# kazuto1011/dusty-gan

Measured on AMD Instinct MI355X. Metric: G+D train images/sec on 64x1024 LiDAR (steps/sec beside it), higher is better.
Workload: dtype bf16

## Files before the change

dusty_gan_amd/_lib.py:

```python
import ctypes as C
import os
import subprocess

_HERE = os.path.dirname(os.path.abspath(__file__))
CSRC = os.path.join(_HERE, "csrc")
LIB_PATH = os.path.join(CSRC, "libdustygan_hip.so")
if os.environ.get("DUSTY_GAN_LIB_DIAG"):
    _d = os.environ["DUSTY_GAN_LIB_DIAG"]
    LIB_PATH = os.path.join(CSRC, "libdustygan_hip_diag%s.so" % ("" if _d == "1" else _d))

DG_OK, DG_EINVAL, DG_EUNSUPPORTED, DG_EHIP = 0, 1, 2, 3
DG_F32, DG_BF16 = 0, 1
DG_BF16X2 = 2
MODE_S2, MODE_UP, MODE_GEMM = 0, 1, 2
EPI_LINEAR, EPI_LRELU, EPI_MASK = 0, 1, 2
DG_FORCE_AUTO, DG_FORCE_DIRECT, DG_FORCE_MFMA, DG_FORCE_THIN, DG_FORCE_LOCKSTEP, DG_FORCE_PINGPONG = 0, 1, 2, 3, 4, 5
DG_FORCE_WG_REGSTAGED, DG_FORCE_WG_DMA_PAIRS, DG_FORCE_WG_DMA_NOPAIRS, DG_FORCE_PINGPONG_SINGLE, DG_FORCE_PROJ_STREAM = 6, 7, 8, 9, 10
DG_FORCE_FP32X3 = 0x100
DG_CONV_FAMILY_DIRECT, DG_CONV_FAMILY_MFMA, DG_CONV_FAMILY_THIN, DG_CONV_FAMILY_LOCKSTEP, DG_CONV_FAMILY_PINGPONG = 1, 2, 3, 4, 5
DG_CONV_FAMILY_PROJ_STREAM = 6
DG_WGRAD_VARIANT_DIRECT, DG_WGRAD_VARIANT_MFMA, DG_WGRAD_VARIANT_THIN, DG_WGRAD_VARIANT_DMA, DG_WGRAD_VARIANT_THIN_MFMA = 1, 2, 3, 5, 7
POLICY_BITS = {"brightness": 1, "saturation": 2, "contrast": 4, "translation": 8, "cutout": 16}

_ERR = {1: "DG_EINVAL (bad argument)", 2: "DG_EUNSUPPORTED (shape not supported by the requested kernel)",
        3: "DG_EHIP (HIP runtime error)"}


class DgError(RuntimeError):
    pass


class DgConv(C.Structure):
    _fields_ = [
        ("mode", C.c_int), ("adj", C.c_int), ("ring", C.c_int),
        ("B", C.c_int), ("Hc", C.c_int), ("Wc", C.c_int),
        ("K", C.c_int), ("N", C.c_int),
        ("in_", C.c_void_p), ("in_sb", C.c_long), ("in_sp", C.c_long), ("in_sk", C.c_long),
        ("out", C.c_void_p), ("out_sb", C.c_long), ("out_sp", C.c_long), ("out_sn", C.c_long),
        ("w", C.c_void_p), ("w_st", C.c_long), ("w_sk", C.c_long), ("w_sn", C.c_long),
        ("scale", C.c_float), ("epi", C.c_int),
        ("bias", C.c_void_p), ("bias_mod", C.c_int),
        ("aux", C.c_void_p), ("dbias", C.c_void_p), ("rowscale", C.c_void_p),
        ("in_dtype", C.c_int), ("out_dtype", C.c_int), ("w_dtype", C.c_int),
        ("nscale", C.c_void_p),
        ("up_frag", C.c_void_p),
        ("dbias_ws", C.c_void_p),
        ("dbias_part", C.c_void_p),
        ("mask_out", C.c_void_p),
        ("mask_in", C.c_void_p),
        ("tanh_sum_parts", C.c_void_p),
    ]


UP_FRAG_BYTES = 3 * 18 * 1024
DBIAS_WS_FLOATS = 32 * 1024


class DgUpFrag(C.Structure):
    _fields_ = [("off", C.c_longlong), ("frag", C.c_void_p), ("m_st", C.c_longlong), ("m_sn", C.c_longlong),
                ("m_sk", C.c_longlong), ("N", C.c_int), ("Hc", C.c_int), ("adj", C.c_int)]


class DgDraw(C.Structure):
    _fields_ = [("kind", C.c_int), ("fill_kind", C.c_int), ("seed", C.c_uint64), ("stream_id", C.c_uint64),
                ("offset_dev", C.c_void_p), ("base", C.c_ulonglong), ("lo", C.c_float), ("hi", C.c_float),
                ("eps", C.c_float), ("ilo", C.c_int), ("ihi", C.c_int), ("n", C.c_long), ("out", C.c_void_p),
                ("out_bf16", C.c_void_p), ("B", C.c_int), ("H", C.c_int), ("W", C.c_int), ("uf", C.c_void_p),
                ("qi", C.c_void_p)]


class DgWgrad(C.Structure):
    _fields_ = [
        ("wmode", C.c_int), ("ring", C.c_int),
        ("B", C.c_int), ("Hc", C.c_int), ("Wc", C.c_int),
        ("Ci", C.c_int), ("Co", C.c_int),
        ("a", C.c_void_p), ("a_sb", C.c_long), ("a_sp", C.c_long), ("a_sc", C.c_long),
        ("g", C.c_void_p), ("g_sb", C.c_long), ("g_sp", C.c_long), ("g_sc", C.c_long),
        ("dw", C.c_void_p), ("scale", C.c_float), ("rowscale", C.c_void_p),
        ("a_dtype", C.c_int), ("g_dtype", C.c_int),
        ("ws", C.c_void_p), ("g_mod", C.c_int),
    ]


XSUM_PARTS = 8


class DgFetch(C.Structure):
    _fields_ = [("pol", C.c_void_p), ("mask", C.c_void_p), ("pool_ctr", C.c_void_p), ("npool", C.c_int),
                ("min_depth", C.c_float), ("max_depth", C.c_float), ("drop_const", C.c_float), ("B", C.c_int), ("HW", C.c_long),
                ("out", C.c_void_p), ("parts", C.c_void_p), ("nslab", C.c_long), ("flip_tab", C.c_void_p)]


class DgAugSet(C.Structure):
    _fields_ = [("x", C.c_void_p), ("xsum", C.c_void_p), ("xsum_parts", C.c_int), ("u_b", C.c_void_p), ("u_c", C.c_void_p), ("t_h", C.c_void_p),
                ("t_w", C.c_void_p), ("o_x", C.c_void_p), ("o_y", C.c_void_p)]


class DgOptSeg(C.Structure):
    _fields_ = [("off", C.c_longlong), ("numel", C.c_longlong), ("part", C.c_void_p), ("splits", C.c_int), ("accumulate", C.c_int),
                ("kind", C.c_int), ("ci", C.c_int), ("co", C.c_int), ("shadow_t", C.c_void_p), ("ws_src", C.c_void_p),
                ("ws_coef", C.c_void_p), ("ws_stride", C.c_longlong), ("ws_n", C.c_int), ("ws_bf16", C.c_int),
                ("ws_scale", C.c_float), ("first_block", C.c_int)]


OPT_MAX_SEG = 20


class DgWgradPlan(C.Structure):
    _fields_ = [("variant", C.c_int), ("splits", C.c_int), ("ws_floats", C.c_long), ("tap_pairs", C.c_int)]


class DgWgradReduce(C.Structure):
    _fields_ = [("ws", C.c_void_p), ("dw", C.c_void_p), ("numel", C.c_long), ("splits", C.c_int), ("accumulate", C.c_int)]


class DgConvPlan(C.Structure):
    _fields_ = [("family", C.c_int), ("bm", C.c_int), ("bn", C.c_int), ("tiles", C.c_int), ("workgroups", C.c_int),
                ("tiles_per_wg", C.c_int), ("thin_mfma", C.c_int), ("mask_bits", C.c_int), ("dbias_rows", C.c_int),
                ("sum_parts", C.c_int)]


_P, _I, _L, _F, _D, _U64 = C.c_void_p, C.c_int, C.c_long, C.c_float, C.c_double, C.c_uint64

PROTOTYPES = {
    "dg_conv": [C.POINTER(DgConv), _I, _P],
    "dg_conv_ex": [C.POINTER(DgConv), _I, _I, _P],
    "dg_conv_plan": [C.POINTER(DgConv), _I, _I, C.POINTER(DgConvPlan)],
    "dg_conv_mfma_supported": [C.POINTER(DgConv)],
    "dg_wgrad": [C.POINTER(DgWgrad), _I, _I, _P],
    "dg_wgrad_plan": [C.POINTER(DgWgrad), _I, _I, C.POINTER(DgWgradPlan)],
    "dg_wgrad_group": [C.POINTER(DgWgrad), _I, _I, _I, _P],
    "dg_wgrad_group_plan": [C.POINTER(DgWgrad), _I, _I, _I, C.POINTER(DgWgradPlan)],
    "dg_wgrad_reduce": [C.POINTER(DgWgradReduce), _I, _P],
    "dg_wgrad_mfma_supported": [C.POINTER(DgWgrad)],
    "dg_wgrad_kernel_variant": [C.POINTER(DgWgrad), _I],
    "dg_wgrad_has_sample_map": [C.POINTER(DgWgrad), _I],
    "dg_blur_fwd": [_P, _P, _I, _I, _I, _I, _I, _P],
    "dg_blur_fwd_mean": [_P, _P, _I, _I, _I, _I, _I, _P, _I, _P, _P],
    "dg_blur_bwd": [_P, _I, _P, _I, _I, _I, _I, _P],
    "dg_blur_bwd_r1": [_P, _I, _P, _F, _P, _I, _I, _I, _I, _P],
    "dg_blur_r1_tangent": [_P, _I, _P, _F, _P, _P, _I, _I, _I, _I, _I, _P],
    "dg_final_fwd": [_P, _I, _P, _P, _F, _I, _L, _P, _P],
    "dg_final_fwd_acc": [_P, _I, _P, _P, _F, _I, _L, _P, _P],
    "dg_final_bwd_data": [_P, _I, _P, _P, _P, _F, _I, _L, _I, _P, _P, _P],
    "dg_batch_wsum": [_P, _I, _P, _F, _I, _L, _P, _P],
    "dg_head_post_fwd": [_P, _P, _P, _I, _I, _F, _F, _I, _L, _P, _P, _P],
    "dg_head_post_fwd_sum": [_P, _P, _P, _I, _I, _F, _F, _I, _L, _P, _P, _P, _P],
    "dg_head_post_bwd": [_P, _P, _P, _P, _P, _I, _F, _F, _I, _L, _F, _F, _P, _P, _P, _I, _P, _P],
    "dg_logistic_noise": [_P, _P, _F, _L, _P, _P],
    "dg_diffaug_fwd": [_P, _P, _P, _P, _P, _P, _P, _I, _I, _I, _I, _P, _P, _P],
    "dg_diffaug_bwd": [_P, _P, _P, _P, _P, _P, _P, _I, _I, _I, _I, _P, _P, _P],
    "dg_diffaug_fwd_acc": [_P, _P, _P, _P, _P, _P, _P, _I, _I, _I, _I, _P, _P, _P],
    "dg_diffaug_fwd_pre": [_P, _P, _P, _P, _P, _P, _P, _I, _I, _I, _I, _P, _P, _P],
    "dg_diffaug_bwd_acc": [_P, _P, _P, _P, _P, _P, _P, _I, _I, _I, _I, _P, _P, _P],
    "dg_diffaug_blur_fwd": [C.POINTER(DgAugSet), _I, _I, _I, _I, _I, _I, _P, _I, _P],
    "dg_blur_bwd_augsum": [_P, _I, _P, _P, _P, _P, _I, _P, _I, _I, _I, _I, _P],
    "dg_diffaug_bwd_pre": [_P, _P, _P, _P, _P, _P, _P, _I, _I, _I, _I, _P, _P, _P],
    "dg_head_post_bwd_aug": [_P, _P, _P, _P, _P, _P, _P, _P, _P, _P, _P, _I, _P, _I, _F, _F, _I, _I, _I, _F, _F, _P, _P, _P,
                             _I, _P, _P],
    "dg_fetch_reals_pool_sum": [_P, _P, _P, _I, _F, _F, _F, _I, _L, _P, _P, _P],
    "dg_fetch_reals_resident_sum": [_P, _P, _L, _P, _F, _F, _F, _I, _L, _P, _P, _P],
    "dg_resident_gather": [_P, _L, _I, _L, _L, _P, _P, _P, _P],
    "dg_gan_d_step": [_I, _F, _P, _P, _I, _F, _P, _P, _P, _P, _P, _P],
    "dg_gan_g_step": [_I, _P, _P, _I, _F, _P, _P, _P],
    "dg_final_gan_bwd": [_I, _I, _F, _P, _P, _I, _F, _I, _P, _P, _P, _P, _P, _P, _I, _P, _F, _L, _I, _P, _P, _P, _P, _P],
    "dg_det_arena": [_P, _L, _P],
    "dg_mean_acc": [_P, _I, _P, _P],
    "dg_fetch_reals": [_P, _P, _F, _F, _F, _L, _P, _P],
    "dg_fetch_reals_sum": [_P, _P, _F, _F, _F, _I, _L, _P, _P, _P],
    "dg_pl_penalty": [_P, _I, _I, _F, _P, _P, _P, _P],
    "dg_head_post_bwd2": [_P, _P, _P, _P, _P, _P, _I, _F, _F, _I, _L, _F, _F, _P, _P, _P, _I, _P],
    "dg_scan_to_polar": [_P, _I, _I, _I, _I, _I, _I, _P, _D, _D, _F, _P, _P, _P, _P, _P],
    "dg_inv_to_xyz": [_P, _P, _I, _I, _I, _I, _F, _F, _F, _F, _P, _P, _P],
    "dg_unit_map": [_P, _L, _I, _P, _P],
    "dg_normals": [_P, _I, _I, _I, _I, _P, _P],
    "dg_scan_project": [_P, _P, _I, _I, _I, _P, _P, _P, _P, _P],
    "dg_angle_accum": [_P, _I, _I, _I, _I, _D, _D, _P, _P, _P],
    "dg_angle_finish": [_P, _P, _I, _I, _P, _P],
    "dg_splat_accum": [_P, _P, _I, _L, _I, _I, _I, _P, _P],
    "dg_render_points": [_P, _P, _I, _L, _I, _P, _I, _P, _I, _D, _P, _P],
    "dg_splat_finish": [_P, _I, _I, _I, _I, _I, _P, _P],
    "dg_image_grid": [_P, _L, _I, _I, _I, _I, _F, _I, _P, _P],
    "dg_turbo_lut": [_P],
    "dg_fps": [_P, _I, _I, _I, _P, _P, _P, _P],
    "dg_chamfer_dir": [_P, _I, _I, _P, _I, _I, _P, _P],
    "dg_chamfer_paired": [_P, _I, _P, _I, _I, _P, _P],
    "dg_chamfer_nn": [_P, _L, _L, _L, _I, _P, _L, _L, _L, _I, _I, _P, _P, _P],
    "dg_emd": [_P, _I, _I, _P, _I, _I, _I, _P, _P],
    "dg_grid_vote": [_P, _L, _P, _I, _P, _P],
    "dg_jsd": [_P, _P, _I, _P, _P],
    "dg_pyr_down": [_P, _L, _I, _I, _P, _P],
    "dg_pyr_up_sub": [_P, _P, _L, _I, _I, _P],
    "dg_extract_patches": [_P, _I, _I, _I, _I, _I, _I, _P, _I, _P, _P],
    "dg_sample_sum": [_P, _I, _L, _I, _P, _P],
# ... 320 lines not shown
```

dusty_gan_amd/csrc/api.hip:

```cpp
#include "common.h"

int dg_conv_direct_launch(const ConvP* p, hipStream_t stream);
int dg_lrelu_bits_launch(const ConvP* p, hipStream_t stream);
int dg_conv_mfma_launch(const ConvP* p, hipStream_t stream, int force, int fp32x3, int wg_cap, DgConvPlan* plan);
int dg_wgrad_mfma_dma_supported(const WgradP* p);
int dg_wgrad_mfma_dma_launch(const WgradP* p, int accumulate, int pairs, hipStream_t stream, DgWgradPlan* plan);
int dg_wgrad_mfma_dma_group_launch(const WgradP* items, int n, int pairs, int rounds, hipStream_t stream, DgWgradPlan* plans);
int dg_conv_thin_launch(const ConvP* p, hipStream_t stream);
int dg_conv_thin_supported(const ConvP* p);
int dg_proj_stream_supported(const ConvP* p);
int dg_proj_stream_launch(const ConvP* p, hipStream_t stream, DgConvPlan* plan);
int dg_conv_thin_mfma_variant(const ConvP* p);
int dg_conv_up_mfma_sum_parts(const ConvP* p);
int dg_conv_s2_mfma_blocks(const ConvP* p);
int dg_wgrad_thin_mfma_variant(const WgradP* p);
int dg_wgrad_thin_ws_splits(const WgradP* p);
int dg_wgrad_mfma_ws_splits(const WgradP* p, int accumulate);
int dg_wgrad_direct_ws_splits(const WgradP* p);
int dg_wgrad_direct_launch(const WgradP* p, hipStream_t stream);
int dg_wgrad_mfma_launch(const WgradP* p, int accumulate, hipStream_t stream, int x3);
int dg_wgrad_thin_launch(const WgradP* p, hipStream_t stream);
int dg_wgrad_thin_supported(const WgradP* p);

namespace {

enum ConvKernel { CONV_DIRECT, CONV_THIN, CONV_MFMA, CONV_PROJ_STREAM };

int select_conv(const DgConv* p, int force_flags, ConvKernel* k, DgConvPlan* plan) {
  if (p && (p->mask_out || p->mask_in)) {
    if (p->mask_out && p->epi != EPI_LRELU) return DG_EINVAL;
    if (p->mask_in && p->epi != EPI_MASK) return DG_EINVAL;
    if (p->out_sn != 1 || p->N % 8 != 0 || p->out_sp % 8 != 0 || p->out_sb % 8 != 0) return DG_EUNSUPPORTED;
  }
  if (!p || !p->in || !p->out || !p->w) return DG_EINVAL;
  if (p->B <= 0 || p->K <= 0 || p->N <= 0) return DG_EINVAL;
  if (p->mode != MODE_GEMM && (p->Hc < 2 || p->Wc < 2)) return DG_EINVAL;
  if (p->epi == EPI_MASK && !p->aux) return DG_EINVAL;
  if (p->bias && p->bias_mod <= 0) return DG_EINVAL;
  if (p->dbias && p->bias_mod <= 0) return DG_EINVAL;
  if (plan) *plan = DgConvPlan{};
  const int force = force_flags & ~DG_FORCE_FP32X3;
  const bool mfma_ok = !p->nscale && dg_conv_mfma_supported(p), thin_ok = dg_conv_thin_supported(p);
  const bool proj_ok = dg_proj_stream_supported(p);
  bool ok = true;
  if (force == DG_FORCE_AUTO) *k = proj_ok ? CONV_PROJ_STREAM : (mfma_ok ? CONV_MFMA : (thin_ok ? CONV_THIN : CONV_DIRECT));
  else if (force == DG_FORCE_PROJ_STREAM) *k = CONV_PROJ_STREAM, ok = proj_ok;
  else if (force == DG_FORCE_MFMA || force == DG_FORCE_LOCKSTEP || force == DG_FORCE_PINGPONG ||
           force == DG_FORCE_PINGPONG_SINGLE) *k = CONV_MFMA, ok = mfma_ok;
  else if (force == DG_FORCE_THIN) *k = CONV_THIN, ok = thin_ok;
  else *k = CONV_DIRECT;
  return ok ? DG_OK : DG_EUNSUPPORTED;
}

int conv_run(const DgConv* p, ConvKernel k, int force_flags, int wg_cap, hipStream_t s, DgConvPlan* plan) {
  if (k == CONV_PROJ_STREAM) return dg_proj_stream_launch(p, s, plan);
  if (k == CONV_MFMA)
    return dg_conv_mfma_launch(p, s, force_flags & ~DG_FORCE_FP32X3, (force_flags & DG_FORCE_FP32X3) ? 1 : 0, wg_cap, plan);
  if (!plan) return k == CONV_THIN ? dg_conv_thin_launch(p, s) : dg_conv_direct_launch(p, s);
  plan->family = k == CONV_THIN ? DG_CONV_FAMILY_THIN : DG_CONV_FAMILY_DIRECT;
  if (k == CONV_THIN) {
    plan->thin_mfma = dg_conv_thin_mfma_variant(p);
    plan->mask_bits = plan->thin_mfma == 1 ? 3 : 0;
    plan->dbias_rows = plan->thin_mfma == 1 ? dg_conv_s2_mfma_blocks(p) : 0;
    plan->sum_parts = plan->thin_mfma == 2 ? dg_conv_up_mfma_sum_parts(p) : 0;
  }
  return DG_OK;
}

int conv_dispatch(const DgConv* p, int force_flags, int wg_cap, hipStream_t s, DgConvPlan* plan) {
  ConvKernel k;
  int rc = select_conv(p, force_flags, &k, plan);
  if (rc || plan || !p->mask_out) return rc ? rc : conv_run(p, k, force_flags, wg_cap, s, plan);
  DgConvPlan pl{};
  rc = conv_run(p, k, force_flags, wg_cap, nullptr, &pl);
  if (rc == DG_OK) rc = conv_run(p, k, force_flags, wg_cap, s, nullptr);
  if (rc == DG_OK && !(pl.mask_bits & 1)) rc = dg_lrelu_bits_launch(p, s);
  return rc;
}

struct WgradKernel {
  int variant;
  int pairs;
  int splits;
  long ws_floats;
  bool takes_gmod;
  bool zero_dw;
};

int select_wgrad(const DgWgrad* p, int accumulate, int force_flags, WgradKernel* k) {
  if (!p || !p->a || !p->g || !p->dw) return DG_EINVAL;
  if (p->B <= 0 || p->Ci <= 0 || p->Co <= 0 || p->Hc <= 0 || p->Wc <= 0) return DG_EINVAL;
  const int force = force_flags & ~DG_FORCE_FP32X3;
  const bool mfma_ok = dg_wgrad_mfma_supported(p), thin_ok = dg_wgrad_thin_supported(p);
  const bool pairs = force == DG_FORCE_WG_DMA_PAIRS || force == DG_FORCE_WG_DMA_NOPAIRS;
  *k = WgradKernel{};
  if ((force == DG_FORCE_AUTO || force == DG_FORCE_MFMA || pairs) && mfma_ok && dg_wgrad_mfma_dma_supported(p)) {
    k->variant = DG_WGRAD_VARIANT_DMA, k->takes_gmod = true;
    k->pairs = force == DG_FORCE_WG_DMA_PAIRS ? 1 : (force == DG_FORCE_WG_DMA_NOPAIRS ? 2 : 0);
    return DG_OK;
  }
  if (force == DG_FORCE_AUTO)
    k->variant = mfma_ok ? DG_WGRAD_VARIANT_MFMA : (thin_ok ? DG_WGRAD_VARIANT_THIN : DG_WGRAD_VARIANT_DIRECT);
  else if (force == DG_FORCE_MFMA || force == DG_FORCE_WG_REGSTAGED) k->variant = mfma_ok ? DG_WGRAD_VARIANT_MFMA : 0;
  else if (force == DG_FORCE_THIN) k->variant = thin_ok ? DG_WGRAD_VARIANT_THIN : 0;
  else if (!pairs) k->variant = DG_WGRAD_VARIANT_DIRECT;
  if (!k->variant) return DG_EUNSUPPORTED;
  const int thin_mfma = k->variant == DG_WGRAD_VARIANT_THIN ? dg_wgrad_thin_mfma_variant(p) : 0;
  if (thin_mfma) k->variant = DG_WGRAD_VARIANT_THIN_MFMA;
  k->takes_gmod = thin_mfma == 1;
  if (k->variant == DG_WGRAD_VARIANT_THIN || k->variant == DG_WGRAD_VARIANT_THIN_MFMA) k->splits = dg_wgrad_thin_ws_splits(p);
  else if (k->variant == DG_WGRAD_VARIANT_MFMA) k->splits = dg_wgrad_mfma_ws_splits(p, accumulate);
  else if ((force == DG_FORCE_AUTO || force == DG_FORCE_DIRECT) && !p->g_mod) k->splits = dg_wgrad_direct_ws_splits(p);
  k->ws_floats = k->splits * (long)(p->wmode == 2 ? 1 : 16) * p->Ci * p->Co;
  k->zero_dw = !accumulate && !p->ws && k->variant != DG_WGRAD_VARIANT_MFMA;
  return DG_OK;
}

int wgrad_dispatch(const DgWgrad* p, int accumulate, int force_flags, hipStream_t s, DgWgradPlan* plan) {
  WgradKernel k;
  const int rc = select_wgrad(p, accumulate, force_flags, &k);
  if (rc == DG_EINVAL) return rc;
  if (plan) *plan = DgWgradPlan{k.variant, k.splits ? k.splits : 1, k.ws_floats, 0};
  if (rc) return rc;
  if (k.variant == DG_WGRAD_VARIANT_DMA) return dg_wgrad_mfma_dma_launch(p, accumulate, k.pairs, s, plan);
// ... 57 lines not shown
```

dusty_gan_amd/csrc/blur_aug.hip:

```cpp
#include "pointwise.h"
#include "diffaug.h"

template <typename T>
__global__ void blur_fwd_kernel(const float* __restrict__ x, T* __restrict__ out, int B, int H, int W, int ring) {
  const long idx = (long)blockIdx.x * blockDim.x + threadIdx.x;
  const long total = (long)B * H * W;
  if (idx >= total) return;
  const int xx = (int)(idx % W), y = (int)((idx / W) % H);
  const long base = idx - (long)y * W - xx;
  const int yu = y == 0 ? 1 : y - 1, yd = y == H - 1 ? H - 2 : y + 1;
  int xl = xx - 1, xr = xx + 1;
  if (ring) { if (xl < 0) xl += W; if (xr >= W) xr -= W; }
  else      { if (xl < 0) xl = 1;  if (xr >= W) xr = W - 2; }
  const float c = x[idx];
  const float v = 0.25f * x[base + (long)yu * W + xx] + 0.5f * c + 0.25f * x[base + (long)yd * W + xx];
  const float h = 0.25f * x[base + (long)y * W + xl] + 0.5f * c + 0.25f * x[base + (long)y * W + xr];
  out[idx * 2 + 0] = (T)v;
  out[idx * 2 + 1] = (T)h;
}

template <typename T>
__global__ void blur_bwd_kernel(const T* __restrict__ d, float* __restrict__ dx, int B, int H, int W, int ring) {
  const long idx = (long)blockIdx.x * blockDim.x + threadIdx.x;
  const long total = (long)B * H * W;
// ... 131 lines not shown
                                                        float oscale, float* __restrict__ ssq, AugP win, int use_win,
                                                        const DgDet det) {
  __shared__ float red[16];
  const int W4 = W >> 2, b = blockIdx.y;
  const long base = (long)b * H * W;
  const int y0 = blockIdx.x * NR;
  const AugSample ws = aug_window(win, b);
  float ssacc = 0.f;
  for (int q4 = threadIdx.x; q4 < W4; q4 += 256) {
    const int x0 = q4 * 4;
    float g[NR][4];
    blur_adj_rows<T, NR>(d, base, y0, x0, H, W, ring, g);
#pragma unroll
    for (int j = 0; j < NR; ++j) {
      const int y = y0 + j;
      const float g0 = g[j][0], g1 = g[j][1], g2 = g[j][2], g3 = g[j][3];
      *(float4*)(dx + base + (long)y * W + x0) = make_float4(oscale * g0, oscale * g1, oscale * g2, oscale * g3);
      if (!use_win) {
        ssacc += g0 * g0 + g1 * g1 + g2 * g2 + g3 * g3;
      } else {
        const AugRow wr = aug_row<false>(win, ws, y);
        const float gq[4] = {g0, g1, g2, g3};
#pragma unroll
        for (int k = 0; k < 4; ++k)
          if (aug_in_window(wr, x0 + k)) ssacc += gq[k];
      }
    }
  }
  if (ssq) {
    const float sblk = dg_block_sum(ssacc, red);
    if (threadIdx.x == 0) dg_acc_add(&ssq[b], sblk, gridDim.x, det);
  }
}
template <typename T>
static void blur_bwd4_launch(const void* d, float* dx, int B, int H, int W, int ring, float oscale, float* ssq, int rows_pb,
                             const AugP& win, int use_win, hipStream_t s) {
  const dim3 grid(H / rows_pb, B);
  const DgDet det = dg_det_current();
  if (rows_pb == 4) blur_bwd4_kernel<T, 4><<<grid, 256, 0, s>>>((const T*)d, dx, H, W, ring, oscale, ssq, win, use_win, det);
  else if (rows_pb == 2) blur_bwd4_kernel<T, 2><<<grid, 256, 0, s>>>((const T*)d, dx, H, W, ring, oscale, ssq, win, use_win, det);
  else blur_bwd4_kernel<T, 1><<<grid, 256, 0, s>>>((const T*)d, dx, H, W, ring, oscale, ssq, win, use_win, det);
}
static void blur_bwd4_launch(const void* d, int dtype, float* dx, int B, int H, int W, int ring, float oscale, float* ssq,
                             int rows_pb, const AugP& win, int use_win, hipStream_t s) {
  if (dtype == DG_BF16) blur_bwd4_launch<bf16>(d, dx, B, H, W, ring, oscale, ssq, rows_pb, win, use_win, s);
  else blur_bwd4_launch<float>(d, dx, B, H, W, ring, oscale, ssq, rows_pb, win, use_win, s);
}
static int blur_rows_pb(int H) { return H % 4 == 0 ? 4 : (H % 2 == 0 ? 2 : 1); }

#define R1T_ROWS 4
template <typename T>
__global__ __launch_bounds__(256) void blur_r1_tangent_kernel(const T* __restrict__ d, T* __restrict__ out, int H, int W,
                                                              int ring, float oscale, float* __restrict__ ssq,
                                                              float* __restrict__ mean_acc, int mean_n, const DgDet det) {
  extern __shared__ float s_g[];
  __shared__ float red[16];
  const int W4 = W >> 2, b = blockIdx.y;
  const long base = (long)b * H * W;
  const int y0 = blockIdx.x * R1T_ROWS;
  float ssacc = 0.f;
  for (int q4 = threadIdx.x; q4 < W4; q4 += 256) {
    const int x0 = q4 * 4;
    float g[R1T_ROWS + 2][4];
    blur_adj_rows<T, R1T_ROWS + 2>(d, base, y0 - 1, x0, H, W, ring, g);
#pragma unroll
    for (int r = 0; r < R1T_ROWS + 2; ++r) {
      const int y = y0 - 1 + r;
      if (y < 0 || y >= H) continue;
      const float g0 = g[r][0], g1 = g[r][1], g2 = g[r][2], g3 = g[r][3];
      *(float4*)(s_g + r * W + x0) = make_float4(oscale * g0, oscale * g1, oscale * g2, oscale * g3);
      if (r >= 1 && r <= R1T_ROWS) ssacc += g0 * g0 + g1 * g1 + g2 * g2 + g3 * g3;
    }
  }
  __syncthreads();
  for (int yy = 0; yy < R1T_ROWS; ++yy) {
    const int y = y0 + yy;
    const int yu = y == 0 ? 1 : y - 1, yd = y == H - 1 ? H - 2 : y + 1;
    const float* rc = s_g + (y - y0 + 1) * W;
    const float* ru = s_g + (yu - y0 + 1) * W;
    const float* rd = s_g + (yd - y0 + 1) * W;
    for (int q4 = threadIdx.x; q4 < W4; q4 += 256) {
      const int x0 = q4 * 4;
      const float4 c4 = *(const float4*)(rc + x0);
      const float4 u4 = *(const float4*)(ru + x0);
      const float4 d4 = *(const float4*)(rd + x0);
      int xl = x0 - 1, xr = x0 + 4;
      if (ring) { if (xl < 0) xl += W; if (xr >= W) xr -= W; }
      else      { if (xl < 0) xl = 1;  if (xr >= W) xr = W - 2; }
      const float c[6] = {rc[xl], c4.x, c4.y, c4.z, c4.w, rc[xr]};
      const float u[4] = {u4.x, u4.y, u4.z, u4.w}, dn[4] = {d4.x, d4.y, d4.z, d4.w};
      float o[8];
#pragma unroll
      for (int k = 0; k < 4; ++k) {
        o[2 * k] = 0.25f * u[k] + 0.5f * c[k + 1] + 0.25f * dn[k];
        o[2 * k + 1] = 0.25f * c[k] + 0.5f * c[k + 1] + 0.25f * c[k + 2];
      }
      T* op = out + (base + (long)y * W + x0) * 2;
      if constexpr (sizeof(T) == 2) {
        Vec16<bf16>::store((bf16*)op, o);
      } else {
        *(float4*)op = make_float4(o[0], o[1], o[2], o[3]);
        *(float4*)(op + 4) = make_float4(o[4], o[5], o[6], o[7]);
      }
    }
  }
  const float sblk = dg_block_sum(ssacc, red);
  if (threadIdx.x == 0) {
    float tot = 0.f;
    const int last = dg_acc_add_last(&ssq[b], sblk, gridDim.x, det, tot);
    if (mean_acc) {
      if (last == 1) dg_acc_add(mean_acc, tot / (float)mean_n, gridDim.y, det);
      else if (last < 0) atomicAdd(mean_acc, sblk / (float)mean_n);
    }
  }
}

__global__ __launch_bounds__(256) void sample_sum_kernel(const float* __restrict__ x, long n, int sq,
                                                         float* __restrict__ out, const DgDet det) {
  __shared__ float red[16];
  const int b = blockIdx.y;
  const float* row = x + (long)b * n;
  float acc = 0.f;
  if ((n & 3) == 0 && (((size_t)row) & 15) == 0) {
    for (long i = ((long)blockIdx.x * blockDim.x + threadIdx.x) * 4; i < n; i += (long)gridDim.x * blockDim.x * 4) {
      const float4 v = *(const float4*)(row + i);
      acc += sq ? v.x * v.x + v.y * v.y + v.z * v.z + v.w * v.w : v.x + v.y + v.z + v.w;
    }
  } else {
    for (long i = (long)blockIdx.x * blockDim.x + threadIdx.x; i < n; i += (long)gridDim.x * blockDim.x) {
      const float v = row[i];
      acc += sq ? v * v : v;
    }
  }
  const float s = dg_block_sum(acc, red);
  if (threadIdx.x == 0) dg_acc_add(&out[b], s, gridDim.x, det);
}


__global__ __launch_bounds__(256) void diffaug_fwd_kernel(AugP a, const float* __restrict__ x, const float* __restrict__ xsum,
                                                          float* __restrict__ y) {
  const int yy = blockIdx.x, b = blockIdx.y, W = a.W;
  const long HW = (long)a.H * W;
  float* yrow = y + (long)b * HW + (long)yy * W;
  const AugSample s = aug_sample(a, b);
  const AugRow r = aug_row<false>(a, s, yy);
  const float mean = aug_mean(a, s, (a.policy & 4) ? xsum[b] : 0.f);
  const float* xrow = x + (long)b * HW + (long)(r.ok ? r.y : 0) * W;
#pragma unroll 4
  for (int xx = threadIdx.x; xx < W; xx += 256) {
    const float v = aug_fwd_px(s, mean, xrow[aug_src_col(s, xx)]);
// ... 116 lines not shown
  const float* grow = gy + (long)b * HW + (long)(r.ok ? r.y : 0) * W;
  const float gb = grow[W - 1];
#pragma unroll 4
  for (int c = threadIdx.x; c < W; c += 256) out[c] = aug_adj_px(a, s, r, grow, gb, gm, c);
}

static inline bool blur4_ok(const void* a, const void* b, int H, int W) {
  return W % 4 == 0 && W >= 8 && H >= 2 && ((size_t)a & 15) == 0 && ((size_t)b & 15) == 0;
}

extern "C" {

int dg_blur_fwd_mean(const float* x, void* out, int dtype, int B, int H, int W, int ring, const float* mean_src, int mean_n,
                     float* mean_acc, void* s_) {
  hipStream_t s = (hipStream_t)s_;
  if (!mean_src || !mean_acc || mean_n < 1) return DG_EINVAL;
  if (!blur4_ok(x, out, H, W)) return DG_EUNSUPPORTED;
  if (dtype == DG_BF16) blur_fwd4_kernel<bf16><<<dim3(H, B), 256, 0, s>>>(x, (bf16*)out, B, H, W, ring, mean_src, mean_n, mean_acc);
  else blur_fwd4_kernel<float><<<dim3(H, B), 256, 0, s>>>(x, (float*)out, B, H, W, ring, mean_src, mean_n, mean_acc);
  HIP_CHECK_RET(hipGetLastError());
  return DG_OK;
}

int dg_blur_fwd(const float* x, void* out, int dtype, int B, int H, int W, int ring, void* s_) {
  hipStream_t s = (hipStream_t)s_;
  const long n = (long)B * H * W;
  if (blur4_ok(x, out, H, W)) {
    if (dtype == DG_BF16) blur_fwd4_kernel<bf16><<<dim3(H, B), 256, 0, s>>>(x, (bf16*)out, B, H, W, ring, nullptr, 0, nullptr);
    else blur_fwd4_kernel<float><<<dim3(H, B), 256, 0, s>>>(x, (float*)out, B, H, W, ring, nullptr, 0, nullptr);
  } else if (dtype == DG_BF16) blur_fwd_kernel<bf16><<<nblk(n), 256, 0, s>>>(x, (bf16*)out, B, H, W, ring);
  else blur_fwd_kernel<float><<<nblk(n), 256, 0, s>>>(x, (float*)out, B, H, W, ring);
  HIP_CHECK_RET(hipGetLastError());
  return DG_OK;
}

int dg_blur_bwd(const void* d, int dtype, float* dx, int B, int H, int W, int ring, void* s_) {
  hipStream_t s = (hipStream_t)s_;
  const long n = (long)B * H * W;
  if (blur4_ok(d, dx, H, W)) blur_bwd4_launch(d, dtype, dx, B, H, W, ring, 1.f, nullptr, 1, AugP{}, 0, s);
  else if (dtype == DG_BF16) blur_bwd_kernel<bf16><<<nblk(n), 256, 0, s>>>((const bf16*)d, dx, B, H, W, ring);
  else blur_bwd_kernel<float><<<nblk(n), 256, 0, s>>>((const float*)d, dx, B, H, W, ring);
  HIP_CHECK_RET(hipGetLastError());
  return DG_OK;
}

int dg_blur_bwd_r1(const void* d, int dtype, float* dx, float oscale, float* ssq, int B, int H, int W, int ring, void* s_) {
  if (!ssq) return DG_EINVAL;
  if (!blur4_ok(d, dx, H, W) || ((long)H * W) % 1024 != 0) return DG_EUNSUPPORTED;
  blur_bwd4_launch(d, dtype, dx, B, H, W, ring, oscale, ssq, blur_rows_pb(H), AugP{}, 0, (hipStream_t)s_);
  HIP_CHECK_RET(hipGetLastError());
  return DG_OK;
}

int dg_blur_r1_tangent(const void* d, int dtype, void* out, float oscale, float* ssq, float* mean_acc, int mean_n, int B, int H,
                       int W, int ring, void* s_) {
  hipStream_t s = (hipStream_t)s_;
  if (!d || !out || !ssq || B <= 0 || (mean_acc && mean_n < 1)) return DG_EINVAL;
  if (dtype != DG_BF16 && dtype != DG_F32) return DG_EINVAL;
  const size_t lds = (size_t)(R1T_ROWS + 2) * W * sizeof(float);
  if (W % 4 != 0 || W < 8 || H < 4 || H % R1T_ROWS != 0 || lds > 60 * 1024 || ((size_t)d & 15) != 0 || ((size_t)out & 15) != 0)
    return DG_EUNSUPPORTED;
  const dim3 grid(H / R1T_ROWS, B);
  const DgDet det = dg_det_current();
  if (dtype == DG_BF16) blur_r1_tangent_kernel<bf16><<<grid, 256, lds, s>>>((const bf16*)d, (bf16*)out, H, W, ring, oscale, ssq, mean_acc, mean_n, det);
  else blur_r1_tangent_kernel<float><<<grid, 256, lds, s>>>((const float*)d, (float*)out, H, W, ring, oscale, ssq, mean_acc, mean_n, det);
  HIP_CHECK_RET(hipGetLastError());
  return DG_OK;
}

static int sample_sum_impl(const float* x, int B, long n, int sq, float* out, bool zero, void* s_) {
  hipStream_t s = (hipStream_t)s_;
  if (zero) { const int zrc = dg_zero_f32(out, B, s); if (zrc) return zrc; }
  unsigned gx = nblk(n, 256 * 8);
  if (gx > 64) gx = 64;
  if (gx < 1) gx = 1;
  sample_sum_kernel<<<dim3(gx, B), 256, 0, s>>>(x, n, sq, out, dg_det_current());
  HIP_CHECK_RET(hipGetLastError());
  return DG_OK;
}

int dg_sample_sum(const float* x, int B, long n, int sq, float* out, void* s_) {
  return sample_sum_impl(x, B, n, sq, out, true, s_);
}
int dg_sample_sum_acc(const float* x, int B, long n, int sq, float* out, void* s_) {
  return sample_sum_impl(x, B, n, sq, out, false, s_);
}

static int diffaug_fwd_impl(const float* x, const float* u_b, const float* u_c, const int* t_h, const int* t_w,
                            const int* o_x, const int* o_y, int policy, int B, int H, int W, float* xsum, float* y,
                            bool zero, void* s_) {
  hipStream_t s = (hipStream_t)s_;
  const AugP a = make_aug(u_b, u_c, t_h, t_w, o_x, o_y, policy, B, H, W);
  if (policy & 4) {
    const int rc = sample_sum_impl(x, B, (long)H * W, 0, xsum, zero, s);
    if (rc) return rc;
  }
  diffaug_fwd_kernel<<<dim3(H, B), 256, 0, s>>>(a, x, xsum, y);
  HIP_CHECK_RET(hipGetLastError());
  return DG_OK;
}

int dg_diffaug_fwd(const float* x, const float* u_b, const float* u_c, const int* t_h, const int* t_w,
                   const int* o_x, const int* o_y, int policy, int B, int H, int W, float* xsum, float* y,
                   void* s_) {
  return diffaug_fwd_impl(x, u_b, u_c, t_h, t_w, o_x, o_y, policy, B, H, W, xsum, y, true, s_);
}
int dg_diffaug_fwd_acc(const float* x, const float* u_b, const float* u_c, const int* t_h, const int* t_w,
                       const int* o_x, const int* o_y, int policy, int B, int H, int W, float* xsum, float* y,
                       void* s_) {
  return diffaug_fwd_impl(x, u_b, u_c, t_h, t_w, o_x, o_y, policy, B, H, W, xsum, y, false, s_);
}

int dg_diffaug_fwd_pre(const float* x, const float* u_b, const float* u_c, const int* t_h, const int* t_w,
                       const int* o_x, const int* o_y, int policy, int B, int H, int W, const float* xsum, float* y,
                       void* s_) {
  hipStream_t s = (hipStream_t)s_;
  const AugP a = make_aug(u_b, u_c, t_h, t_w, o_x, o_y, policy, B, H, W);
  diffaug_fwd_kernel<<<dim3(H, B), 256, 0, s>>>(a, x, xsum, y);
  HIP_CHECK_RET(hipGetLastError());
  return DG_OK;
// ... 77 lines not shown
```

dusty_gan_amd/csrc/conv_mfma_pp.hip:

```cpp
#include "conv_mfma_persist_impl.h"

#include <type_traits>

namespace pp {

using persist::Geo;
using persist::Tile;

typedef __attribute__((ext_vector_type(4))) float f32x4_t;

#define PP_WAIT(vm) asm volatile("s_waitcnt vmcnt(%0) lgkmcnt(0)" ::"n"(vm) : "memory")

constexpr int NHT = 256;
struct HTab { unsigned long long e[NHT]; };

__device__ __forceinline__ unsigned long long pp_stamp() {
  unsigned long long t;
  __builtin_amdgcn_sched_barrier(0);
  asm volatile("s_memtime %0\n\ts_waitcnt lgkmcnt(0)" : "=s"(t)::"memory");
  __builtin_amdgcn_sched_barrier(0);
  return t;
}

template <int CTRL>
// ... 93 lines not shown
    t.xt += dstep.xt + c; c = t.xt >= tiles_x; if (c) t.xt -= tiles_x;
    if (MODE == MODE_UP && !DUAL) { t.px += dstep.px + c; c = t.px >> 1; t.px &= 1; }
    t.Y += dstep.Y + c; c = t.Y >= rows; if (c) t.Y -= rows;
    t.bt += dstep.bt + c;
  };

  const bf16* in = (const bf16*)p.in;
  const bf16* w = (const bf16*)p.w;
  const int lrow = lane >> 3, pos = lane & 7;
  auto swzA = [](int row) { return ((row >> 1) & 3) << 1; };
  auto swzB = [](int row) { return ((row >> 1) & 1) | (((row / CPL) & 3) << 1); };

  unsigned voffA[NPAIR][IA + 1], voffB[IB];
  int colA[IA + 1];
  unsigned sampA[IA + 1];
  {
    const int pitch = g.SW + (DUAL ? 2 : 1);
#pragma unroll
    for (int u = 0; u <= IA; ++u) {
      const int m = (u < IA ? (wave + NWV * u) : 32) * 8 + lrow;
      int seg = m / pitch, c = m - seg * pitch;
      if (seg >= g.NSB) { seg = 0; c = 0; }
      colA[u] = cmul * c;
      sampA[u] = (unsigned)(seg * (int)p.in_sb * 2 + (pos ^ swzA(m)) * 16);
    }
  }
#pragma unroll
  for (int u = 0; u < IB; ++u) {
    const int row = (wave + NWV * u) * 8 + lrow;
    voffB[u] = (unsigned)((DUAL ? row & 63 : row) * (int)p.w_sn * 2 + (pos ^ swzB(row)) * 16);
  }
  const unsigned dst_wave = (unsigned)wave * 1024u;

  const int wm = wave >> 1, wn = wave & 1;
  const int a16 = lane & 15, g4 = lane >> 4;
  const unsigned lds0 = (unsigned)(size_t)(__attribute__((address_space(3))) unsigned char*)lds;
  unsigned pbase[2];
  {
    const int rowbase = ((wm * 64) >> g.lsw) * (g.SW + (DUAL ? 2 : 1)) + ((wm * 64) & (g.SW - 1));
#pragma unroll
    for (int t = 0; t < 2; ++t) {
      const int r = rowbase + a16 + t + (DUAL ? wn : 0);
      pbase[t] = (unsigned)(r * SB + ((g4 ^ swzA(r)) << 4));
    }
  }
  const unsigned wrow = (unsigned)(wn * WC + (a16 >> 2) * CPL + (a16 & 3));
  const unsigned wbase = (unsigned)(AIMG + wrow * SB + ((g4 ^ (((a16 >> 1) & 1) | ((a16 >> 2) << 1))) << 4));

  float* s_rs = (float*)(lds + NPS * PSTAGE);
  float* s_bias = s_rs + NDB;
  float* s_db = s_bias + NDB;
  const unsigned srs0 = lds0 + NPS * PSTAGE, sbias0 = srs0 + NDB * 4, sdb0 = sbias0 + NDB * 4;
  const bool want_db = MASK && p.dbias != nullptr;
  const bool db_rows = MASK && DBW * p.N <= NDBR * NDB;
  const unsigned sdbw0 = db_rows ? sbias0 + (unsigned)((DUAL ? wave : wave / WN) * p.N) * 4u : sdb0;
  for (int i = tid; i < NDB; i += 64 * NWV) {
    s_bias[i] = (!MASK && p.bias && i < p.N) ? p.bias[i % p.bias_mod] * (p.epi == EPI_LRELU ? SQRT2 : 1.f) : 0.f;
    s_db[i] = 0.f;
    s_rs[i] = (p.rowscale && i < p.B) ? p.rowscale[i] : 1.f;
  }
  if (MASK)
    for (int i = tid; i < NDBX; i += 64 * NWV) s_db[NDB + i] = 0.f;
  __syncthreads();
  const unsigned long long tk1 = (dbg & 8) ? pp_stamp() : 0ull;

  f32x4_t acc[TM][TN];
  auto zero_acc = [&]() __attribute__((always_inline)) {
#pragma unroll
    for (int i = 0; i < TM; ++i)
#pragma unroll
      for (int j = 0; j < TN; ++j) acc[i][j] = f32x4_t{0.f, 0.f, 0.f, 0.f};
  };
  zero_acc();
  i32x4 fp[2][TM], fw[2][TN];

  bf16* out = (bf16*)p.out;
  const unsigned lane_c0 = (unsigned)((DUAL ? 0 : wn * WC) + g4 * CPL);
  const unsigned lane_coff = X2 ? lane_c0 * 2 + ((lane_c0 >> 6) << 7) : lane_c0 * 2;
  const unsigned par_off = DUAL ? (unsigned)(wn * (int)p.out_sp * 2) : 0u;
  const long px_b = (long)(MODE == MODE_S2 ? 1 : 2) * p.out_sp * 2;
  unsigned pix_off;
  {
    const int trow = wm * 64 + a16;
    const int sb = trow >> g.lsw, x = trow & (g.SW - 1);
    pix_off = (unsigned)((sb * (int)p.out_sb + (MODE == MODE_S2 ? x : 2 * x) * (int)p.out_sp) * 2) + lane_coff + par_off;
  }
  constexpr int CH = WC / 8;
  constexpr int RPB = 64 / CH;
  constexpr int NRD = 16 / RPB;
  static_assert(NRD == NST / TM, "strip geometry");
  auto swzS = [](int px) { return CH == 8 ? (px & 7) : ((px >> 1) & 3); };
  const unsigned scr0 = lds0 + NPS * PSTAGE + 3 * NDB * 4 + NDBX * 4 + (unsigned)wave * SCR;
  const unsigned scr_w = scr0 + (unsigned)(a16 * (CH * 16) + (((g4 * NRD) ^ swzS(a16)) << 4));
  unsigned scr_r, st_off;
  {
    const int pr = lane / CH, c = lane % CH;
    scr_r = scr0 + (unsigned)(pr * (CH * 16) + ((c ^ swzS(pr)) << 4));
    const int trow = wm * 64 + pr;
    const int sb = trow >> g.lsw, x = trow & (g.SW - 1);
    st_off = (unsigned)((sb * (int)p.out_sb + (MODE == MODE_S2 ? x : 2 * x) * (int)p.out_sp) * 2 + c * 16) +
             (DUAL ? par_off : (unsigned)((wn * WC) * 2));
  }
  static_assert(NRD == 1 || RPB * CH * 16 == 1024, "strip read offset");
  auto tile_off = [&](const Tile& t) __attribute__((always_inline)) -> long {
    const int n0 = t.xt * BM;
    return (long)(t.bt * g.NSB) * p.out_sb + ((long)t.Y * Wo + (MODE == MODE_S2 ? n0 : 2 * n0 + t.px)) * p.out_sp +
           t.nt * NCH * (X2 ? 2 : 1);
  };
  i32x4 axr[(MASK && !BITS) ? NST : 1];
  unsigned mbits[BITS ? TM : 1];
  const unsigned pix_off_m = pix_off >> 4;
  auto load_aux = [&](const Tile& t) __attribute__((always_inline)) {
    if constexpr (BITS) {
      const char* mb = (const char*)p.mask_in + (tile_off(t) >> 3);
#pragma unroll
      for (int i = 0; i < TM; ++i) {
        const char* src = mb + (long)i * px_b;
        if (CPL == 16) asm volatile("global_load_ushort %0, %1, %2" : "=v"(mbits[i]) : "v"(pix_off_m), "s"(src) : "memory");
        else asm volatile("global_load_ubyte %0, %1, %2" : "=v"(mbits[i]) : "v"(pix_off_m), "s"(src) : "memory");
      }
    } else {
      const char* ab = (const char*)((const bf16*)p.aux + tile_off(t));
#pragma unroll
      for (int i = 0; i < TM; ++i) {
        const char* src = ab + (long)(i * 16) * px_b;
        asm volatile("global_load_dwordx4 %0, %1, %2" : "=v"(axr[(NST / TM) * i]) : "v"(pix_off), "s"(src) : "memory");
        if (NST / TM == 2) asm volatile("global_load_dwordx4 %0, %1, %2 offset:16" : "=v"(axr[2 * i + 1]) : "v"(pix_off), "s"(src) : "memory");
      }
    }
  };
  auto flush_db = [&](float (&dbacc)[CPL], int nt) __attribute__((always_inline)) {
// ... 93 lines not shown
          unsigned pw;
          asm("v_cvt_pk_bf16_f32 %0, %1, %2" : "=v"(pw) : "v"(v2[0]), "v"(v2[1]));
          pk[e2] = (int)pw;
          if constexpr (X2) {
            const float l0 = v2[0] - __builtin_bit_cast(float, pw << 16);
            const float l1 = v2[1] - __builtin_bit_cast(float, pw & 0xffff0000u);
            unsigned pl;
            asm("v_cvt_pk_bf16_f32 %0, %1, %2" : "=v"(pl) : "v"(l0), "v"(l1));
            pkl[e2] = (int)pl;
          }
        }
        if (!MASK && mob) {
          unsigned tb[4];
#pragma unroll
          for (int e2 = 0; e2 < 4; ++e2)
            asm("v_pk_max_i16 %0, %1, 0\n\tv_pk_min_u16 %0, %0, 1 op_sel_hi:[1,0]" : "=&v"(tb[e2]) : "v"(pk[e2]));
          const unsigned mm = tb[0] | (tb[1] << 2) | (tb[2] << 4) | (tb[3] << 6);
          const unsigned gb = (mm & 0x55u) | ((mm >> 15) & 0xAAu);
          if (h == 0) mrow = gb; else mrow |= gb << 8;
          if (h == NST / TM - 1) {
            char* dstm = mob + (long)i * px_b;
            if (CPL == 16) asm volatile("global_store_short %0, %1, %2" ::"v"(pix_off_m), "v"(mrow), "s"(dstm) : "memory");
            else asm volatile("global_store_byte %0, %1, %2" ::"v"(pix_off_m), "v"(mrow), "s"(dstm) : "memory");
          }
        }
        if (!STRIP) {
          char* dstp = ob + (long)(i * 16) * px_b + pix_off + h * 16;
          if (!(dbg & 128)) *(i32x4*)dstp = pk; else asm volatile("" ::"v"(pk));
          if constexpr (X2) {
            if (!(dbg & 128)) *(i32x4*)(dstp + 128) = pkl; else asm volatile("" ::"v"(pkl));
          }
          continue;
        }
        if (h == 0 && i > 0) store_row(i - 1);
        asm volatile("ds_write_b128 %0, %1" ::"v"(scr_w ^ (unsigned)(h << 4)), "v"(pk) : "memory");
      }
      if (STRIP) {
        asm volatile("s_waitcnt lgkmcnt(0)" ::: "memory");
#pragma unroll
        for (int h = 0; h < NRD; ++h)
          asm volatile("ds_read_b128 %0, %1 offset:%2" : "=v"(rd[h]) : "v"(scr_r), "n"(h * 1024) : "memory");
      }
      __builtin_amdgcn_sched_barrier(0);
    }
    if (STRIP) store_row(TM - 1);
    if (want_db) flush_db(dbacc, t.nt);
    zero_acc();
  };

  const bool stamps = (dbg & 8) != 0;
  unsigned long long tsum[6] = {0, 0, 0, 0, 0, 0};
  unsigned long long tend = 0, tkf = 0;

  if (wave >= 4) __builtin_amdgcn_s_barrier();
  unsigned so_c = PSTAGE, so_i = 0;
  bool pending = false;
  bool warm = true;
  Tile tprev = first;
  const long tap_b = (long)p.w_st * 2;
  const unsigned spb = (unsigned)p.in_sp * 2u;

  auto dma_s = [&](unsigned voff, const char* sbase, unsigned ldsbase, auto off_tag) __attribute__((always_inline)) {
    constexpr int OFF = decltype(off_tag)::value;
    asm volatile("s_add_u32 m0, %0, %3\n\ts_nop 0\n\tglobal_load_lds_dwordx4 %1, %2"
                 ::"s"(ldsbase), "v"(voff), "s"(sbase), "n"(OFF) : "memory", "scc");
  };

  auto pair_iter = [&](auto iss_tag, const bool first, const int pi, const char* sA, const char* sB0, const char* sB1,
                       const char* sB0b, const char* sB1b) __attribute__((always_inline)) {
    constexpr bool ISS = decltype(iss_tag)::value;
    const bool comp = !warm;
    auto step = [&](auto t_tag) __attribute__((always_inline)) {
      constexpr int t = decltype(t_tag)::value;
      unsigned long long t0 = 0, t1 = 0, t2 = 0, t3 = 0, t4 = 0, t5 = 0;
      if (stamps) { t0 = pp_stamp(); if (tend) tsum[5] += t0 - tend; }
      const bool last = t == 1 && first && !warm;
      {
        const unsigned so = lds0 + so_c;
        const unsigned pa0 = so + pbase[t], pa1 = so + (pbase[t] ^ 64u);
        const unsigned wa0 = so + wbase + t * BT, wa1 = so + ((wbase ^ 64u) + t * BT);
        const unsigned dst = lds0 + so_i + dst_wave;
        constexpr int NP = t == 0 ? IA + IB : IB;
        auto piece = [&](auto q_tag) __attribute__((always_inline)) {
          constexpr int q = decltype(q_tag)::value;
          if (!ISS || (dbg & 1)) return;
          if constexpr (t == 0 && q < IA) dma_s(voffA[pi][q], sA, dst, std::integral_constant<int, NWV * q * 1024>{});
          else if constexpr (t == 0) dma_s(voffB[q - IA], (DUAL && q - IA == 1) ? sB0b : sB0, dst, std::integral_constant<int, AIMG + NWV * (q - IA) * 1024>{});
          else dma_s(voffB[q], (DUAL && q == 1) ? sB1b : sB1, dst, std::integral_constant<int, AIMG + BT + NWV * q * 1024>{});
        };
        if (ISS && t == 0 && wave == 0 && !(dbg & 1))
          dma_s(voffA[pi][IA], sA, lds0 + so_i, std::integral_constant<int, 32 * 1024>{});
        constexpr int NR = 2 * TM + 2 * TN;
        int q = 0;
        auto pieces_upto = [&](int r) __attribute__((always_inline)) {
#define PP_PIECE(Q) if constexpr (Q < NP) { if (q == Q && r * NP >= Q * NR) { piece(std::integral_constant<int, Q>{}); ++q; } }
          PP_PIECE(0) PP_PIECE(1) PP_PIECE(2) PP_PIECE(3) PP_PIECE(4) PP_PIECE(5) PP_PIECE(6) PP_PIECE(7)
#undef PP_PIECE
        };
#pragma unroll
        for (int r = 0; r < NR; ++r) {
          pieces_upto(r);
          if (dbg & 16) continue;
          if (r < 2 * TM) {
            const int i = r >> 1;
            if (r & 1) LDS_READ128(fp[1][i], pa1, i * 16 * SB); else LDS_READ128(fp[0][i], pa0, i * 16 * SB);
          } else {
            const int jj = (r - 2 * TM) >> 1;
            if (r & 1) LDS_READ128(fw[1][jj], wa1, jj * 4 * SB); else LDS_READ128(fw[0][jj], wa0, jj * 4 * SB);
          }
        }
        pieces_upto(1 << 20);
        pieces_upto(1 << 20);
      }
      if (stamps) t1 = pp_stamp();
      if (!ISS) PP_WAIT(0);
      else if (t == 0) { if (wave == 0) PP_WAIT(IA + IB + 1); else PP_WAIT(IA + IB); }
      else PP_WAIT(IB);
      auto finish_tile = [&]() __attribute__((always_inline)) {
        if (!(dbg & 4)) epilogue(tprev);
        else {
#pragma unroll
          for (int i = 0; i < TM; ++i)
#pragma unroll
            for (int jj = 0; jj < TN; ++jj) asm volatile("" ::"v"(acc[i][jj]));
          zero_acc();
        }
        pending = false;
      };
      if (t == 0 && pending && wave >= 4) finish_tile();
      if (stamps) t2 = pp_stamp();
      __builtin_amdgcn_s_barrier();
      if (stamps) t3 = pp_stamp();
      __builtin_amdgcn_sched_barrier(0);
      if (t == 0 && pending) finish_tile();
      __builtin_amdgcn_sched_barrier(0);
      if (comp) {
        if (stamps && tkf == 0) tkf = t3;
#pragma unroll
        for (int ks = 0; ks < 2; ++ks) {
          if (!(dbg & 2)) {
#pragma unroll
            for (int i = 0; i < TM; ++i)
#pragma unroll
              for (int jj = 0; jj < TN; ++jj)
                acc[i][jj] = __builtin_amdgcn_mfma_f32_16x16x32_bf16(__builtin_bit_cast(bf16x8, fw[ks][jj]),
                                                                      __builtin_bit_cast(bf16x8, fp[ks][i]), acc[i][jj], 0, 0, 0);
          }
          if (ks == 0) {
            __builtin_amdgcn_sched_barrier(0);
            if (MASK && last && !(dbg & (4 | 64))) load_aux(tprev);
          }
        }
        if (last) pending = true;
      }
      __builtin_amdgcn_sched_barrier(0);
      if (stamps) t4 = pp_stamp();
      if (ISS || t == 0 || wave < 4) __builtin_amdgcn_s_barrier();
      if (stamps) {
        t5 = pp_stamp();
        tsum[0] += t1 - t0; tsum[1] += t2 - t1; tsum[2] += t3 - t2; tsum[3] += t4 - t3; tsum[4] += t5 - t4;
        tend = t5;
      }
    };
    step(std::integral_constant<int, 0>{});
    step(std::integral_constant<int, 1>{});
    const unsigned sw_ = so_c; so_c = so_i; so_i = sw_;
  };

  Tile ti = first;
  for (int c = 0; c < tcount; ++c) {
    unsigned long long hl;
    int nh;
    {
      const unsigned long long e = ht.e[ti.Y];
      nh = (int)(e >> 60) & 7;
      hl = e & 0x0fffffffffffffffull;
    }
    const char* in_t = (const char*)(in + (long)(ti.bt * g.NSB) * p.in_sb);
    const char* w_t = (const char*)(w + (long)(ti.nt * NCH) * p.w_sn);
    const int x0 = cmul * ti.xt * BM;
#pragma unroll
    for (int pi = 0; pi < NPAIR; ++pi) {
      const int cb = MODE == MODE_S2 ? pi - 1 : ((DUAL || ti.px == 0) ? -1 : 0);
#pragma unroll
      for (int u = 0; u <= IA; ++u)
        voffA[pi][u] = __umul24((unsigned)((x0 + colA[u] + cb) & (Ws - 1)), spb) + sampA[u];
    }
    const int kxa = MODE == MODE_S2 ? 0 : (ti.px == 0 ? 3 : 2), kxb = MODE == MODE_S2 ? 2 : (ti.px == 0 ? 1 : 0);
    bool firstg = true;
    for (int h = 0; h < nh; ++h) {
      const int it_r = (int)(hl & 1023) >> 2, it_ky = (int)hl & 3;
      hl >>= 10;
      const char* sA_row = in_t + (long)it_r * Ws * spb;
      const char* sB_row = w_t + (long)(it_ky * 4) * tap_b;
      for (int kc = 0; kc < (X2 ? 3 : 1) * KC; ++kc) {
        const int kq = X2 ? kc / 3 : kc, sub = X2 ? kc - 3 * kq : 0;
        const char* sA_k = sA_row + kq * (X2 ? 2 * SB : SB) + (sub == 1 ? SB : 0);
        const char* sB_k = sB_row + kq * (X2 ? 2 * SB : SB) + (sub == 2 ? SB : 0);
#pragma unroll
        for (int pi = 0; pi < NPAIR; ++pi) {
          pair_iter(std::true_type{}, firstg, pi, sA_k, sB_k + (long)(kxa + pi) * tap_b, sB_k + (long)(kxb + pi) * tap_b,
                    sB_k + 2 * tap_b, sB_k);
          if (firstg) { firstg = false; warm = false; }
        }
      }
    }
    tprev = ti;
    tile_next(ti);
  }
  pair_iter(std::false_type{}, true, 0, nullptr, nullptr, nullptr, nullptr, nullptr);
  const unsigned long long tk2 = (dbg & 8) ? pp_stamp() : 0ull;
  const unsigned long long tr2 = (dbg & 8) ? __builtin_amdgcn_s_memrealtime() : 0ull;
  if (pending && !(dbg & 4)) {
    asm volatile("s_waitcnt vmcnt(0)" ::: "memory");
    epilogue(tprev);
  }
  if (stamps && blockIdx.x == 0 && lane == 0) {
    float* sink = (float*)p.out + wave * 8;
    asm volatile("s_waitcnt vmcnt(0)" ::: "memory");
    const unsigned long long tk3 = pp_stamp();
    for (int k = 0; k < 6; ++k) sink[k] = (float)tsum[k];
    float* ph = (float*)p.out + 64 + wave * 8;
    ph[0] = (float)(tk1 - tk0); ph[1] = (float)(tkf - tk0); ph[2] = (float)(tk2 - tk0); ph[3] = (float)(tk3 - tk0);
    ph[4] = (float)tcount;
    ph[5] = (float)(tr2 - tr0);
  }
  if (want_db) {
    asm volatile("s_waitcnt vmcnt(0) lgkmcnt(0)" ::: "memory");
    __syncthreads();
    for (int n = tid; n < p.N; n += 64 * NWV) {
// ... 27 lines not shown
  const int cap = (wg_cap > 0 && wg_cap < resident) ? wg_cap : resident;
  const int G = g.ntiles < cap ? g.ntiles : cap;
  if (plan) {
    plan->family = DG_CONV_FAMILY_PINGPONG; plan->bm = DUAL ? 512 : 256; plan->bn = DUAL ? BN / 2 : BN; plan->tiles = g.ntiles; plan->workgroups = G;
    plan->tiles_per_wg = (g.ntiles + G - 1) / G;
    plan->mask_bits = MASK ? (bits ? 2 : 0) : 1;
    plan->dbias_rows = (MASK && (DUAL ? 8 : 4) * p->N <= 2048) ? G : 0;
    return DG_OK;
  }
  HTab ht;
  {
    const int rows = MODE == MODE_S2 ? p->Hc : 2 * p->Hc;
    for (int y = 0; y < NHT; ++y) {
      unsigned long long hl = 0;
      const int nh = y < rows ? persist::pack_htaps<MODE>(p->adj, y, p->Hc, hl) : 0;
      ht.e[y] = hl | ((unsigned long long)nh << 60);
    }
  }
  if constexpr (X2) {
    conv_pp_kernel<BN, MODE, MASK, DUAL, false, true><<<(unsigned)G, 512, 0, stream>>>(*p, g, ht);
  } else if constexpr (MASK) {
    if (bits) conv_pp_kernel<BN, MODE, true, DUAL, true><<<(unsigned)G, 512, 0, stream>>>(*p, g, ht);
    else conv_pp_kernel<BN, MODE, true, DUAL, false><<<(unsigned)G, 512, 0, stream>>>(*p, g, ht);
  } else conv_pp_kernel<BN, MODE, false, DUAL><<<(unsigned)G, 512, 0, stream>>>(*p, g, ht);
  HIP_CHECK_RET(hipGetLastError());
  return DG_OK;
}

}

int dg_conv_mfma_pp_launch(const ConvP* p0, hipStream_t stream, int min_tiles, int wg_cap, DgConvPlan* plan, int dual) {
  if (p0->mode != MODE_S2 && p0->mode != MODE_UP) return DG_EUNSUPPORTED;
  const bool x2 = p0->in_dtype == DG_BF16X2;
  if (p0->in_dtype != p0->out_dtype || p0->in_dtype != p0->w_dtype || (p0->in_dtype != DG_BF16 && !x2)) return DG_EUNSUPPORTED;
  ConvP q = *p0;
  if (x2) {
    if (p0->K % 64 || p0->N % 64 || p0->in_sp % 64 || p0->in_sb % 64 || p0->out_sp % 64 || p0->out_sb % 64 || p0->w_sn % 64 ||
        p0->w_st % 64 || (((size_t)p0->in | (size_t)p0->out | (size_t)p0->w | (size_t)p0->aux) & 255))
      return DG_EUNSUPPORTED;
    if (p0->mask_out || p0->mask_in) return DG_EUNSUPPORTED;
    q.in_sb *= 2; q.in_sp *= 2; q.out_sb *= 2; q.out_sp *= 2; q.w_st *= 2; q.w_sn *= 2;
  }
  const ConvP* p = &q;
  if (p->K % 64 != 0 || !p->ring || p->nscale) return DG_EUNSUPPORTED;
  if (p->mode == MODE_UP && p->adj && p->K < 128) return DG_EUNSUPPORTED;
  if (p->in_sk != 1 || p->w_sk != 1 || p->out_sn != 1) return DG_EUNSUPPORTED;
  if (p->out_sp % 8 != 0 || p->in_sp % 8 != 0 || p->w_sn % 8 != 0) return DG_EUNSUPPORTED;
  if (p->N > 512 || (p->bias && p->bias_mod < p->N && p->N % p->bias_mod != 0)) return DG_EUNSUPPORTED;
  if (p->dbias && p->bias_mod < p->N) return DG_EUNSUPPORTED;
  const int Ws = p->mode == MODE_S2 ? 2 * p->Wc : p->Wc;
  if ((Ws & (Ws - 1)) != 0 || p->in_sp * 2 >= (1 << 24)) return DG_EUNSUPPORTED;
  if ((p->mode == MODE_S2 ? p->Hc : 2 * p->Hc) > 256) return DG_EUNSUPPORTED;
  const bool mask = p->epi == EPI_MASK;
  if (mask ? p->bias != nullptr : p->dbias != nullptr) return DG_EUNSUPPORTED;
  if (p->rowscale && p->B > 512) return DG_EUNSUPPORTED;
  persist::Geo g;
  int bn = 0;
  if (dual && p->mode == MODE_UP && p->N % 128 != 0 && p->N % 64 == 0 && persist::make_geo<256, 64>(p, g) && g.SW >= 64 &&
      g.NSB * (g.SW + 2) <= 264 && g.ntiles / 2 >= min_tiles) {
    g.ntiles /= 2;
    if (x2) return mask ? pp::launch<128, MODE_UP, true, true, true>(p, g, stream, wg_cap, plan)
                        : pp::launch<128, MODE_UP, false, true, true>(p, g, stream, wg_cap, plan);
    return mask ? pp::launch<128, MODE_UP, true, true>(p, g, stream, wg_cap, plan)
                : pp::launch<128, MODE_UP, false, true>(p, g, stream, wg_cap, plan);
  }
  if (p->N % 128 == 0 && persist::make_geo<256, 128>(p, g) && g.SW >= 64 && g.ntiles >= min_tiles) bn = 128;
  else if (p->N % 64 == 0 && persist::make_geo<256, 64>(p, g) && g.SW >= 64 && g.ntiles >= min_tiles) bn = 64;
  if (!bn) return DG_EUNSUPPORTED;
  const int sel = (bn == 128 ? 0 : 4) + (p->mode == MODE_UP ? 2 : 0) + (mask ? 1 : 0);
  if (x2) switch (sel) {
    case 0: return pp::launch<128, MODE_S2, false, false, true>(p, g, stream, wg_cap, plan);
    case 1: return pp::launch<128, MODE_S2, true, false, true>(p, g, stream, wg_cap, plan);
    case 2: return pp::launch<128, MODE_UP, false, false, true>(p, g, stream, wg_cap, plan);
    case 3: return pp::launch<128, MODE_UP, true, false, true>(p, g, stream, wg_cap, plan);
    case 4: return pp::launch<64, MODE_S2, false, false, true>(p, g, stream, wg_cap, plan);
    case 5: return pp::launch<64, MODE_S2, true, false, true>(p, g, stream, wg_cap, plan);
    case 6: return pp::launch<64, MODE_UP, false, false, true>(p, g, stream, wg_cap, plan);
    default: return pp::launch<64, MODE_UP, true, false, true>(p, g, stream, wg_cap, plan);
  }
  switch (sel) {
    case 0: return pp::launch<128, MODE_S2, false>(p, g, stream, wg_cap, plan);
    case 1: return pp::launch<128, MODE_S2, true>(p, g, stream, wg_cap, plan);
    case 2: return pp::launch<128, MODE_UP, false>(p, g, stream, wg_cap, plan);
    case 3: return pp::launch<128, MODE_UP, true>(p, g, stream, wg_cap, plan);
    case 4: return pp::launch<64, MODE_S2, false>(p, g, stream, wg_cap, plan);
    case 5: return pp::launch<64, MODE_S2, true>(p, g, stream, wg_cap, plan);
    case 6: return pp::launch<64, MODE_UP, false>(p, g, stream, wg_cap, plan);
    default: return pp::launch<64, MODE_UP, true>(p, g, stream, wg_cap, plan);
  }
}
```

dusty_gan_amd/csrc/conv_thin.hip:

```cpp
#include "common.h"
#include "mfma_common.h"
#include "thin_up_frag.h"

#include <stdlib.h>
#include <type_traits>

#define SK_PX 64
template <int KMAX>
__global__ __launch_bounds__(256) void thin_smallk_kernel(ConvP p, int tiles_x, int n_base) {
  __shared__ float s_in[6][2 * SK_PX + 2][KMAX];
  __shared__ float s_w[16][KMAX][64];
  __shared__ int s_tap[1 + 2 * 6];
  __shared__ float s_db[64];
  const int tid = threadIdx.x;
  const int Y = blockIdx.x % p.Hc, b = blockIdx.x / p.Hc;
  const int Wf = 2 * p.Wc;
  if (tid == 0) {
    int nt = 0;
    for (int i = 0; i < 6; ++i) {
      int r, ky;
      if (dg_tap1d(MODE_S2, p.adj, 0, Y, p.Hc, i, r, ky)) { s_tap[1 + 2 * nt] = r; s_tap[2 + 2 * nt] = ky; ++nt; }
    }
    s_tap[0] = nt;
  }
// ... 411 lines not shown
  const int tid = threadIdx.x, lane = tid & 63;
  const int wave = __builtin_amdgcn_readfirstlane(tid >> 6);
  const long units = (long)p.B * p.Hc;
  const long u0 = (long)blockIdx.x * rows_pb;
  const bf16* A = (const bf16*)p.a;
  const bf16* G = (const bf16*)p.g;
  const int lr = lane & 31, lh = lane >> 5;
  const int m_ky = lr >> 3, m_kx = (lr >> 1) & 3, m_ci = lr & 1;
  const int g16 = lane >> 4, i16 = lane & 15;
  const int kh = g16 >> 1, cb = g16 & 1, q = i16 >> 2, pp = i16 & 3;
  unsigned char* my_g = s_g + wave * 16 * 144;
  tw_f32x16 acc[2];
#pragma unroll
  for (int j = 0; j < 2; ++j)
#pragma unroll
    for (int e = 0; e < 16; ++e) acc[j][e] = 0.f;
  const int seg = p.Wc / 4;
  const int npc = Wf / 4;
  tw_u32x4 sa[NPT];
  unsigned sh = 0;
  auto fetch_a = [&](long u) __attribute__((always_inline)) {
    const int b = (int)(u / p.Hc), Y = (int)(u % p.Hc);
    const bf16* img = A + (long)b * p.a_sb;
#pragma unroll
    for (int k = 0; k < NPT; ++k) {
      const int i = tid + 256 * k;
      if (i < Wf) {
        const int kk = i / npc, pc = i % npc;
        int ra, rg;
        dg_wgrad1d(0, 0, Y, p.Hc, kk, ra, rg);
        sa[k] = *(const tw_u32x4*)(img + ((long)ra * Wf + 4 * pc) * 2);
      }
    }
    if (tid < 8) {
      int ra, rg;
      dg_wgrad1d(0, 0, Y, p.Hc, tid >> 1, ra, rg);
      sh = *(const unsigned*)(img + ((long)ra * Wf + ((tid & 1) ? 0 : Wf - 1)) * 2);
    }
  };
  auto put_a = [&]() __attribute__((always_inline)) {
#pragma unroll
    for (int k = 0; k < NPT; ++k) {
      const int i = tid + 256 * k;
      if (i < Wf) *(tw_u32x4*)(s_a + (i / npc) * ncol + 4 + 4 * (i % npc)) = sa[k];
    }
    if (tid < 8) s_a[(tid >> 1) * ncol + ((tid & 1) ? Wf + 4 : 3)] = sh;
  };
  const long uend = u0 + rows_pb < units ? u0 + rows_pb : units;
  const int spr = seg / 16, gpr = (spr + WG_GS - 1) / WG_GS, ngr = (int)(uend - u0) * gpr;
  auto load_group = [&](int gq, tw_u32x4 (&gt)[WG_GS][2]) __attribute__((always_inline)) {
    const long u = u0 + gq / gpr;
    const int s0 = (gq % gpr) * WG_GS;
    const int b = (int)(u / p.Hc), Y = (int)(u % p.Hc);
    const int bg = p.g_mod > 0 ? b % p.g_mod : b;
    const bf16* grow = G + (long)bg * p.g_sb + ((long)Y * p.Wc + wave * seg + 16 * s0) * p.g_sp;
#pragma unroll
    for (int st = 0; st < WG_GS; ++st)
      if (s0 + st < spr) {
#pragma unroll
        for (int v = 0; v < 2; ++v) {
          const int c = lane + 64 * v, row = c >> 3, part = c & 7;
          gt[st][v] = *(const tw_u32x4*)(grow + (long)(16 * st + row) * p.g_sp + part * 8);
        }
      }
  };
  const bf16* s_a16 = (const bf16*)s_a;
  auto run_group = [&](int gq, const tw_u32x4 (&gt)[WG_GS][2]) __attribute__((always_inline)) {
    if (gq % gpr == 0) {
      __syncthreads();
      put_a();
      __syncthreads();
      if (u0 + gq / gpr + 1 < uend) fetch_a(u0 + gq / gpr + 1);
    }
    const int s0 = (gq % gpr) * WG_GS;
#pragma unroll
    for (int st = 0; st < WG_GS; ++st) {
      if (s0 + st >= spr) break;
      const int xb = wave * seg + 16 * (s0 + st);
#pragma unroll
      for (int v = 0; v < 2; ++v) {
        const int c = lane + 64 * v, row = c >> 3, part = c & 7;
        *(tw_u32x4*)(my_g + row * 144 + part * 16) = gt[st][v];
      }
      tw_bf16x8 fa;
#pragma unroll
      for (int j = 0; j < 8; ++j)
        fa[j] = s_a16[((long)m_ky * ncol + 2 * (xb + 8 * lh + j) + m_kx + 3) * 2 + m_ci];
#pragma unroll
      for (int jt = 0; jt < 2; ++jt) {
        const unsigned char* ptr = my_g + (8 * kh + q) * 144 + (jt * 32 + 16 * cb + 4 * pp) * 2;
        const tw_bf16x4 lo = __builtin_amdgcn_ds_read_tr16_b64_v4bf16((tw_bf16x4 __attribute__((address_space(3)))*)(ptr));
        const tw_bf16x4 hi = __builtin_amdgcn_ds_read_tr16_b64_v4bf16((tw_bf16x4 __attribute__((address_space(3)))*)(ptr + 4 * 144));
        const tw_bf16x8 fg = __builtin_shufflevector(lo, hi, 0, 1, 2, 3, 4, 5, 6, 7);
        acc[jt] = __builtin_amdgcn_mfma_f32_32x32x16_bf16(fa, fg, acc[jt], 0, 0, 0);
      }
    }
  };
  tw_u32x4 gta[WG_GS][2], gtb[WG_GS][2];
  fetch_a(u0);
  load_group(0, gta);
  for (int gq = 0; gq < ngr; gq += 2) {
    if (gq + 1 < ngr) load_group(gq + 1, gtb);
    run_group(gq, gta);
    if (gq + 2 < ngr) load_group(gq + 2, gta);
    if (gq + 1 < ngr) run_group(gq + 1, gtb);
  }
  const int b0 = (int)(u0 / p.Hc);
// ... 435 lines not shown
}
static bool wgrad_down_mfma_ok(const WgradP* p) {
  if (!(p->wmode == 0 && p->a_dtype == DG_BF16 && p->g_dtype == DG_BF16 && p->Ci == 2 && p->Co == 64 && p->a_sc == 1 &&
        p->g_sc == 1 && p->a_sp == 2 && p->g_sp == 64 && p->Wc % 64 == 0 && p->Hc % WG_ROWS_PB == 0))
    return false;
  return wgrad_down_mfma_lds(p) <= 160 * 1024 && 2 * p->Wc <= 4096 && p->a_sb % 8 == 0 && ((size_t)p->a & 15) == 0 &&
         p->g_sb % 8 == 0 && ((size_t)p->g & 15) == 0;
}
static int wgrad_up_pairs(const WgradP* p) { return (p->Co > 2 && p->g_sp == 4) ? 2 : 1; }
static size_t wgrad_up_mfma_lds_np(const WgradP* p, int np) {
  size_t lds = (size_t)np * 32 * (p->Wc * 2 + 16) + 4 * 16 * 144;
  if (lds < (size_t)4 * np * 32 * 64 * 4) lds = (size_t)4 * np * 32 * 64 * 4;
  return lds;
}
static size_t wgrad_up_mfma_lds(const WgradP* p) {
  const size_t two = wgrad_up_mfma_lds_np(p, wgrad_up_pairs(p));
  return two <= 160 * 1024 ? two : wgrad_up_mfma_lds_np(p, 1);
}
static bool wgrad_up_mfma_ok(const WgradP* p) {
  if (!(p->wmode == 1 && p->a_dtype == DG_BF16 && p->g_dtype == DG_BF16 && p->Ci == 64 && p->a_sc == 1 &&
        p->a_sp == 64 && p->g_sc == 1 && (p->g_sp == 2 || p->g_sp == 4) && p->Co <= p->g_sp && p->g_sb % 2 == 0 &&
        p->Wc % 64 == 0 && p->Hc >= 2 && p->Hc % WGU_ROWS_PB == 0 && p->a_sb % 8 == 0 && ((size_t)p->a & 15) == 0))
    return false;
  return wgrad_up_mfma_lds(p) <= 160 * 1024;
}
int dg_wgrad_thin_mfma_variant(const WgradP* p) {
  if (!dg_wgrad_thin_supported(p)) return 0;
  return wgrad_down_mfma_ok(p) ? 1 : (wgrad_up_mfma_ok(p) ? 2 : 0);
}

static int wgrad_down_rows_pb(const WgradP* p) {
  return ((long)p->B * p->Hc >= 2048 && p->Hc % 4 == 0) ? 4 : WG_ROWS_PB;
}
static unsigned wgrad_valu_grid(const WgradP* p) {
  const long units = (long)p->B * p->Hc;
  return units < 1024 ? (unsigned)units : 1024u;
}
int dg_wgrad_thin_ws_splits(const WgradP* p) {
  if (!dg_wgrad_thin_supported(p)) return 0;
  const long units = (long)p->B * p->Hc;
  long nb = 0;
  if (wgrad_down_mfma_ok(p)) nb = units / wgrad_down_rows_pb(p);
  else if (wgrad_up_mfma_ok(p)) {
    const bool one_pass = p->Co <= 2 || (wgrad_up_pairs(p) == 2 && wgrad_up_mfma_lds(p) == wgrad_up_mfma_lds_np(p, 2));
    if (one_pass) nb = units / WGU_ROWS_PB;
  } else if (!p->g_mod) nb = wgrad_valu_grid(p);
  return nb > 0 && nb <= 65536 ? (int)nb : 0;
}

int dg_wgrad_thin_launch(const WgradP* p, hipStream_t s) {
  if (!dg_wgrad_thin_supported(p)) return DG_EUNSUPPORTED;
  if (p->ws && !dg_wgrad_thin_ws_splits(p)) return DG_EUNSUPPORTED;
  if (p->g_mod && !wgrad_down_mfma_ok(p)) return DG_EUNSUPPORTED;
  const long units = (long)p->B * p->Hc;
  const unsigned grid = wgrad_valu_grid(p);
  if (wgrad_down_mfma_ok(p)) {
    const size_t lds = wgrad_down_mfma_lds(p);
    const int Wf = 2 * p->Wc;
    {
      const void* fn = Wf <= 256 ? (const void*)thin_wgrad_down_mfma_kernel<1>
                                 : (Wf <= 1024 ? (const void*)thin_wgrad_down_mfma_kernel<4> : (const void*)thin_wgrad_down_mfma_kernel<16>);
      if (lds > 64 * 1024)
        HIP_CHECK_RET(hipFuncSetAttribute(fn, hipFuncAttributeMaxDynamicSharedMemorySize, (int)lds));
      const int rows_pb = wgrad_down_rows_pb(p);
      const unsigned nb = (unsigned)(units / rows_pb);
      if (Wf <= 256) thin_wgrad_down_mfma_kernel<1><<<nb, 256, lds, s>>>(*p, rows_pb);
      else if (Wf <= 1024) thin_wgrad_down_mfma_kernel<4><<<nb, 256, lds, s>>>(*p, rows_pb);
      else thin_wgrad_down_mfma_kernel<16><<<nb, 256, lds, s>>>(*p, rows_pb);
      HIP_CHECK_RET(hipGetLastError());
      return DG_OK;
    }
  }
  if (wgrad_up_mfma_ok(p)) {
    const size_t lds = wgrad_up_mfma_lds(p);
    {
      const bool both = wgrad_up_pairs(p) == 2 && lds == wgrad_up_mfma_lds_np(p, 2);
      if (lds > 64 * 1024)
        HIP_CHECK_RET(hipFuncSetAttribute(both ? (const void*)thin_wgrad_up_mfma_kernel<2> : (const void*)thin_wgrad_up_mfma_kernel<1>,
                                          hipFuncAttributeMaxDynamicSharedMemorySize, (int)lds));
      if (both) {
        thin_wgrad_up_mfma_kernel<2><<<(unsigned)(units / WGU_ROWS_PB), 256, lds, s>>>(*p, 0);
      } else {
        for (int gpair = 0; 2 * gpair < p->Co; ++gpair)
          thin_wgrad_up_mfma_kernel<1><<<(unsigned)(units / WGU_ROWS_PB), 256, lds, s>>>(*p, gpair);
      }
      HIP_CHECK_RET(hipGetLastError());
      return DG_OK;
    }
  }
  if (p->wmode == 0) {
    const size_t lds = (size_t)4 * (2 * p->Wc + 2) * (p->Ci <= 2 ? 2 : 4) * sizeof(float);
    if (lds > 64 * 1024)
      HIP_CHECK_RET(hipFuncSetAttribute(p->Ci <= 2 ? (const void*)thin_wgrad_down_kernel<2> : (const void*)thin_wgrad_down_kernel<4>,
                                        hipFuncAttributeMaxDynamicSharedMemorySize, (int)lds));
    for (int cb = 0; cb < p->Co; cb += 64) {
      if (p->Ci <= 2) thin_wgrad_down_kernel<2><<<grid, 256, lds, s>>>(*p, cb);
      else thin_wgrad_down_kernel<4><<<grid, 256, lds, s>>>(*p, cb);
    }
  } else {
    const size_t lds = (size_t)2 * 2 * p->Wc * 4 * sizeof(float);
    if (lds > 64 * 1024)
      HIP_CHECK_RET(hipFuncSetAttribute((const void*)thin_wgrad_up_kernel<4>, hipFuncAttributeMaxDynamicSharedMemorySize, (int)lds));
    for (int cb = 0; cb < p->Ci; cb += 64)
      thin_wgrad_up_kernel<4><<<grid, 256, lds, s>>>(*p, cb);
  }
  HIP_CHECK_RET(hipGetLastError());
// ... 18 lines not shown

  auto wval = [&](int ky, int kx, int c, int n) -> bf16 {
    return c < p.K ? w[(long)(ky * 4 + kx) * p.w_st + (long)n * p.w_sn + c] : (bf16)0.f;
  };
  tw_bf16x8 fb[NS][2], fbx[2];
#pragma unroll
  for (int jt = 0; jt < 2; ++jt) {
    const int n = jt * 32 + lr;
#pragma unroll
    for (int s = 0; s < NS; ++s)
#pragma unroll
      for (int j = 0; j < 8; ++j) {
        const int ky = CP == 2 ? 2 * s + lh : s;
        const int kx = CP == 2 ? (j >> 1) : 2 * lh + (j >> 2);
        const int c = CP == 2 ? (j & 1) : (j & 3);
        fb[s][jt][j] = wval(ky, kx, c, n);
      }
#pragma unroll
    for (int j = 0; j < 8; ++j) fbx[jt][j] = CP == 2 ? wval(3, j >> 1, j & 1, n) : (bf16)0.f;
  }

  float csum[8];
#pragma unroll
  for (int e = 0; e < 8; ++e) csum[e] = 0.f;
  const int gw = blockIdx.x * 4 + wave, nw = gridDim.x * 4;
  const int nt = (int)ntiles, tq = nt / nw, tr = nt % nw;
  const int t0 = gw * tq + (gw < tr ? gw : tr), tcnt = tq + (gw < tr ? 1 : 0);
  int xt = t0 % tiles_x, Y = (t0 / tiles_x) % p.Hc, b = t0 / (tiles_x * p.Hc);
  unsigned char* my = s_t[wave];
  auto window_of = [&](int bb, int r, int c0) -> uint4 {
    constexpr int NPX = 8 / CP;
    const bf16* img = in + (long)bb * p.in_sb;
    if (c0 >= 0 && c0 + NPX <= Wf) return *(const uint4*)(img + ((long)r * Wf + c0) * CP);
    unsigned d[4];
#pragma unroll
    for (int q = 0; q < 4; ++q) {
      int cc = c0 + (CP == 2 ? q : (q >> 1));
      if (cc < 0) cc += Wf; else if (cc >= Wf) cc -= Wf;
      d[q] = *(const unsigned*)(img + ((long)r * Wf + cc) * CP + (CP == 2 ? 0 : (q & 1) * 2));
    }
    return make_uint4(d[0], d[1], d[2], d[3]);
  };
  typedef unsigned v4u __attribute__((ext_vector_type(4)));
  typedef unsigned v2u __attribute__((ext_vector_type(2)));
  constexpr int NPXD = CP / 2;
  constexpr int NF = 2 * NS + 1 + (MB == 2 ? 1 : 0);
  constexpr int NSTO = 4 + (MB == 1 ? 4 : 0);
  v4u pa[2][NS];
  typedef typename std::conditional<CP == 2, unsigned, v2u>::type wrap_t;
  wrap_t pw[2][NS];
  v2u pm[2];
  float prs[2];
  const int Wd = Wf * NPXD;
  const float* rs_src = (p.dbias && p.rowscale) ? p.rowscale : (const float*)p.w;
  const unsigned zero_off = 0u;
  auto out_base = [&](int xt_, int Y_, int b_) -> long { return (long)b_ * p.out_sb + ((long)Y_ * p.Wc + xt_ * 32) * 64; };
  auto prefetch = [&](int xt_, int Y_, int b_, auto buf_tag) __attribute__((always_inline)) {
    constexpr int I = decltype(buf_tag)::value;
    const char* img = (const char*)(in + (long)b_ * p.in_sb);
    const int d0 = (2 * (xt_ * 32 + lr) - 1 + (CP == 2 ? 0 : 2 * lh)) * NPXD;
    const int d0c = min(max(d0, 0), Wd - 4);
    const int dw = d0 < 0 ? Wd - NPXD : 0;
#pragma unroll
    for (int s = 0; s < NS; ++s) {
      const int ky = CP == 2 ? 2 * s + lh : s;
      int r = 2 * Y_ - 1 + ky;
      if (!p.adj) { if (r < 0) r = -r; if (r >= Hf) r = 2 * Hf - 2 - r; }
      else r = min(max(r, 0), Hf - 1);
      const unsigned ro = (unsigned)(r * Wd);
      const unsigned oa = (ro + (unsigned)d0c) * 4u, ow = (ro + (unsigned)dw) * 4u;
      v4u ta;
      wrap_t tw;
      asm volatile("global_load_dwordx4 %0, %1, %2" : "=v"(ta) : "v"(oa), "s"(img) : "memory");
      if (CP == 2) asm volatile("global_load_dword %0, %1, %2" : "=v"(tw) : "v"(ow), "s"(img) : "memory");
      else asm volatile("global_load_dwordx2 %0, %1, %2" : "=v"(tw) : "v"(ow), "s"(img) : "memory");
      pa[I][s] = ta;
      pw[I][s] = tw;
    }
    const float* rsp = rs_src + ((p.dbias && p.rowscale) ? b_ : 0);
    float trs;
    asm volatile("global_load_dword %0, %1, %2" : "=v"(trs) : "v"(zero_off), "s"(rsp) : "memory");
    prs[I] = trs;
    if (MB == 2) {
      const char* mb = (const char*)p.mask_in + (out_base(xt_, Y_, b_) >> 3);
      const unsigned om = (unsigned)(lr * 8);
      v2u tm;
      asm volatile("global_load_dwordx2 %0, %1, %2" : "=v"(tm) : "v"(om), "s"(mb) : "memory");
      pm[I] = tm;
    }
  };
  auto advance = [&](int& xt_, int& Y_, int& b_) __attribute__((always_inline)) {
    if (++xt_ == tiles_x) { xt_ = 0; if (++Y_ == p.Hc) { Y_ = 0; ++b_; } }
  };
  prs[0] = prs[1] = 1.f;
  pm[0] = pm[1] = v2u{0u, 0u};
#pragma unroll
  for (int s = 0; s < NS; ++s) { pa[0][s] = pa[1][s] = v4u{0u, 0u, 0u, 0u}; pw[0][s] = pw[1][s] = wrap_t{}; }
  int xt2 = xt, Y2 = Y, b2 = b;
  if (tcnt > 0) prefetch(xt2, Y2, b2, std::integral_constant<int, 0>{});
  advance(xt2, Y2, b2);
  if (tcnt > 1) prefetch(xt2, Y2, b2, std::integral_constant<int, 1>{});
  advance(xt2, Y2, b2);
  float c_pos = p.scale * SQRT2, c_neg = p.scale * (LRELU_SLOPE * SQRT2);
  asm volatile("" : "+v"(c_pos), "+v"(c_neg));
  const float c_lin = p.epi == EPI_LRELU ? c_pos : p.scale;
  const float slope = p.epi == EPI_LRELU ? LRELU_SLOPE : 1.f;
  unsigned char* my_w = my + lr * 144 + lh * 8;
  unsigned char* my_r = my + (lane >> 3) * 144 + (lane & 7) * 16;
  auto tile = [&](auto buf_tag, const int ti) __attribute__((always_inline)) {
    constexpr int I = decltype(buf_tag)::value;
    const bool more = ti + 2 < tcnt;
#define S2_WAIT(n) asm volatile("s_waitcnt vmcnt(%0)" ::"n"(n) : "memory")
    if (ti >= 2) { if (ti + 1 < tcnt) S2_WAIT(2 * NSTO + NF); else S2_WAIT(2 * NSTO); }
    else if (ti == 1) { if (tcnt > 2) S2_WAIT(NSTO + NF); else S2_WAIT(NSTO); }
    else { if (tcnt > 1) S2_WAIT(NF); else S2_WAIT(0); }
#undef S2_WAIT
    v4u a_cur[NS];
    wrap_t w_cur[NS];
#pragma unroll
    for (int s = 0; s < NS; ++s) {
      v4u ta = pa[I][s];
      wrap_t tw = pw[I][s];
      asm volatile("" : "+v"(ta), "+v"(tw));
      a_cur[s] = ta; w_cur[s] = tw;
    }
    float rs = prs[I];
    v2u mword = pm[I];
    asm volatile("" : "+v"(rs), "+v"(mword));
    if (!(p.dbias && p.rowscale)) rs = 1.f;
    if (xt == 0 || xt == tiles_x - 1) {
      const bool lo = xt == 0 && lr == 0 && (CP == 2 || lh == 0);
      const bool hi = xt == tiles_x - 1 && lr == 31 && (CP == 2 || lh == 1);
#pragma unroll
      for (int s = 0; s < NS; ++s) {
        const v4u a = a_cur[s];
        if constexpr (CP == 2) {
          const unsigned w = w_cur[s];
          if (lo) a_cur[s] = v4u{w, a.x, a.y, a.z};
          if (hi) a_cur[s] = v4u{a.y, a.z, a.w, w};
        } else {
          const v2u w = w_cur[s];
          if (lo) a_cur[s] = v4u{w.x, w.y, a.x, a.y};
          if (hi) a_cur[s] = v4u{a.z, a.w, w.x, w.y};
        }
      }
    }
    if (p.adj && (Y == 0 || Y == p.Hc - 1)) {
#pragma unroll
      for (int s = 0; s < NS; ++s) {
        const int ky = CP == 2 ? 2 * s + lh : s;
        const int r = 2 * Y - 1 + ky;
        if (r < 0 || r >= Hf) a_cur[s] = v4u{0u, 0u, 0u, 0u};
      }
    }
    int nxt = xt, nY = Y, nb = b;
    advance(nxt, nY, nb);
    const long obase = out_base(xt, Y, b);
    uint2 araw[(MB != 2) ? 8 : 1];
    if (MB == 0 && p.epi == EPI_MASK) {
#pragma unroll
      for (int q = 0; q < 8; ++q)
        araw[MB != 2 ? q : 0] = *(const uint2*)((const bf16*)p.aux + obase + lr * 64 + (q >> 2) * 32 + (q & 3) * 8 + lh * 4);
    }
    const int X = xt * 32 + lr;
    auto window = [&](int r, int c0) -> uint4 { return window_of(b, r, c0); };
    tw_f32x16 acc[2];
#pragma unroll
    for (int jt = 0; jt < 2; ++jt)
#pragma unroll
      for (int g = 0; g < 4; ++g) {
        const float4 b4 = *(const float4*)&s_binit[jt * 32 + g * 8 + lh * 4];
        acc[jt][4 * g] = b4.x; acc[jt][4 * g + 1] = b4.y; acc[jt][4 * g + 2] = b4.z; acc[jt][4 * g + 3] = b4.w;
      }
#pragma unroll
    for (int s = 0; s < NS; ++s) {
      const tw_bf16x8 fa = __builtin_bit_cast(tw_bf16x8, a_cur[s]);
#pragma unroll
      for (int jt = 0; jt < 2; ++jt) acc[jt] = __builtin_amdgcn_mfma_f32_32x32x16_bf16(fb[s][jt], fa, acc[jt], 0, 0, 0);
    }
    if (more) prefetch(xt2, Y2, b2, buf_tag);
    advance(xt2, Y2, b2);
    if (p.adj && CP == 2 && (Y == 1 || Y == p.Hc - 2)) {
      const int c0 = 2 * X - 1;
      if (Y == 1) {
        uint4 a = make_uint4(0, 0, 0, 0);
        if (lh == 0) a = window(0, c0);
        const tw_bf16x8 fa = __builtin_bit_cast(tw_bf16x8, a);
#pragma unroll
        for (int jt = 0; jt < 2; ++jt) acc[jt] = __builtin_amdgcn_mfma_f32_32x32x16_bf16(fbx[jt], fa, acc[jt], 0, 0, 0);
      }
      if (Y == p.Hc - 2) {
        uint4 a = make_uint4(0, 0, 0, 0);
        if (lh == 0) a = window(Hf - 1, c0);
        const tw_bf16x8 fa = __builtin_bit_cast(tw_bf16x8, a);
#pragma unroll
        for (int jt = 0; jt < 2; ++jt) acc[jt] = __builtin_amdgcn_mfma_f32_32x32x16_bf16(fb[0][jt], fa, acc[jt], 0, 0, 0);
      }
    }
    if (p.adj && CP == 4 && (Y == 1 || Y == p.Hc - 2)) {
      const int c0 = 2 * X - 1 + 2 * lh;
      if (Y == 1) {
        const tw_bf16x8 fa = __builtin_bit_cast(tw_bf16x8, window(0, c0));
#pragma unroll
        for (int jt = 0; jt < 2; ++jt) acc[jt] = __builtin_amdgcn_mfma_f32_32x32x16_bf16(fb[NS - 1][jt], fa, acc[jt], 0, 0, 0);
      }
      if (Y == p.Hc - 2) {
        const tw_bf16x8 fa = __builtin_bit_cast(tw_bf16x8, window(Hf - 1, c0));
#pragma unroll
        for (int jt = 0; jt < 2; ++jt) acc[jt] = __builtin_amdgcn_mfma_f32_32x32x16_bf16(fb[0][jt], fa, acc[jt], 0, 0, 0);
      }
    }
    const unsigned msh0 = mword.x >> (4 * lh), msh1 = mword.y >> (4 * lh);
    auto phase1 = [&](auto form_tag) __attribute__((always_inline)) {
      constexpr int FORM = decltype(form_tag)::value;
#pragma unroll
      for (int jt = 0; jt < 2; ++jt)
#pragma unroll
        for (int g = 0; g < 4; ++g) {
          float v[4];
#pragma unroll
          for (int r = 0; r < 4; ++r) {
            const float a = acc[jt][4 * g + r];
            if (FORM == 1) {
              int sel;
// ... 29 lines not shown
        unsigned tb[4];
#pragma unroll
        for (int e = 0; e < 4; ++e)
          asm("v_pk_max_i16 %0, %1, 0\n\tv_pk_min_u16 %0, %0, 1 op_sel_hi:[1,0]" : "=&v"(tb[e]) : "v"(w4[e]));
        const unsigned mm = tb[0] | (tb[1] << 2) | (tb[2] << 4) | (tb[3] << 6);
        ((unsigned char*)p.mask_out)[(obase >> 3) + lane + 64 * u] = (unsigned char)((mm & 0x55u) | ((mm >> 15) & 0xAAu));
      }
      if (p.dbias) {
        const bf16* v = (const bf16*)&raw;
#pragma unroll
        for (int e = 0; e < 8; ++e) csum[e] += rs * (float)v[e];
      }
      *(uint4*)(otile + u * 1024) = raw;
    }
    xt = nxt; Y = nY; b = nb;
  };
  for (int ti = 0; ti < tcnt; ti += 2) {
    tile(std::integral_constant<int, 0>{}, ti);
    if (ti + 1 < tcnt) tile(std::integral_constant<int, 1>{}, ti + 1);
  }
  if (p.dbias) {
#pragma unroll
    for (int e = 0; e < 8; ++e) {
      float v = csum[e];
      for (int d = 8; d < 64; d <<= 1) v += __shfl_xor(v, d, 64);
      if (lane < 8) s_dbw[tid >> 6][lane * 8 + e] = v;
    }
    __syncthreads();
    if (tid < 64) s_db[tid] = (s_dbw[0][tid] + s_dbw[1][tid]) + (s_dbw[2][tid] + s_dbw[3][tid]);
    if (tid < 64) {
      if (p.dbias_part) {
        p.dbias_part[(long)blockIdx.x * 64 + tid] = s_db[tid];
      } else if (p.dbias_ws && gridDim.x > DG_DBIAS_SLOTS) {
        const int slot = blockIdx.x % DG_DBIAS_SLOTS;
        const unsigned mine = (gridDim.x - slot + DG_DBIAS_SLOTS - 1) / DG_DBIAS_SLOTS;
        float* w = p.dbias_ws + slot * DG_DBIAS_SLOT_FLOATS;
        atomicAdd(&w[tid], s_db[tid]);
        if (dg_wave_ticket_last(dg_dbias_slot_ticket(w), mine)) atomicAdd(&p.dbias[tid % p.bias_mod], atomicExch(&w[tid], 0.f));
      } else {
        atomicAdd(&p.dbias[tid % p.bias_mod], s_db[tid]);
      }
    }
  }
}

int dg_conv_s2_mfma_supported(const ConvP* p) {
  if (p->mode != MODE_S2 || !p->ring || p->nscale) return 0;
  if (p->in_dtype != DG_BF16 || p->out_dtype != DG_BF16 || p->w_dtype != DG_BF16) return 0;
  if (p->N != 64 || p->K > 4 || p->Wc % 32 != 0 || p->Hc < 4) return 0;
  const int cp = p->in_sp;
  if ((cp != 2 && cp != 4) || p->K > cp || p->in_sk != 1 || p->w_sk != 1 || p->out_sn != 1 || p->out_sp != 64) return 0;
  if (p->dbias && p->bias_mod != 64) return 0;
  if (p->bias && p->scale == 0.f) return 0;
  if (p->out_sb % 64 != 0) return 0;
  return 1;
}

#ifndef S2_CAP
#define S2_CAP 768
#endif
int dg_conv_s2_mfma_blocks(const ConvP* p) {
  if (!dg_conv_s2_mfma_supported(p)) return 0;
  const long ntiles = (long)p->B * p->Hc * (p->Wc / 32);
  const long blocks = (ntiles + 3) / 4;
  return (int)(blocks > S2_CAP ? S2_CAP : blocks);
}

int dg_conv_s2_mfma_launch(const ConvP* p, hipStream_t s) {
  if (!dg_conv_s2_mfma_supported(p)) return DG_EUNSUPPORTED;
  const int tiles_x = p->Wc / 32;
  const long ntiles = (long)p->B * p->Hc * tiles_x;
  long blocks = (ntiles + 3) / 4;
  const long cap = S2_CAP;
  if (blocks > cap) blocks = cap;
  const int mb = (p->epi == EPI_LRELU && p->mask_out) ? 1 : ((p->epi == EPI_MASK && p->mask_in) ? 2 : 0);
#define DG_S2_LAUNCH(CP_, MB_) thin_s2_mfma_kernel<CP_, MB_><<<(unsigned)blocks, 256, 0, s>>>(*p, tiles_x, ntiles)
  if (p->in_sp == 2) { if (mb == 1) DG_S2_LAUNCH(2, 1); else if (mb == 2) DG_S2_LAUNCH(2, 2); else DG_S2_LAUNCH(2, 0); }
  else { if (mb == 1) DG_S2_LAUNCH(4, 1); else if (mb == 2) DG_S2_LAUNCH(4, 2); else DG_S2_LAUNCH(4, 0); }
#undef DG_S2_LAUNCH
  HIP_CHECK_RET(hipGetLastError());
  return DG_OK;
}
```

dusty_gan_amd/csrc/pointwise.hip:

```cpp
#include "pointwise.h"

template <typename T>
__global__ __launch_bounds__(256) void final_fwd_kernel(const T* __restrict__ d4, const float* __restrict__ wf,
                                                        const float* __restrict__ bias, float scale, long n,
                                                        float* __restrict__ y, const DgDet det) {
  __shared__ float red[16];
  constexpr int V = Vec16<T>::V;
  const int b = blockIdx.y;
  const T* row = d4 + (long)b * n;
  float acc = 0.f;
  for (long i = ((long)blockIdx.x * blockDim.x + threadIdx.x) * V; i < n; i += (long)gridDim.x * blockDim.x * V) {
    float a[V];
    Vec16<T>::load(row + i, a);
#pragma unroll
    for (int k = 0; k < V; k += 4) {
      const float4 w4 = *(const float4*)(wf + i + k);
      acc += a[k] * w4.x + a[k + 1] * w4.y + a[k + 2] * w4.z + a[k + 3] * w4.w;
    }
  }
  const float s = dg_block_sum(acc, red);
  if (threadIdx.x == 0) dg_acc_add(&y[b], s * scale + ((bias && blockIdx.x == 0) ? bias[0] : 0.f), gridDim.x, det);
}
template <typename T>
__global__ __launch_bounds__(256) void final_fwd_scalar_kernel(const T* __restrict__ d4, const float* __restrict__ wf,
// ... 266 lines not shown
                                                            const float* __restrict__ y_fake, int B, float w_gan, int r1,
                                                            float* __restrict__ dy, float* __restrict__ up,
                                                            float* __restrict__ rs, float* __restrict__ acc,
                                                            float* __restrict__ dfinal_b, const T* __restrict__ d4,
                                                            const float* __restrict__ wf, float scale, long n, int C,
                                                            T* __restrict__ dd4, float* __restrict__ dbias,
                                                            float* __restrict__ dwf, float* __restrict__ dbias_part) {
  constexpr int V = Vec16<T>::V;
  constexpr int NW = 8;
  __shared__ float part[NW][64 * V];
  __shared__ float s_dy[256], s_u[256], s_r[256], red[17];
  const int ns = mode_g ? B : 2 * B;
  gan_step_body(fm, mode_g, y_real, y_fake, B, w_gan, s_dy, r1 ? s_u : nullptr, r1 ? s_r : nullptr, blockIdx.x == 0, acc,
                dfinal_b, red);
  __syncthreads();
  if (blockIdx.x == 0)
    for (int b = threadIdx.x; b < ns; b += 64 * NW) {
      dy[b] = s_dy[b];
      if (up && r1) up[b] = s_u[b];
      if (rs && r1) rs[b] = s_r[b];
    }
  if (!r1) {
    for (int b = threadIdx.x; b < ns; b += 64 * NW) { s_u[b] = s_dy[b]; s_r[b] = 1.f; }
    __syncthreads();
  }
  const int wave = threadIdx.x >> 6, lane = threadIdx.x & 63;
  const long i = ((long)blockIdx.x * 64 + lane) * V;
  float w[V], db[V], dw[V];
#pragma unroll
  for (int k = 0; k < V; ++k) { w[k] = 0.f; db[k] = 0.f; dw[k] = 0.f; }
  if (i < n) {
#pragma unroll
    for (int k4 = 0; k4 < V; k4 += 4) {
      const float4 r = *(const float4*)(wf + i + k4);
      w[k4] = r.x * scale; w[k4 + 1] = r.y * scale; w[k4 + 2] = r.z * scale; w[k4 + 3] = r.w * scale;
    }
    constexpr int NB = 8;
    for (int b0 = wave; b0 < ns; b0 += NW * NB) {
      float a[NB][V];
#pragma unroll
      for (int j = 0; j < NB; ++j) {
        const int b = b0 + NW * j;
        if (b < ns) Vec16<T>::load(d4 + (long)b * n + i, a[j]);
        else {
#pragma unroll
          for (int k = 0; k < V; ++k) a[j][k] = 0.f;
        }
      }
#pragma unroll
      for (int j = 0; j < NB; ++j) {
        const int b = b0 + NW * j;
        if (b < ns) {
          float g[V];
          const float u = s_u[b], rsb = s_r[b], c = s_dy[b];
#pragma unroll
          for (int k = 0; k < V; ++k) {
            g[k] = u * w[k] * (a[j][k] > 0.f ? SQRT2 : LRELU_SLOPE * SQRT2);
            db[k] += rsb * g[k];
            dw[k] += c * a[j][k];
          }
          Vec16<T>::store(dd4 + (long)b * n + i, g);
        }
      }
    }
  }
  if (dbias) {
#pragma unroll
    for (int k = 0; k < V; ++k) part[wave][lane * V + k] = db[k];
    __syncthreads();
    for (int e = threadIdx.x; e < 64 * V; e += 64 * NW) {
      const long ie = (long)blockIdx.x * 64 * V + e;
      if (ie < n) {
        float v = part[0][e];
#pragma unroll
        for (int w8 = 1; w8 < NW; ++w8) v += part[w8][e];
        if (dbias_part) dbias_part[ie] = v; else atomicAdd(&dbias[ie % C], v);
      }
    }
  }
  if (dwf) {
    __syncthreads();
#pragma unroll
    for (int k = 0; k < V; ++k) part[wave][lane * V + k] = dw[k];
    __syncthreads();
    for (int e = threadIdx.x; e < 64 * V; e += 64 * NW) {
      const long ie = (long)blockIdx.x * 64 * V + e;
      if (ie < n) {
        float v = part[0][e];
#pragma unroll
        for (int w8 = 1; w8 < NW; ++w8) v += part[w8][e];
        dwf[ie] += v * scale;
      }
    }
  }
}

__global__ __launch_bounds__(256) void mean_acc_kernel(const float* __restrict__ x, int n, float* __restrict__ acc) {
  __shared__ float red[16];
  float s = 0.f;
  for (int i = threadIdx.x; i < n; i += blockDim.x) s += x[i];
  const float t = dg_block_sum(s, red);
  if (threadIdx.x == 0) acc[0] += t / n;
}

__global__ void scale_kernel(const float* __restrict__ x, float a, long n, float* __restrict__ y) {
  const long i = (long)blockIdx.x * blockDim.x + threadIdx.x;
  if (i < n) y[i] = a * x[i];
// ... 106 lines not shown
    if (dtype == DG_BF16) batch_wsum_kernel<bf16><<<grid, 256, 0, s>>>((const bf16*)src, coef, scale, B, n, out);
    else batch_wsum_kernel<float><<<grid, 256, 0, s>>>((const float*)src, coef, scale, B, n, out);
  } else if (dtype == DG_BF16) {
    batch_wsum_scalar_kernel<bf16><<<nblk(n), 256, 0, s>>>((const bf16*)src, coef, scale, B, n, out);
  } else {
    batch_wsum_scalar_kernel<float><<<nblk(n), 256, 0, s>>>((const float*)src, coef, scale, B, n, out);
  }
  HIP_CHECK_RET(hipGetLastError());
  return DG_OK;
}

int dg_scale(const float* x, float a, long n, float* y, void* s_) {
  hipStream_t s = (hipStream_t)s_;
  scale_kernel<<<nblk(n), 256, 0, s>>>(x, a, n, y);
  HIP_CHECK_RET(hipGetLastError());
  return DG_OK;
}

int dg_gan_d_step(int metric, float smoothing, const float* y_real, const float* y_fake, int B, float w_gan,
                  float* dy, float* up, float* rs, float* acc, float* dfinal_b, void* s_) {
  if (!y_real || !y_fake || !dy || !acc || B <= 0) return DG_EINVAL;
  GanForm fm;
  const int rc = gan_form(metric, 0, smoothing, &fm);
  if (rc != DG_OK) return rc;
  gan_step_kernel<<<1, 256, 0, (hipStream_t)s_>>>(fm, 0, y_real, y_fake, B, w_gan, dy, up, rs, acc, dfinal_b);
  HIP_CHECK_RET(hipGetLastError());
  return DG_OK;
}

int dg_gan_g_step(int metric, const float* y_real, const float* y_fake, int B, float w_gan, float* dy, float* acc,
                  void* s_) {
  if (!y_fake || !dy || !acc || B <= 0) return DG_EINVAL;
  GanForm fm;
  const int rc = gan_form(metric, 1, 1.f, &fm);
  if (rc != DG_OK) return rc;
  if (fm.kr != PHI_NONE && !y_real) return DG_EINVAL;
  gan_step_kernel<<<1, 256, 0, (hipStream_t)s_>>>(fm, 1, y_real, y_fake, B, w_gan, dy, nullptr, nullptr, acc,
                                                  nullptr);
  HIP_CHECK_RET(hipGetLastError());
  return DG_OK;
}

int dg_final_gan_bwd(int metric, int mode_g, float smoothing, const float* y_real, const float* y_fake, int B, float w_gan,
                     int r1, float* dy, float* up, float* rs, float* acc, float* dfinal_b, const void* d4, int dtype,
                     const float* wf, float scale, long n, int C, void* dd4, float* dbias, float* dwf, float* dbias_part,
                     void* s_) {
  if (!y_fake || !dy || !acc || !d4 || !wf || !dd4 || B <= 0 || n <= 0) return DG_EINVAL;
  if (dbias_part && (!dbias || n % C != 0)) return DG_EINVAL;
  if (!mode_g && !y_real) return DG_EINVAL;
  GanForm fm;
  const int rc = gan_form(metric, mode_g ? 1 : 0, mode_g ? 1.f : smoothing, &fm);
  if (rc != DG_OK) return rc;
  if (mode_g && fm.kr != PHI_NONE && !y_real) return DG_EINVAL;
  if (mode_g && r1) return DG_EINVAL;
  const int ns = mode_g ? B : 2 * B;
  const int V = dtype == DG_BF16 ? 8 : 4;
  if (!(vec_ok(d4, n, dtype) && vec_ok(dd4, n, dtype) && C % V == 0 && ns <= 256 && ((size_t)wf & 15) == 0 &&
        (!dwf || ((size_t)dwf & 15) == 0)))
    return DG_EUNSUPPORTED;
  const unsigned grid = nblk(n / V, 64);
  hipStream_t s = (hipStream_t)s_;
  if (dtype == DG_BF16)
    final_gan_bwd_kernel<bf16><<<grid, 512, 0, s>>>(fm, mode_g ? 1 : 0, y_real, y_fake, B, w_gan, r1, dy, up, rs, acc, dfinal_b,
                                                    (const bf16*)d4, wf, scale, n, C, (bf16*)dd4, dbias, dwf, dbias_part);
  else
    final_gan_bwd_kernel<float><<<grid, 512, 0, s>>>(fm, mode_g ? 1 : 0, y_real, y_fake, B, w_gan, r1, dy, up, rs, acc, dfinal_b,
                                                     (const float*)d4, wf, scale, n, C, (float*)dd4, dbias, dwf, dbias_part);
  HIP_CHECK_RET(hipGetLastError());
  return DG_OK;
}

int dg_pl_penalty(const float* dz, int B, int K, float w, float* pl_ema, float* v, float* acc, void* s_) {
  if (!dz || !pl_ema || !v || !acc || B <= 0 || B > 256 || K <= 0) return DG_EINVAL;
  pl_penalty_kernel<<<1, 256, 0, (hipStream_t)s_>>>(dz, B, K, w, pl_ema, v, acc);
  HIP_CHECK_RET(hipGetLastError());
  return DG_OK;
}

int dg_mean_acc(const float* x, int n, float* acc, void* s_) {
  if (!x || !acc || n <= 0) return DG_EINVAL;
  mean_acc_kernel<<<1, 256, 0, (hipStream_t)s_>>>(x, n, acc);
  HIP_CHECK_RET(hipGetLastError());
  return DG_OK;
}

}

#define DG_DET_MAX_DEVICES 64
static DgDet g_det_table[DG_DET_MAX_DEVICES];
DgDet dg_det_current() {
  int dev = 0;
  if (hipGetDevice(&dev) != hipSuccess || dev < 0 || dev >= DG_DET_MAX_DEVICES) return DgDet{nullptr, nullptr, 0};
  return g_det_table[dev];
}
extern "C" int dg_det_arena(float* arena, long n, void* shadow) {
  if ((arena == nullptr) != (shadow == nullptr) || n < 0) return DG_EINVAL;
  if (shadow && ((size_t)shadow & 15) != 0) return DG_EINVAL;
  int dev = 0;
  HIP_CHECK_RET(hipGetDevice(&dev));
  if (dev < 0 || dev >= DG_DET_MAX_DEVICES) return DG_EINVAL;
  g_det_table[dev] = DgDet{arena, (unsigned long long*)shadow, arena ? n : 0};
  return DG_OK;
}
```

dusty_gan_amd/csrc/wgrad_mfma_dma.hip:

```cpp
#include "common.h"

#include <stdlib.h>

#include <type_traits>

#ifndef DG_WG_BM_MAX
#define DG_WG_BM_MAX 128
#endif
#ifndef DG_WG_BN_MAX
#define DG_WG_BN_MAX 128
#endif

namespace {

typedef __attribute__((ext_vector_type(8))) __bf16 bf16x8;
typedef __attribute__((ext_vector_type(2))) int i32x2;
typedef __attribute__((ext_vector_type(4))) int i32x4;
typedef __attribute__((ext_vector_type(16))) float f32x16;
typedef __attribute__((ext_vector_type(4))) float f32x4;

constexpr int BKP = 64;
constexpr int NS = 2;
constexpr int PAIR_MIN_WS = 24;

// ... 38 lines not shown
  const long units = (long)p.B * p.Hc;
  const long u0 = units * bz / gz, u1 = units * (bz + 1) / gz;
  const int cpr = p.Wc / BKP;
  const long nchunks64 = (u1 - u0) * cpr;
  const int Wa = WMODE == 0 ? 2 * p.Wc : p.Wc;
  const int Wg = WMODE == 1 ? 2 * p.Wc : p.Wc;
  const bf16* A = (const bf16*)p.a;
  const bf16* G = (const bf16*)p.g;
  const int wave = __builtin_amdgcn_readfirstlane(tid >> 6), lane = tid & 63;
  const int asp = (int)p.a_sp, gsp = (int)p.g_sp;

  constexpr int CA = RA / 16, CG = RG / 16;
  constexpr int RPA = 64 / CA, RPG = 64 / CG;
  auto swz = [](int row, int rowbytes) { return rowbytes == 256 ? (row & 3) : ((row >> 1) & 1); };
  int rowA[PA], rowG[PG];
  unsigned chA[PA], chG[PG];
  auto chunk_off = [](int c) { return (unsigned)(X2 ? (c >> 3) * 256 + (c & 7) * 16 : c * 16); };
#pragma unroll
  for (int v = 0; v < PA; ++v) {
    const int r = (wave + 4 * v) * RPA + lane / CA, c = lane % CA;
    rowA[v] = r;
    chA[v] = chunk_off((((c >> 2) ^ swz(r, RA)) << 2) | (c & 3));
  }
#pragma unroll
  for (int v = 0; v < PG; ++v) {
    const int r = (wave + 4 * v) * RPG + lane / CG, c = lane % CG;
    rowG[v] = r;
    chG[v] = chunk_off((((c >> 2) ^ swz(r, RG)) << 2) | (c & 3));
  }
  const int rowX = BKP + lane / CA;
  const unsigned chX = chunk_off(((((lane % CA) >> 2) ^ swz(rowX, RA)) << 2) | (lane % CA & 3));
  const unsigned aspb = (unsigned)asp * 2u, gspb = (unsigned)gsp * 2u;
  const int da = NT == 2 ? (WMODE == 0 ? kxp - 1 : -kxp)
                         : (WMODE == 0 ? kxp - 1 : (kxp == 0 ? 1 : (kxp == 3 ? -1 : 0)));
  const int kx_s0 = NT == 2 ? (WMODE == 0 ? kxp : kxp + 2) : kxp, kx_s1 = WMODE == 0 ? kxp + 2 : kxp;
  const int dg = WMODE == 1 ? (NT == 2 ? 1 - kxp : ((kxp == 0 || kxp == 2) ? 1 : 0)) : 0;
  const unsigned lds0 = (unsigned)(size_t)(__attribute__((address_space(3))) unsigned char*)lds;
  auto dma_s = [&](unsigned voff, const char* sbase, unsigned ldsaddr) __attribute__((always_inline)) {
    if (wg_dbg & 1) return;
    asm volatile("s_mov_b32 m0, %0\n\ts_nop 0\n\tglobal_load_lds_dwordx4 %1, %2" ::"s"(ldsaddr), "v"(voff), "s"(sbase) : "memory");
  };
  const int nchunks = (int)nchunks64;
  int ib = (int)(u0 / p.Hc), im = (int)(u0 % p.Hc), ixc = 0;
  const char* abase = nullptr;
  const char* gbase = nullptr;
  auto set_unit = [&](int b, int m) __attribute__((always_inline)) {
    int rowa, rowg;
    dg_wgrad1d(WMODE, 0, m, p.Hc, ky, rowa, rowg);
    auto uni = [](const bf16* q) __attribute__((always_inline)) {
      const unsigned long long v = (unsigned long long)q;
      const unsigned lo = __builtin_amdgcn_readfirstlane((unsigned)v), hi = __builtin_amdgcn_readfirstlane((unsigned)(v >> 32));
      return (const char*)(((unsigned long long)hi << 32) | lo);
    };
    const int bg = p.g_mod > 0 ? b % p.g_mod : b;
    abase = uni(A + (long)b * p.a_sb + (long)rowa * Wa * asp + ci0 * (X2 ? 2 : 1));
    gbase = uni(G + (long)bg * p.g_sb + (long)rowg * Wg * gsp + co0 * (X2 ? 2 : 1));
  };
  set_unit(ib, im);
  int iseg = 0;
  auto issue = [&](unsigned st_off) __attribute__((always_inline)) {
    const unsigned base = lds0 + st_off + (unsigned)wave * 1024u;
    const int x0 = ixc * BKP;
    const char* ab = abase + ((X2 && iseg == 1) ? 128 : 0);
    const char* gb = gbase + ((X2 && iseg == 2) ? 128 : 0);
#pragma unroll
    for (int v = 0; v < PA; ++v) {
      const unsigned ca = (unsigned)(((WMODE == 0 ? 2 : 1) * (x0 + rowA[v]) + da) & (Wa - 1));
      dma_s(__umul24(ca, aspb) + chA[v], ab, base + 4 * v * 1024);
    }
    if (NT == 2 && wave == 0) {
      const unsigned ca = (unsigned)(((WMODE == 0 ? 2 : 1) * (x0 + rowX) + da) & (Wa - 1));
      dma_s(__umul24(ca, aspb) + chX, ab, lds0 + st_off + 4 * PA * 1024);
    }
#pragma unroll
    for (int v = 0; v < PG; ++v) {
      const unsigned cg = (unsigned)((WMODE == 1 ? 2 : 1) * (x0 + rowG[v]) + dg);
      dma_s(__umul24(cg, gspb) + chG[v], gb, base + STA + 4 * v * 1024);
    }
    if (X2 && ++iseg < 3) return;
    iseg = 0;
    if (++ixc == cpr) {
      ixc = 0;
      if (++im == p.Hc) { im = 0; ++ib; }
      set_unit(ib, im);
    }
  };

  const int wm = wave >> 1, wn = wave & 1;
  const int lr = lane & 31, lh = lane >> 5;
  const int g16 = lane >> 4, i16 = lane & 15;
  const int kh = g16 >> 1, cb = g16 & 1, q = i16 >> 2, pp = i16 & 3;
  unsigned offA[NT][TM], offG[TN];
#pragma unroll
  for (int t = 0; t < NT; ++t)
#pragma unroll
    for (int i = 0; i < TM; ++i) {
      const int colb = (wm * (BM / 2) + i * 32 + 16 * cb + 4 * pp) * 2;
      offA[t][i] = lds0 + (8 * kh + q + t) * RA + ((((colb >> 6) ^ swz(q + t, RA)) << 6) | (colb & 63));
    }
#pragma unroll
  for (int j = 0; j < TN; ++j) {
    const int colb = (wn * (BN / 2) + j * 32 + 16 * cb + 4 * pp) * 2;
    offG[j] = lds0 + STA + (8 * kh + q) * RG + ((((colb >> 6) ^ swz(q, RG)) << 6) | (colb & 63));
  }

  f32x16 acc[NT][TM][TN];
#pragma unroll
// ... 235 lines not shown
        for (int j = 0; j < 8; ++j) acc += v[j];
      }
      for (; sp < it.splits; sp += 16) acc += __builtin_nontemporal_load(src + (long)sp * stride);
    }
    s_part[sg][el] = acc;
    __syncthreads();
    if (sg == 0 && 4 * i4 < it.numel) {
      f32x4 t = s_part[0][el];
#pragma unroll
      for (int j = 1; j < 16; ++j) t += s_part[j][el];
      f32x4* dst = (f32x4*)it.dw + i4;
      if (it.accumulate) t += *dst;
      *dst = t;
    }
    return;
  }
  const long i4 = (long)(blockIdx.x - r.first_block[k]) * 256 + threadIdx.x;
  if (4 * i4 >= it.numel) return;
  const f32x4* src = (const f32x4*)it.ws + i4;
  const long stride = it.numel / 4;
  f32x4 acc = {0.f, 0.f, 0.f, 0.f};
  int s = 0;
  for (; s + 8 <= it.splits; s += 8) {
    f32x4 v[8];
#pragma unroll
    for (int j = 0; j < 8; ++j) v[j] = __builtin_nontemporal_load(src + (long)(s + j) * stride);
#pragma unroll
    for (int j = 0; j < 8; ++j) acc += v[j];
  }
  for (; s < it.splits; ++s) acc += __builtin_nontemporal_load(src + (long)s * stride);
  f32x4* dst = (f32x4*)it.dw + i4;
  if (it.accumulate) acc += *dst;
  *dst = acc;
}

}

int dg_wgrad_mfma_dma_supported(const WgradP* p) {
  const bool x2 = p->a_dtype == DG_BF16X2;
  if (p->a_dtype != p->g_dtype || (p->a_dtype != DG_BF16 && !x2)) return 0;
  if (x2 && (p->a_sp % 64 || p->g_sp % 64 || p->a_sb % 64 || p->g_sb % 64 || (((size_t)p->a | (size_t)p->g) & 255))) return 0;
  if (p->wmode != 0 && p->wmode != 1) return 0;
  if (!p->ring || p->a_sc != 1 || p->g_sc != 1) return 0;
  if (p->Ci % 64 != 0 || p->Co % 64 != 0 || p->Wc % BKP != 0 || p->Hc < 2) return 0;
  if (p->a_sp % 8 != 0 || p->g_sp % 8 != 0) return 0;
  if ((p->Wc & (p->Wc - 1)) != 0) return 0;
  if (p->a_sp * (x2 ? 4 : 2) >= (1 << 24) || p->g_sp * (x2 ? 4 : 2) >= (1 << 24)) return 0;
  if ((long)p->B * p->Hc * (p->Wc / BKP) > 0x7fffffffL) return 0;
  return 1;
}

int dg_wgrad_mfma_dma_launch(const WgradP* p, int accumulate, int pairs, hipStream_t stream, DgWgradPlan* plan) {
  if (!dg_wgrad_mfma_dma_supported(p)) return DG_EUNSUPPORTED;
  if (p->g_mod < 0 || (p->ws && ((size_t)p->ws & 15) != 0)) return DG_EINVAL;
  const bool m128 = p->Ci % 128 == 0, n128 = p->Co % 128 == 0;
  if (p->wmode == 0) {
    if (m128 && n128) return launch_dma<0, 128, 128>(p, accumulate, pairs, stream, plan);
    if (m128) return launch_dma<0, 128, 64>(p, accumulate, pairs, stream, plan);
    if (n128) return launch_dma<0, 64, 128>(p, accumulate, pairs, stream, plan);
    return launch_dma<0, 64, 64>(p, accumulate, pairs, stream, plan);
  }
  if (m128 && n128) return launch_dma<1, 128, 128>(p, accumulate, pairs, stream, plan);
  if (m128) return launch_dma<1, 128, 64>(p, accumulate, pairs, stream, plan);
  if (n128) return launch_dma<1, 64, 128>(p, accumulate, pairs, stream, plan);
  return launch_dma<1, 64, 64>(p, accumulate, pairs, stream, plan);
}

int dg_wgrad_mfma_dma_group_launch(const WgradP* items, int n, int pairs, int rounds, hipStream_t stream, DgWgradPlan* plans) {
  if (n < 1 || n > GROUP_MAX) return DG_EINVAL;
  GroupP g{};
  int blocks = 0;
  double fl[GROUP_MAX], fsum = 0.0;
  for (int i = 0; i < n; ++i) {
    fl[i] = (double)items[i].B * items[i].Hc * items[i].Wc * items[i].Ci * items[i].Co;
    fsum += fl[i];
  }
  for (int i = 0; i < n; ++i) {
    const WgradP* p = &items[i];
    if (!dg_wgrad_mfma_dma_supported(p) || (!plans && !p->ws)) return DG_EUNSUPPORTED;
    if (p->g_mod < 0 || (!plans && ((size_t)p->ws & 15) != 0)) return DG_EINVAL;
    long target = 512;
    if (rounds > 0) {
      target = (long)(rounds * 512.0 * fl[i] / fsum + 0.5);
      if (target < 64) target = 64;
    }
    const int bm = (p->Ci % 128 == 0 && DG_WG_BM_MAX >= 128) ? 128 : 64, bn = (p->Co % 128 == 0 && DG_WG_BN_MAX >= 128) ? 128 : 64;
    const DmaGeo ge = bm == 128 ? (bn == 128 ? dma_geo<128, 128>(p, 1, pairs, true, target) : dma_geo<128, 64>(p, 1, pairs, true, target))
                                : (bn == 128 ? dma_geo<64, 128>(p, 1, pairs, true, target) : dma_geo<64, 64>(p, 1, pairs, true, target));
    if (plans) {
      plans[i].variant = DG_WGRAD_VARIANT_DMA;
      plans[i].splits = (int)ge.split;
      plans[i].ws_floats = ge.split * 16L * p->Ci * p->Co;
      plans[i].tap_pairs = ge.use_pairs ? 1 : 0;
      continue;
    }
    GroupItem& it = g.it[i];
    it.p = x2_strides(*p);
    it.tiles_n = ge.tiles_n;
    it.gx = ge.tiles_m * ge.tiles_n; it.gy = ge.use_pairs ? 8 : 16; it.gz = (int)ge.split;
    it.first = blocks;
    it.variant = variant_code(p->wmode, bm, bn, ge.use_pairs ? 2 : 1, p->a_dtype == DG_BF16X2);
    it.accumulate = 1;
    blocks += (it.gx * it.gy * it.gz + 7) / 8 * 8;
  }
  if (plans) return DG_OK;
  g.n = n;
  wgrad_group_kernel<<<(unsigned)blocks, 256, 0, stream>>>(g);
  HIP_CHECK_RET(hipGetLastError());
  return DG_OK;
}

extern "C" int dg_wgrad_reduce(const DgWgradReduce* items, int n, void* stream) {
  if (!items || n < 1 || n > RED_MAX) return DG_EINVAL;
  ReduceItems r{};
  int blocks = 0;
  int order[RED_MAX];
  for (int i = 0; i < n; ++i) order[i] = i;
  for (int i = 1; i < n; ++i)
    for (int j = i; j > 0 && items[order[j]].splits > items[order[j - 1]].splits; --j) {
      const int t = order[j]; order[j] = order[j - 1]; order[j - 1] = t;
    }
  for (int i = 0; i < n; ++i) {
    const DgWgradReduce& it = items[order[i]];
    if (!it.ws || !it.dw || it.numel <= 0 || it.numel % 4 != 0 || it.splits < 1) return DG_EINVAL;
    if (((size_t)it.ws & 15) != 0 || ((size_t)it.dw & 15) != 0) return DG_EINVAL;
    r.it[i] = it;
    r.first_block[i] = blocks;
    blocks += (int)((it.numel / 4 + (it.splits > RED_WIDE ? 15 : 255)) / (it.splits > RED_WIDE ? 16 : 256));
  }
  r.first_block[n] = blocks;
  r.n = n;
  wgrad_reduce_kernel<<<(unsigned)blocks, 256, 0, (hipStream_t)stream>>>(r);
  HIP_CHECK_RET(hipGetLastError());
// ... 3 lines not shown
```

dusty_gan_amd/engine.py:

```python
import ctypes as C
import math
import os
import warnings
from collections import OrderedDict

import torch

from . import _lib as L

ARCH_ID = {"none": 0, "dusty1": 1, "dusty2": 2}

PROFILE = None
TRACE = None


def _align(n, a=64):
    return (n + a - 1) // a * a


class Segment:
    __slots__ = ("name", "off", "shape", "numel", "kind")

    def __init__(self, name, off, shape, kind):
        self.name, self.off, self.shape, self.kind = name, off, tuple(shape), kind
# ... 451 lines not shown
    def __enter__(self):
        self.outer = self.ops._group is not None
        if not self.outer:
            self.ops._group = []
            self.ws = WGRAD_WS._cur()
            self.ws.pre_reduce = self._issue_now
        return self

    def _issue_now(self):
        items, self.ops._group = self.ops._group, []
        self.ops._launch_group(items)

    def __exit__(self, et, ev, tb):
        if self.outer:
            return False
        items, self.ops._group = self.ops._group, None
        self.ws.pre_reduce = None
        if et is None:
            self.ops._launch_group(items)
        return False


class Ops:
    group_enabled = os.environ.get("DUSTY_GAN_WGRAD_GROUP", "1") != "0"
    group_rounds = 0
    default_wg_cap = 0
    _dbias_ws = {}

    def __init__(self, dtype, x3=False):
        self.lib = L.lib()
        self.dtype = dtype
        self.x3 = bool(x3) and dtype == torch.float32
        self.dt = L.dtype_code(dtype)
        self.es = _es(self.dt)
        self.force = L.DG_FORCE_AUTO
        self.wg_cap = Ops.default_wg_cap
        self.use_ws = True
        self._group = None
        self._x2_scratch = {}

    def _f32_copy(self, role, t):
        key = (role, t.numel(), str(t.device))
        b = self._x2_scratch.get(key)
        if b is None:
            b = self._x2_scratch[key] = torch.empty(t.numel(), dtype=torch.float32, device=t.device)
        return b

    @property
    def _f(self):
        return self.force | (L.DG_FORCE_FP32X3 if self.x3 else 0)

    def conv(self, mode, adj, ring, B, Hc, Wc, K, N, x, x_strides, out, out_strides, w_ptr, scale, epi,
             bias=None, bias_mod=0, aux=None, dbias=None, rowscale=None, in_dt=None, out_dt=None, nscale=None,
             x_off=0, out_off=0, aux_off=0, w_strides=None, w_dt=None, up_frag=None, defer_db=False, tanh_sums=None):
        x2_out = None
        if mode == L.MODE_GEMM and (is_x2(x) or is_x2(out) or is_x2(aux)):
            if is_x2(x):
                x = x2_unpack(x, self._f32_copy("x", x), x_off, B * K)
            if is_x2(aux):
                aux = x2_unpack(aux, self._f32_copy("aux", aux), aux_off, B * N)
            if is_x2(out):
                x2_out, out = out, self._f32_copy("out", out)
        if is_x2(x):
            in_dt = L.DG_BF16X2
        if is_x2(out):
            out_dt = L.DG_BF16X2
            assert aux is None or is_x2(aux), "DG_EPI_MASK: aux has out's layout and dtype"
        if in_dt == L.DG_BF16X2 and out_dt == L.DG_BF16X2 and w_strides is None:
            tw = X2_TWIN.get(int(w_ptr))
            if tw is None:
                raise L.DgError("no DG_BF16X2 twin registered for this weight shadow (ParamStore.enable_x2)")
            w_ptr, w_dt = tw, L.DG_BF16X2
        p = L.DgConv()
        p.mode, p.adj, p.ring = mode, adj, int(ring)
        p.B, p.Hc, p.Wc, p.K, p.N = B, Hc, Wc, K, N
        in_dt = self.dt if in_dt is None else in_dt
        out_dt = self.dt if out_dt is None else out_dt
        ies, oes = _es(in_dt), _es(out_dt)
        p.in_ = L.ptr(x) + ies * x_off
        p.in_sb, p.in_sp, p.in_sk = x_strides
        p.out = L.ptr(out) + oes * out_off
        p.out_sb, p.out_sp, p.out_sn = out_strides
        p.w = w_ptr
        if w_strides is None:
            p.w_st, p.w_sn, p.w_sk = N * K, K, 1
        else:
            p.w_st, p.w_sk, p.w_sn = w_strides
        p.scale, p.epi = scale, epi
        p.bias, p.bias_mod = bias, bias_mod
        p.aux = None if aux is None else L.ptr(aux) + oes * aux_off
        p.dbias, p.rowscale = dbias, L.ptr(rowscale)
        p.in_dtype, p.out_dtype, p.w_dtype = in_dt, out_dt, (self.dt if w_dt is None else w_dt)
        p.nscale = L.ptr(nscale)
        p.up_frag = up_frag
        sum_parts = 0
        if tanh_sums is not None:
            p.tanh_sum_parts = L.ptr(tanh_sums)
            pl = self._conv_plan(p)
            sum_parts = pl.sum_parts if B * pl.sum_parts <= tanh_sums.numel() else 0
            if not sum_parts:
                p.tanh_sum_parts = None
        if epi == L.EPI_LRELU and out_dt == L.DG_BF16:
            p.mask_out = MaskBits.slice_ptr(out, out_off, N, out_strides)
        elif epi == L.EPI_MASK and aux is not None and out_dt == L.DG_BF16:
            p.mask_in = MaskBits.slice_ptr(aux, aux_off, N, out_strides)
        if dbias is not None:
            ws = Ops._dbias_ws.get(str(x.device))
            if ws is None:
                ws = Ops._dbias_ws[str(x.device)] = torch.zeros(L.DBIAS_WS_FLOATS, dtype=torch.float32, device=x.device)
            p.dbias_ws = L.ptr(ws)
        final = None

        def plan():
            nonlocal final
            if final is None:
                final = self._conv_plan(p)
            return final
        db_rows = 0
        if dbias is not None and DETERMINISTIC:
            pl = plan()
            if pl.dbias_rows > 0:
                part = WGRAD_WS.take(pl.dbias_rows * N, x.device)
                if part is not None:
                    db_rows, p.dbias_part = pl.dbias_rows, part
        if TRACE is not None:
            pl = plan()
            TRACE.append(("conv", pl.family, pl.bm, pl.bn, pl.tiles, pl.workgroups, pl.tiles_per_wg, _conv_tag(p), pl.thin_mfma,
                          (1 if p.mask_out else 0) | (pl.mask_bits & 2 if p.mask_in else 0)))

        def record():
            pl = plan()
            names = {L.DG_CONV_FAMILY_THIN: "conv_thin_kernel", L.DG_CONV_FAMILY_DIRECT: "conv_direct_kernel"}
            mb = 0
            if p.mask_out or p.mask_in:
                mb = pl.mask_bits if p.mask_in else 1
            cost = conv_algorithmic(mode, B, Hc, Wc, K, N, ies, oes, _es(p.w_dtype), epi == L.EPI_MASK, mb)
            return (names.get(pl.family, "conv_mfma_kernel"),) + cost + (_conv_tag(p),)
        _launch(lambda: self.lib.dg_conv_ex(C.byref(p), self._f, self.wg_cap, L.stream_ptr()), "dg_conv_ex", record)
        self._db_rows_done(p, db_rows, dbias, N, defer_db)
        if x2_out is not None:
            x2_pack(out, x2_out, out_off, B * N)
        return sum_parts

    def _conv_plan(self, p):
        pl = L.DgConvPlan()
        L.check(self.lib.dg_conv_plan(C.byref(p), self._f, self.wg_cap, C.byref(pl)), "dg_conv_plan")
        return pl

    def _db_rows_done(self, p, rows, dbias, N, defer_db):
        if rows:
            WGRAD_WS.add(p.dbias_part, dbias, N, rows, 1)
            if not defer_db:
                WGRAD_WS.flush()

    def wgrad_plan(self, p, accumulate=1):
        pl = L.DgWgradPlan()
        L.check(self.lib.dg_wgrad_plan(C.byref(p), accumulate, self._f, C.byref(pl)), "dg_wgrad_plan")
        return pl

    def wgrad(self, wmode, ring, B, Hc, Wc, Ci, Co, a, a_strides, g, g_strides, dw_ptr, scale, rowscale=None,
              accumulate=1, a_dt=None, g_dt=None, a_off=0, g_off=0, g_mod=0, defer=False):
        p = self._wgrad_params(wmode, ring, B, Hc, Wc, Ci, Co, a, a_strides, g, g_strides, dw_ptr, scale, rowscale, a_dt,
                               g_dt, a_off, g_off, g_mod)
        pl = self.wgrad_plan(p, accumulate) if self.use_ws else None
        if (self._group is not None and defer and pl is not None and pl.ws_floats > 0 and pl.variant == L.DG_WGRAD_VARIANT_DMA
                and len(self._group) < self.GROUP_MAX and pl.ws_floats <= WgradWorkspace.FLOATS):
            self._group.append((p, (a, g, rowscale), dw_ptr, int(accumulate)))
            return
        if pl is not None and pl.ws_floats > 0:
            p.ws = WGRAD_WS.take(pl.ws_floats, a.device)
        if TRACE is not None:
            TRACE.append(("wgrad", self.lib.dg_wgrad_kernel_variant(C.byref(p), self._f), _wgrad_tag(p),
                          0 if pl is None else pl.splits, 0 if pl is None else pl.tap_pairs, bool(p.ws), g_mod))
        self._wgrad_launch(p, accumulate)
        if p.ws:
            WGRAD_WS.add(p.ws, dw_ptr, (1 if wmode == 2 else 16) * Ci * Co, pl.splits, int(accumulate))
            if not defer:
                WGRAD_WS.flush()

    def _wgrad_launch(self, p, accumulate):
        def record():
            v = self.lib.dg_wgrad_kernel_variant(C.byref(p), self._f)
            name = {L.DG_WGRAD_VARIANT_THIN: "wgrad_thin_kernel", L.DG_WGRAD_VARIANT_THIN_MFMA: "wgrad_thin_kernel",
                    L.DG_WGRAD_VARIANT_DIRECT: "wgrad_direct_kernel"}.get(v, "wgrad_mfma_kernel")
            return (name,) + _wgrad_cost(p) + (_wgrad_tag(p),)
        _launch(lambda: self.lib.dg_wgrad(C.byref(p), accumulate, self._f, L.stream_ptr()), "dg_wgrad", record)

    GROUP_MAX = 4

    def grouped(self):
        return _WgradGroup(self)

    def _launch_group(self, items):
        if not items:
            return
        if len(items) > 1:
            need = []
            for it in items:
                pl = self.wgrad_plan(it[0], 1)
                need.append((pl.ws_floats + 63) // 64 * 64)
            if sum(need) > WgradWorkspace.FLOATS:
                piece, tot = [], 0
                for it, nf in zip(items, need):
                    if piece and tot + nf > WgradWorkspace.FLOATS:
                        self._launch_group(piece)
                        piece, tot = [], 0
                    piece.append(it)
                    tot += nf
                if len(piece) < len(items):
                    self._launch_group(piece)
                    return
        n = len(items)
        arr = (L.DgWgrad * n)()
        for i, it in enumerate(items):
            C.memmove(C.byref(arr, i * C.sizeof(L.DgWgrad)), C.byref(it[0]), C.sizeof(L.DgWgrad))
        plans = (L.DgWgradPlan * n)()
        grouped = n > 1 and Ops.group_enabled
        if grouped:
            L.check(self.lib.dg_wgrad_group_plan(arr, n, self._f, Ops.group_rounds, plans), "dg_wgrad_group_plan")
        else:
            for i in range(n):
                L.check(self.lib.dg_wgrad_plan(C.byref(arr[i]), 1, self._f, C.byref(plans[i])), "dg_wgrad_plan")
        sizes = [(plans[i].ws_floats + 63) // 64 * 64 for i in range(n)]
        base = WGRAD_WS.take(sum(sizes), items[0][1][0].device)
        if base is None:
            for it in items:
                L.check(self.lib.dg_wgrad(C.byref(it[0]), it[3], self._f, L.stream_ptr()), "dg_wgrad")
            return
        off = 0
        for i in range(n):
            arr[i].ws = base + 4 * off
            off += sizes[i]
        descs = [_wgrad_tag(it[0]) for it in items]
        if TRACE is not None:
            for i, it in enumerate(items):
                TRACE.append(("wgrad", L.DG_WGRAD_VARIANT_DMA, descs[i], plans[i].splits, plans[i].tap_pairs, True, it[0].g_mod))
            if grouped:
                TRACE.append(("wgrad_group", n, descs))
        if grouped:
            def record():
                fb = [_wgrad_cost(it[0]) for it in items]
                return "wgrad_mfma_kernel", sum(f for f, _ in fb), sum(b for _, b in fb), f"group of {n} layers"
            _launch(lambda: self.lib.dg_wgrad_group(arr, n, self._f, Ops.group_rounds, L.stream_ptr()), "dg_wgrad_group", record)
        else:
            for i in range(n):
                self._wgrad_launch(arr[i], 1)
        for i, it in enumerate(items):
            WGRAD_WS.add(arr[i].ws, it[2], 16 * it[0].Ci * it[0].Co, plans[i].splits, it[3])

    def wgrad_takes_map(self, wmode, ring, B, Hc, Wc, Ci, Co, a, a_strides, g, g_strides, dw_ptr):
        p = self._wgrad_params(wmode, ring, B, Hc, Wc, Ci, Co, a, a_strides, g, g_strides, dw_ptr, 1.0, None, None, None,
                               0, 0, 0)
        return self.lib.dg_wgrad_has_sample_map(C.byref(p), self._f) == 1

    def _wgrad_params(self, wmode, ring, B, Hc, Wc, Ci, Co, a, a_strides, g, g_strides, dw_ptr, scale, rowscale, a_dt, g_dt,
                      a_off, g_off, g_mod):
        if wmode == 2:
            if is_x2(a):
                a = x2_unpack(a, self._f32_copy("wa", a))
            if is_x2(g):
                g = x2_unpack(g, self._f32_copy("wg", g))
        if is_x2(a):
            a_dt = L.DG_BF16X2
        if is_x2(g):
            g_dt = L.DG_BF16X2
        p = L.DgWgrad()
        p.wmode, p.ring = wmode, int(ring)
        p.B, p.Hc, p.Wc, p.Ci, p.Co = B, Hc, Wc, Ci, Co
        a_dt = self.dt if a_dt is None else a_dt
        g_dt = self.dt if g_dt is None else g_dt
        p.a = L.ptr(a) + _es(a_dt) * a_off
        p.a_sb, p.a_sp, p.a_sc = a_strides
        p.g = L.ptr(g) + _es(g_dt) * g_off
        p.g_sb, p.g_sp, p.g_sc = g_strides
        p.dw, p.scale, p.rowscale = dw_ptr, scale, L.ptr(rowscale)
        p.a_dtype, p.g_dtype = a_dt, g_dt
        p.ws, p.g_mod = None, int(g_mod)
        return p


def x2_eligible(cfg):
    return bool(cfg.ring and all(c % 64 == 0 for c in cfg.ch) and (cfg.W & (cfg.W - 1)) == 0 and cfg.w0 >= 64)


class GEngine:
    head_tanh_fused = os.environ.get("DUSTY_GAN_HEAD_TANH", "1") != "0"

    def __init__(self, cfg: NetCfg, dtype, x3=False, x2=False):
        self.cfg, self.dtype = cfg, dtype
        self.ops = Ops(dtype, x3=x3)
        self.x2_asked = bool(x2)
        self.x2 = self.x2_asked and self.ops.x3 and x2_eligible(cfg)
        self.ws_B = 0
        self.chs = [cfg.ch[3], cfg.ch[2], cfg.ch[1], cfg.ch[0]]
        self.ta = None
        self._dzT = None

    def alloc(self, B, device):
        if self.ws_B == B and self.a[0].device == device:
            return
        c = self.cfg
        T = self.dtype
        hw = [(c.h0 << i, c.w0 << i) for i in range(5)]
        chs = self.chs
        self.grid = hw
        self.a = [torch.empty(B * hw[i][0] * hw[i][1] * chs[i], dtype=T, device=device) for i in range(4)]
        self.dp = [torch.empty_like(t) for t in self.a]
        if self.x2:
            for t in self.a + self.dp:
                tag_x2(t)
        self.abits = [MaskBits.register(self.a[3])]
        HW = c.H * c.W
        self.gout = torch.empty(B, c.nheads, c.H, c.W, dtype=torch.float32, device=device)
        self.draw = torch.empty_like(self.gout)
        self.cp = 2 if c.nheads <= 2 else 4
        self.draw_pm = (torch.empty(B, c.H, c.W, self.cp, dtype=torch.bfloat16, device=device)
                        if (T == torch.bfloat16 and c.nheads <= 4 and c.ring) else None)
        self.hp_ws = torch.zeros(B * 1024, dtype=torch.float32, device=device)
        self.mask = torch.empty(B, max(c.nheads - 1, 1), c.H, c.W, dtype=torch.float32, device=device)
        self.depth = torch.empty(B, 1, c.H, c.W, dtype=torch.float32, device=device)
        self.dsum_parts = torch.empty(B * 256, dtype=torch.float32, device=device)
        self.zT = torch.empty(B * c.nz, dtype=T, device=device)
        self.noise_pixel = None
        self.noise_image = None
        k = c.nheads - 1
        s_depth = 1.0 / math.sqrt(1 * 16)
        s_conf = 1.0 / math.sqrt(k * 16) if k else 0.0
        self.head_scales = (s_depth, s_conf)
        self.nscale = torch.tensor([s_depth] + [s_conf] * k, dtype=torch.float32, device=device)
        self.HW = HW
# ... 223 lines not shown
        B, sp = S.B, L.stream_ptr()
        out = self.forward(st, S.latent, S.gumbel, training=False, z_ready=True, want_sums=False)
        pm = self.draw_pm is not None
        C = S.chamfer
        nterm = len(S.terms) + (C is not None)
        for i, code in enumerate(S.terms):
            fn, what = (lib.dg_inv_loss_grad, "dg_inv_loss_grad") if i == 0 else (lib.dg_inv_loss_grad_add, "dg_inv_loss_grad_add")
            draw = L.ptr(self.draw) if (nterm > 1 or not pm) else None
            draw_pm = L.ptr(self.draw_pm) if i == nterm - 1 else None
            L.check(fn(L.ptr(self.gout), c.nheads * self.HW, 1, L.ptr(S.ref), L.ptr(S.mask), L.ptr(S.msum), code, B, self.HW,
                       self.head_scales[0], draw, c.nheads, draw_pm, self.cp, L.ptr(S.parts), L.ptr(S.tickets), S.nchunk,
                       L.ptr(S.loss), sp), what)
        if C is not None:
            HW, arch = self.HW, ARCH_ID[c.arch]
            depth = out["depth"]
            L.check(lib.dg_inv_to_xyz(L.ptr(depth), L.ptr(C.angle), B, c.H, c.W, 1, C.min_depth, C.max_depth, 0.0, C.tol, None,
                                      L.ptr(C.P), sp), "dg_inv_to_xyz")
            cloud = (3 * HW, 1, HW, HW)
            L.check(lib.dg_chamfer_nn(L.ptr(C.R), *cloud, L.ptr(C.P), *cloud, B, L.ptr(C.d1), L.ptr(C.idx1), sp), "dg_chamfer_nn")
            L.check(lib.dg_chamfer_nn(L.ptr(C.P), *cloud, L.ptr(C.R), *cloud, B, L.ptr(C.d2), L.ptr(C.idx2), sp), "dg_chamfer_nn")
            L.check(lib.dg_inv_chamfer_scatter(L.ptr(C.R), L.ptr(C.idx1), B, HW, L.ptr(C.acc), sp), "dg_inv_chamfer_scatter")
            add = int(nterm > 1)
            L.check(lib.dg_inv_chamfer_grad(L.ptr(C.P), L.ptr(C.R), L.ptr(C.d1), L.ptr(C.d2), L.ptr(C.idx2), L.ptr(C.acc),
                                            L.ptr(depth), L.ptr(C.angle), L.ptr(self.gout),
                                            L.ptr(self.noise_pixel) if arch else None, L.ptr(self.mask) if arch else None, arch,
                                            c.tau, c.drop_const, C.min_depth, C.max_depth, C.tol, B, HW, *self.head_scales, add,
                                            L.ptr(self.draw) if (add or not pm) else None, c.nheads, L.ptr(self.draw_pm), self.cp,
                                            L.ptr(S.parts), L.ptr(S.tickets), S.nchunk, L.ptr(S.loss), sp), "dg_inv_chamfer_grad")
        self._backward_chain(st, None, self.draw, self.draw_pm, self.dp, acts=None, chain=None, second_of=None,
                             head_ready=True)
        dzT = self.grad_z_T(st)
        S.optimizer_launch(dzT, self.zT, L.dtype_code(self.dtype))
        return out


class AugGrad:

    def __init__(self, A, gy, rp, gsum, args, keep):
        self.A, self.gy, self.rp, self.gsum, self.args, self.keep = A, gy, rp, gsum, args, keep
        self.shape = gy.shape

    def materialize(self):
        return self.A.backward_pre(self.gy, self.rp, self.gsum)


class DEngine:

    def __init__(self, cfg: NetCfg, dtype, x3=False, x2=False):
        self.cfg, self.dtype = cfg, dtype
        self.ops = Ops(dtype, x3=x3)
        self.x2_asked = bool(x2)
        self.x2 = self.x2_asked and self.ops.x3 and x2_eligible(cfg)
        self.ws_B = 0

    def alloc(self, nb, device):
        if self.ws_B >= nb and self.h[0].device == device:
            return
        c, T = self.cfg, self.dtype
        self.grid = [(c.H >> i, c.W >> i) for i in range(5)]
        self.chs = [2, c.ch[0], c.ch[1], c.ch[2], c.ch[3]]
        self.per = [self.grid[i][0] * self.grid[i][1] * self.chs[i] for i in range(5)]
        self.h = [torch.empty(nb * self.per[i], dtype=T, device=device) for i in range(5)]
        self.e = [torch.empty(nb * self.per[i], dtype=T, device=device) for i in range(5)]
        self.hbits = [MaskBits.register(t) for t in self.h[1:4]]
        self.h4f = self.e4f = None
        if self.x2:
            for t in self.h[1:] + self.e[1:]:
                tag_x2(t)
            self.h4f, self.e4f = torch.empty_like(self.h[4]), torch.empty_like(self.e[4])
        self.y = torch.empty(nb, dtype=torch.float32, device=device)
        self.ws_B = nb

    def forward(self, st, x, slot, tangent_of=None, mean=None):
        c, o, lib = self.cfg, self.ops, L.lib()
        n = x.shape[0]
        dst = L.ptr(self.h[0]) + o.es * slot * self.per[0]
        if mean is not None:
            rc = lib.dg_blur_fwd_mean(L.ptr(x), dst, o.dt, n, c.H, c.W, int(c.ring), L.ptr(mean[0]), int(mean[1]), mean[2],
                                      L.stream_ptr())
            if rc == L.DG_EUNSUPPORTED:
                L.check(lib.dg_mean_acc(L.ptr(mean[0]), int(mean[1]), mean[2], L.stream_ptr()), "dg_mean_acc")
                mean = None
            else:
                L.check(rc, "dg_blur_fwd_mean")
        if mean is None:
            L.check(lib.dg_blur_fwd(L.ptr(x), dst, o.dt, n, c.H, c.W, int(c.ring), L.stream_ptr()), "dg_blur_fwd")
        return self._layers(st, n, slot, tangent_of)

    def forward_aug(self, st, A, sources, slot):
        c, o, lib = self.cfg, self.ops, L.lib()
        n = sources[0][0].shape[0]
        sets = [A.aug_set(x, rp) for x, rp in sources] if (c.W % 4 == 0 and len(sources) <= 2) else [None]
        if all(q is not None for q in sets):
            arr = (L.DgAugSet * len(sets))(*[q[0] for q in sets])
            rc = lib.dg_diffaug_blur_fwd(arr, len(sets), A.mask, n, c.H, c.W, int(c.ring),
                                         L.ptr(self.h[0]) + o.es * slot * self.per[0], o.dt, L.stream_ptr())
            if rc != L.DG_EUNSUPPORTED:
                L.check(rc, "dg_diffaug_blur_fwd")
                return self._layers(st, n * len(sets), slot, None)
        xcat = torch.empty(n * len(sources), 1, c.H, c.W, dtype=torch.float32, device=sources[0][0].device)
        for k, (x, rp) in enumerate(sources):
            A.apply(x, rp, out=xcat[k * n:(k + 1) * n])
        return self.forward(st, xcat, slot)

    def _layers(self, st, n, slot, tangent_of):
        c, o, lib = self.cfg, self.ops, L.lib()
        sp = L.stream_ptr()
        if self.x2:
            st.enable_x2()
        st.refresh_shadows(self.dtype)
        es = o.es
        for i in range(1, 5):
            hc, wc = self.grid[i]
            ci, co = self.chs[i - 1], self.chs[i]
            tang = tangent_of is not None
            o.conv(L.MODE_S2, 0, c.ring, n, hc, wc, ci, co, self.h[i - 1], (self.per[i - 1], ci, 1), self.h[i],
                   (self.per[i], co, 1), L.ptr(st.coci[f"d{i}_w"]), 1.0 / math.sqrt(ci * 16),
                   L.EPI_MASK if tang else L.EPI_LRELU, bias=None if tang else st.fptr(f"d{i}_b"), bias_mod=co,
                   aux=self.h[i] if tang else None, x_off=slot * self.per[i - 1], out_off=slot * self.per[i],
                   aux_off=(tangent_of or 0) * self.per[i])
        if tangent_of is None:
            nf = self.per[4]
            h4 = self._h4(slot, n)
            y = L.AccArena.take(n, self.y.device)
            if y is not None:
                L.check(lib.dg_final_fwd_acc(L.ptr(h4) + es * slot * nf, o.dt, st.fptr("final_w"), st.fptr("final_b"),
                                             1.0 / math.sqrt(nf), n, nf, L.ptr(y), sp), "dg_final_fwd_acc")
                return y
            L.check(lib.dg_final_fwd(L.ptr(h4) + es * slot * nf, o.dt, st.fptr("final_w"), st.fptr("final_b"),
                                     1.0 / math.sqrt(nf), n, nf, L.ptr(self.y) + 4 * slot, sp), "dg_final_fwd")
        return self.y[slot:slot + n]

    def _h4(self, slot, n):
        if not self.x2:
            return self.h[4]
        return x2_unpack(self.h[4], self.h4f, slot * self.per[4], n * self.per[4])

    def _e4(self):
        return self.e4f if self.x2 else self.e[4]

    def _e4_done(self, slot, n):
        if self.x2:
            x2_pack(self.e4f, self.e[4], slot * self.per[4], n * self.per[4])

    def _bwd_layer(self, st, i, slot, n, rowscale, want_dbias):
        c, o = self.cfg, self.ops
        hc, wc = self.grid[i]
        ci, co = self.chs[i - 1], self.chs[i]
        first = i == 1
        frag = st.up_frag("d1_w", (ci * co, co, 1), ci, hc, 1) if (first and c.ring and co == 64 and ci <= 3) else None
        o.conv(L.MODE_UP, 1, c.ring, n, hc, wc, co, ci, self.e[i], (self.per[i], co, 1), self.e[i - 1],
               (self.per[i - 1], ci, 1), st.sptr(f"d{i}_w"),
               1.0 / math.sqrt(ci * 16), L.EPI_LINEAR if first else L.EPI_MASK,
               aux=None if first else self.h[i - 1],
               dbias=(st.fptr(f"d{i - 1}_b", st.grad) if (want_dbias and not first) else None), bias_mod=ci,
               rowscale=rowscale, x_off=slot * self.per[i], out_off=slot * self.per[i - 1],
               aux_off=slot * self.per[i - 1], up_frag=frag, defer_db=True)

    def backward_data(self, st, slot, n, up, rowscale, want_dbias, skip_final=False):
        o, lib = self.ops, L.lib()
        nf = self.per[4]
        if not skip_final:
            L.check(lib.dg_final_bwd_data(L.ptr(self._h4(slot, n)) + o.es * slot * nf, o.dt, st.fptr("final_w"), L.ptr(up),
                                          L.ptr(rowscale), 1.0 / math.sqrt(nf), n, nf, self.chs[4],
                                          L.ptr(self._e4()) + o.es * slot * nf,
                                          st.fptr("d4_b", st.grad) if want_dbias else None, L.stream_ptr()),
                    "dg_final_bwd_data")
            self._e4_done(slot, n)
        for i in (4, 3, 2):
            self._bwd_layer(st, i, slot, n, rowscale, want_dbias)

    def final_gan_bwd(self, st, slot, B, metric, mode_g, smoothing, w_gan, y_real, y_fake, r1, dy, up, rs, acc_ptr,
                      want_dbias, want_wgrad):
        if PROFILE is not None:
            return False
        o, lib = self.ops, L.lib()
        nf = self.per[4]
        C4 = self.chs[4]
        part = WGRAD_WS.take(nf, self.h[4].device) if (want_dbias and DETERMINISTIC and nf % C4 == 0 and C4 % 4 == 0) else None
        nsl = B if mode_g else 2 * B
        h4 = self._h4(slot, nsl)
        rc = lib.dg_final_gan_bwd(metric, int(mode_g), float(smoothing), y_real, y_fake, B, w_gan, int(r1), L.ptr(dy),
                                  L.ptr(up), L.ptr(rs), acc_ptr,
                                  st.fptr("final_b", st.grad) if not mode_g else None,
                                  L.ptr(h4) + o.es * slot * nf, o.dt, st.fptr("final_w"), 1.0 / math.sqrt(nf), nf,
                                  C4, L.ptr(self._e4()) + o.es * slot * nf,
                                  st.fptr("d4_b", st.grad) if want_dbias else None,
                                  st.fptr("final_w", st.grad) if want_wgrad else None, part, L.stream_ptr())
        if rc == L.DG_EUNSUPPORTED:
            return False
        L.check(rc, "dg_final_gan_bwd")
        self._e4_done(slot, nsl)
        if part is not None:
            WGRAD_WS.add(part, st.fptr("d4_b", st.grad), C4, nf // C4, 1)
        return True

    def r1_fused_ok(self):
        c = self.cfg
        return c.W % 4 == 0 and (c.H * c.W) % 1024 == 0

    def backward_input(self, st, slot, n, dx, r1=None):
        c, o, lib = self.cfg, self.ops, L.lib()
        if r1 is not None and not self.r1_fused_ok():
            return False
        self._bwd_layer(st, 1, slot, n, None, False)
        if r1 is not None:
            L.check(lib.dg_blur_bwd_r1(L.ptr(self.e[0]) + o.es * slot * self.per[0], o.dt, L.ptr(dx), float(r1[0]),
                                       L.ptr(r1[1]), n, c.H, c.W, int(c.ring), L.stream_ptr()), "dg_blur_bwd_r1")
            return True
        L.check(lib.dg_blur_bwd(L.ptr(self.e[0]) + o.es * slot * self.per[0], o.dt, L.ptr(dx), n, c.H, c.W,
                                int(c.ring), L.stream_ptr()), "dg_blur_bwd")
        return True

    def r1_turnaround(self, st, slot, n, tslot, oscale, ssq, mean_ptr):
        c, o, lib = self.cfg, self.ops, L.lib()
        if c.W % 4 or c.H % 4 or 6 * c.W * 4 > 60 * 1024:
            return False
        self._bwd_layer(st, 1, slot, n, None, False)
        L.check(lib.dg_blur_r1_tangent(L.ptr(self.e[0]) + o.es * slot * self.per[0], o.dt,
                                       L.ptr(self.h[0]) + o.es * tslot * self.per[0], float(oscale), L.ptr(ssq), mean_ptr, int(n),
                                       n, c.H, c.W, int(c.ring), L.stream_ptr()), "dg_blur_r1_tangent")
        self._layers(st, n, tslot, slot)
        return True

    def backward_input_aug(self, st, slot, n, A, rp, lazy=False):
        c, o, lib = self.cfg, self.ops, L.lib()
        self._bwd_layer(st, 1, slot, n, None, False)
        dx = torch.empty(n, 1, c.H, c.W, dtype=torch.float32, device=self.e[0].device)
        gsum = L.AccArena.take(n, dx.device) if c.W % 4 == 0 else None
        if gsum is not None:
            args, keep = A._args(rp, n, dx.device)
            rc = lib.dg_blur_bwd_augsum(L.ptr(self.e[0]) + o.es * slot * self.per[0], o.dt, L.ptr(dx), args[2], args[4],
                                        args[5], A.mask, L.ptr(gsum), n, c.H, c.W, int(c.ring), L.stream_ptr())
            if rc != L.DG_EUNSUPPORTED:
                L.check(rc, "dg_blur_bwd_augsum")
                if lazy:
                    return AugGrad(A, dx, rp, gsum, args, keep)
                return A.backward_pre(dx, rp, gsum)
        L.check(lib.dg_blur_bwd(L.ptr(self.e[0]) + o.es * slot * self.per[0], o.dt, L.ptr(dx), n, c.H, c.W,
                                int(c.ring), L.stream_ptr()), "dg_blur_bwd")
        return A.backward(dx, rp)

    def wgrad(self, st, a_slot, g_slot, n, rowscale, layers=(1, 2, 3, 4), g_mod=0):
        c, o = self.cfg, self.ops
        with o.grouped():
            for i in layers:
                hc, wc = self.grid[i]
                ci, co = self.chs[i - 1], self.chs[i]
                o.wgrad(0, c.ring, n, hc, wc, ci, co, self.h[i - 1], (self.per[i - 1], ci, 1), self.e[i],
                        (self.per[i], co, 1), st.fptr(f"d{i}_w", st.grad), 1.0 / math.sqrt(ci * 16), rowscale=rowscale,
                        a_off=a_slot * self.per[i - 1], g_off=g_slot * self.per[i], g_mod=g_mod, defer=True)

    def wgrad_r1(self, st, B, rs3, layers=(1, 2, 3, 4)):
        c, o = self.cfg, self.ops
        with o.grouped():
            for i in layers:
                hc, wc = self.grid[i]
                ci, co = self.chs[i - 1], self.chs[i]
                if o.wgrad_takes_map(0, c.ring, 3 * B, hc, wc, ci, co, self.h[i - 1], (self.per[i - 1], ci, 1), self.e[i],
                                     (self.per[i], co, 1), st.fptr(f"d{i}_w", st.grad)):
                    self.wgrad(st, 0, 0, 3 * B, rs3, layers=(i,), g_mod=2 * B)
                else:
                    self.wgrad(st, 0, 0, 2 * B, rs3, layers=(i,))
                    self.wgrad(st, 2 * B, 0, B, None, layers=(i,))

    def final_wgrad_term(self, slot, n):
        nf = self.per[4]
        return (L.ptr(self.h[4]) + self.ops.es * slot * nf, self.dtype == torch.bfloat16, None, int(n), nf, 1.0 / math.sqrt(nf))

    def final_wgrad(self, st, slot, n, coef):
        o, lib = self.ops, L.lib()
        nf = self.per[4]
        L.check(lib.dg_batch_wsum(L.ptr(self._h4(slot, n)) + o.es * slot * nf, o.dt, L.ptr(coef), 1.0 / math.sqrt(nf), n,
                                  nf, st.fptr("final_w", st.grad), L.stream_ptr()), "dg_batch_wsum")
```

dusty_gan_amd/trainers/dcgan_amp.py:

```python
import math
import os
import os.path as osp
from collections import OrderedDict
from collections.abc import Mapping

import torch
import torch.distributed as dist

from .. import _lib as L
from .. import engine as E
from ..models import define_D, define_G
from ..models.loss import GANLoss
from ..utils import cycle, sigmoid_to_tanh, tanh_to_sigmoid
from ..utils.context_manager import gradient_accumulation
from ..utils import dist as D_
from ..utils.diff_augment import DiffAugment
from ..utils.lidar import LiDAR
from ..utils.rng import Philox
from ..utils.synthetic import SyntheticLiDAR


def _world():
    return dist.get_world_size() if dist.is_available() and dist.is_initialized() else 1

# ... 611 lines not shown
    def _allreduce(self, store):
        if self._multi:
            E.WGRAD_WS.flush()
            self._coll(lambda: D_.allreduce_grads(store.grad), name="all-reduce grads")
        elif self._force_seg:
            E.WGRAD_WS.flush()
            self._coll(lambda: None)
        return 1.0 / self.world

    def _allreduce_async(self, key, buf):
        E.WGRAD_WS.flush()
        if self._multi:
            self._comm_issue(key, lambda: D_.allreduce_grads(buf, async_op=True)[0])
        elif self._force_seg:
            self._coll(lambda: None)

    @_own_counters
    def optimize_D(self, reals=None, rands=None):
        lib, sp = L.lib(), L.stream_ptr()
        B = self.local_batch
        Gb, D = _backbone(self.G), self.D
        self.G.train()
        gengs = self._g_engines()
        deng = D.engine()
        deng.alloc(3 * B, self.device)
        Dst, Gst = D.store, Gb.store
        Dst.refresh_shadows(self.dtype)
        Gst.refresh_shadows(self.dtype)
        gp = float(self.loss_weight.get("gp", 0.0)) if "gp" in self.criterion else 0.0
        w_gan = float(self.loss_weight["gan"]) / self.n_acc
        self._mb = []
        extra_D = None
        dev = self.device
        if not getattr(self, "_arena_ready", False):
            self._begin_step(draw_B=B if rands is None else None)
        self._arena_ready = False
        if "D" in self._grads_zeroed:
            self._grads_zeroed.discard("D")
        else:
            self.optim_D.zero_grad()
        scal = L.AccArena.take(16, dev)[:7]
        f32 = dict(dtype=torch.float32, device=dev)
        for j in gradient_accumulation(self.n_acc, True, (self.G, self.D)):
            if reals is not None:
                x_real, m_real = reals[j]
            else:
                x_real, m_real = self.fetch_reals(self._next_batch())
            rand = self._prep_rand(rands[j] if rands is not None else None, B)
            synth = gengs[j].forward(Gst, rand["z"], rand["noise"], training=True,
                                     z_ready=bool(rand.get("z_ready")) and j == 0)
            y = deng.forward_aug(Dst, self.A, [(x_real, rand["aug"][0]), (synth["depth"], rand["aug"][1])], 0)
            dy = torch.empty(2 * B, **f32)
            up = torch.empty(2 * B, **f32) if gp > 0 else None
            rs = None
            if gp > 0:
                if getattr(self, "_rs3", None) is None or self._rs3.numel() != 3 * B or self._rs3.device != self.device:
                    self._rs3 = torch.ones(3 * B, **f32)
                rs = self._rs3
            fused = deng.final_gan_bwd(Dst, 0, B, self.gan_code, False, float(self.criterion["gan"].smoothing), w_gan,
                                       L.ptr(y), L.ptr(y) + 4 * B, gp > 0, dy, up, rs, L.ptr(scal), True, True)
            if not fused:
                L.check(lib.dg_gan_d_step(self.gan_code, float(self.criterion["gan"].smoothing), L.ptr(y),
                                          L.ptr(y) + 4 * B, B, w_gan, L.ptr(dy), L.ptr(up), L.ptr(rs), L.ptr(scal),
                                          Dst.fptr("final_b", Dst.grad), sp), "dg_gan_d_step")
            bucketed = self._bucketed()
            cut = Dst.seg["d4_w"].off
            if gp > 0:
                deng.backward_data(Dst, 0, 2 * B, up, rs, want_dbias=True, skip_final=fused)
                vscale = gp / self.n_acc / B
                ssq = L.AccArena.take(B, dev)
                if ssq is None or not deng.r1_turnaround(Dst, 0, B, 2 * B, vscale, ssq, L.ptr(scal) + 12):
                    g = torch.empty(B, 1, self.H, self.W, **f32)
                    vg = torch.empty_like(g)
                    if ssq is None or not deng.backward_input(Dst, 0, B, vg, r1=(vscale, ssq)):
                        deng.backward_input(Dst, 0, B, g)
                        if ssq is None:
                            ssq = torch.empty(B, **f32)
                            L.check(lib.dg_sample_sum(L.ptr(g), B, self.H * self.W, 1, L.ptr(ssq), sp), "dg_sample_sum")
                        else:
                            L.check(lib.dg_sample_sum_acc(L.ptr(g), B, self.H * self.W, 1, L.ptr(ssq), sp), "dg_sample_sum_acc")
                        L.check(lib.dg_scale(L.ptr(g), vscale, g.numel(), L.ptr(vg), sp), "dg_scale")
                    deng.forward(Dst, vg, 2 * B, tangent_of=0, mean=(ssq, B, L.ptr(scal) + 12))
                for layers in (((4,), (3, 2, 1)) if bucketed else ((4, 3, 2, 1),)):
                    deng.wgrad_r1(Dst, B, rs, layers=layers)
                    if 4 in layers:
                        if not fused:
                            deng.final_wgrad(Dst, 0, 2 * B, dy)
                        if (not bucketed and self.n_acc == 1 and not deng.x2 and self.optim_D.will_fuse(self.dtype)):
                            extra_D = {"final_w": deng.final_wgrad_term(2 * B, B)}
                        else:
                            deng.final_wgrad(Dst, 2 * B, B, None)
                        if bucketed:
                            self._allreduce_async("D.hi", Dst.grad[cut:])
            else:
                deng.backward_data(Dst, 0, 2 * B, dy, None, want_dbias=True, skip_final=fused)
                if not bucketed:
                    deng.wgrad(Dst, 0, 0, 2 * B, None)
                    if not fused:
                        deng.final_wgrad(Dst, 0, 2 * B, dy)
                else:
                    deng.wgrad(Dst, 0, 0, 2 * B, None, layers=(4,))
                    if not fused:
                        deng.final_wgrad(Dst, 0, 2 * B, dy)
                    self._allreduce_async("D.hi", Dst.grad[cut:])
                    deng.wgrad(Dst, 0, 0, 2 * B, None, layers=(3, 2, 1))
            self._mb.append({"x_real": x_real, "m_real": m_real, "rand": rand, "synth": synth, "geng": gengs[j]})
        if self._bucketed():
            self._allreduce_async("D.lo", Dst.grad[:Dst.seg["d4_w"].off])
            self._comm_wait("D.hi", "D.lo")
            gscale = 1.0 / self.world
        else:
            gscale = self._allreduce(Dst)
        self.optim_D.step(gscale=gscale, shadow_dtype=self.dtype, extra=extra_D, sole=self.n_acc == 1)
        self._dev_scal = scal
        return scal

    @_own_counters
    def optimize_G(self):
        lib, sp = L.lib(), L.stream_ptr()
        B = self.local_batch
        Gb, D = _backbone(self.G), self.D
        Gst, Dst = Gb.store, D.store
        pl_on = "pl" in self.criterion
        if "G" in getattr(self, "_grads_zeroed", ()):
            self._grads_zeroed.discard("G")
        else:
            self.optim_G.zero_grad(skip=("proj_w",) if self.n_acc == 1 else ())
        gather_proj = (self.world > 1 or self._force_seg) and self.n_acc == 1 and next(iter(Gst.seg)) == "proj_w"
        fuse_proj = (not gather_proj and self.world == 1 and self.n_acc == 1 and self.dtype in (torch.bfloat16, torch.float32)
                     and (self.dtype == torch.bfloat16 or self._fuse_proj_fp32)
                     and next(iter(Gst.seg)) == "proj_w" and Gst.seg["proj_w"].off == 0 and self._fuse_proj_ok
                     and self.optim_G.betas[0] == 0.0 and E.PROFILE is None)
        fuse_gathered = (gather_proj and self.dtype == torch.bfloat16 and Gst.seg["proj_w"].off == 0
                         and self._fuse_proj_ok and self.optim_G.betas[0] == 0.0 and E.PROFILE is None)
        if not (fuse_proj or fuse_gathered):
            self.optim_G.regen_grad = None
        deng = D.engine()
        w_gan = float(self.loss_weight["gan"]) / self.n_acc
        f32 = dict(dtype=torch.float32, device=self.device)
# ... 480 lines not shown
```

include/dusty_gan_hip.h:

```cpp
#ifndef DUSTY_GAN_HIP_H
#define DUSTY_GAN_HIP_H
#include <stdint.h>

#ifdef __cplusplus
extern "C" {
#endif

#define DG_OK 0
#define DG_EINVAL 1
#define DG_EUNSUPPORTED 2
#define DG_EHIP 3

#define DG_F32 0
#define DG_BF16 1
#define DG_BF16X2 2

#define DG_MODE_S2 0
#define DG_MODE_UP 1
#define DG_MODE_GEMM 2

#define DG_EPI_LINEAR 0
#define DG_EPI_LRELU 1
#define DG_EPI_MASK 2

typedef struct DgConv {
  int mode, adj, ring;
  int B, Hc, Wc;
  int K, N;
  const void* in;
  long in_sb, in_sp, in_sk;
  void* out;
  long out_sb, out_sp, out_sn;
  const void* w;
  long w_st, w_sk, w_sn;
  float scale;
  int epi;
  const float* bias;
  int bias_mod;
  const void* aux;
  float* dbias;
  const float* rowscale;
  int in_dtype, out_dtype, w_dtype;
  const float* nscale;
  const void* up_frag;
  float* dbias_ws;
  float* dbias_part;
  void* mask_out;
  const void* mask_in;
  float* tanh_sum_parts;
} DgConv;
#define DG_UP_FRAG_BYTES (3 * 18 * 1024)
#define DG_DBIAS_SLOTS 32
#define DG_DBIAS_SLOT_FLOATS 1024

typedef struct DgWgrad {
  int wmode, ring;
  int B, Hc, Wc;
  int Ci, Co;
  const void* a;
  long a_sb, a_sp, a_sc;
  const void* g;
  long g_sb, g_sp, g_sc;
  float* dw;
  float scale;
  const float* rowscale;
  int a_dtype, g_dtype;
  float* ws;
  int g_mod;
} DgWgrad;

int dg_conv(const DgConv* p, int force, void* stream);
#define DG_FORCE_AUTO 0
#define DG_FORCE_DIRECT 1
#define DG_FORCE_MFMA 2
#define DG_FORCE_THIN 3
#define DG_FORCE_LOCKSTEP 4
#define DG_FORCE_PINGPONG 5
#define DG_FORCE_WG_REGSTAGED 6
#define DG_FORCE_WG_DMA_PAIRS 7
#define DG_FORCE_WG_DMA_NOPAIRS 8
#define DG_FORCE_PINGPONG_SINGLE 9
#define DG_FORCE_PROJ_STREAM 10
#define DG_FORCE_FP32X3 0x100
#define DG_CONV_FAMILY_DIRECT 1
#define DG_CONV_FAMILY_MFMA 2
#define DG_CONV_FAMILY_THIN 3
#define DG_CONV_FAMILY_LOCKSTEP 4
#define DG_CONV_FAMILY_PINGPONG 5
#define DG_CONV_FAMILY_PROJ_STREAM 6
typedef struct DgConvPlan {
  int family;
  int bm, bn;
  int tiles;
  int workgroups;
  int tiles_per_wg;
  int thin_mfma;
  int mask_bits;
  int dbias_rows;
  int sum_parts;
} DgConvPlan;
int dg_conv_ex(const DgConv* p, int force, int wg_cap, void* stream);
int dg_conv_plan(const DgConv* p, int force, int wg_cap, DgConvPlan* plan);
int dg_conv_mfma_supported(const DgConv* p);

int dg_wgrad(const DgWgrad* p, int accumulate, int force, void* stream);
#define DG_WGRAD_VARIANT_DIRECT 1
#define DG_WGRAD_VARIANT_MFMA 2
#define DG_WGRAD_VARIANT_THIN 3
#define DG_WGRAD_VARIANT_DMA 5
#define DG_WGRAD_VARIANT_THIN_MFMA 7
typedef struct DgWgradPlan {
  int variant;
  int splits;
  long ws_floats;
  int tap_pairs;
} DgWgradPlan;
int dg_wgrad_plan(const DgWgrad* p, int accumulate, int force, DgWgradPlan* plan);
int dg_wgrad_group(const DgWgrad* items, int n, int force, int rounds, void* stream);
int dg_wgrad_group_plan(const DgWgrad* items, int n, int force, int rounds, DgWgradPlan* plans);
typedef struct DgWgradReduce {
  const float* ws;
  float* dw;
  long numel;
  int splits;
  int accumulate;
} DgWgradReduce;
int dg_wgrad_reduce(const DgWgradReduce* items, int n, void* stream);
int dg_wgrad_mfma_supported(const DgWgrad* p);
int dg_wgrad_kernel_variant(const DgWgrad* p, int force);
int dg_wgrad_has_sample_map(const DgWgrad* p, int force);

int dg_blur_fwd(const float* x, void* out, int dtype, int B, int H, int W, int ring, void* stream);
int dg_blur_fwd_mean(const float* x, void* out, int dtype, int B, int H, int W, int ring, const float* mean_src, int mean_n,
                     float* mean_acc, void* stream);
int dg_blur_bwd(const void* d, int dtype, float* dx, int B, int H, int W, int ring, void* stream);
int dg_blur_bwd_r1(const void* d, int dtype, float* dx, float oscale, float* ssq, int B, int H, int W, int ring, void* stream);
int dg_blur_r1_tangent(const void* d, int dtype, void* out, float oscale, float* ssq, float* mean_acc, int mean_n, int B, int H,
                       int W, int ring, void* stream);

int dg_final_fwd(const void* d4, int dtype, const float* wf, const float* bias, float scale, int B, long n, float* y,
                 void* stream);
int dg_final_fwd_acc(const void* d4, int dtype, const float* wf, const float* bias, float scale, int B, long n, float* y,
                 void* stream);
int dg_final_bwd_data(const void* d4, int dtype, const float* wf, const float* up, const float* rowscale, float scale,
                      int B, long n, int C, void* dd4, float* dbias, void* stream);
int dg_batch_wsum(const void* src, int dtype, const float* coef, float scale, int B, long n, float* out, void* stream);

int dg_head_post_fwd(float* gout, const float* noise_pixel, const float* noise_image, int arch, int training,
                     float tau, float drop_const, int B, long HW, float* mask, float* depth, void* stream);
int dg_head_post_fwd_sum(float* gout, const float* noise_pixel, const float* noise_image, int arch, int training,
                         float tau, float drop_const, int B, long HW, float* mask, float* depth, float* dsum, void* stream);
int dg_head_post_bwd(const float* gout, const float* noise_pixel, const float* noise_image, const float* mask,
                     const float* ddepth, int arch, float tau, float drop_const, int B, long HW, float s_depth,
                     float s_conf, float* draw, float* dbias, void* draw_pm , int cp,
                     float* bias_ws, void* stream);
int dg_logistic_noise(const float* u1, const float* u2, float eps, long n, float* out, void* stream);

int dg_diffaug_fwd(const float* x, const float* u_b, const float* u_c, const int* t_h, const int* t_w, const int* o_x,
                   const int* o_y, int policy, int B, int H, int W, float* xsum_ws, float* y, void* stream);
int dg_diffaug_fwd_acc(const float* x, const float* u_b, const float* u_c, const int* t_h, const int* t_w, const int* o_x,
                   const int* o_y, int policy, int B, int H, int W, float* xsum_ws, float* y, void* stream);
int dg_diffaug_fwd_pre(const float* x, const float* u_b, const float* u_c, const int* t_h, const int* t_w, const int* o_x,
                       const int* o_y, int policy, int B, int H, int W, const float* xsum, float* y, void* stream);
int dg_diffaug_bwd(const float* gy, const float* u_b, const float* u_c, const int* t_h, const int* t_w, const int* o_x,
                   const int* o_y, int policy, int B, int H, int W, float* gsum_ws, float* gx, void* stream);
int dg_diffaug_bwd_acc(const float* gy, const float* u_b, const float* u_c, const int* t_h, const int* t_w, const int* o_x,
                   const int* o_y, int policy, int B, int H, int W, float* gsum_ws, float* gx, void* stream);
#define DG_XSUM_PARTS 8
typedef struct DgAugSet {
  const float* x;
  const float* xsum;
  int xsum_parts;
  const float *u_b, *u_c;
  const int *t_h, *t_w, *o_x, *o_y;
} DgAugSet;
int dg_diffaug_blur_fwd(const DgAugSet* sets, int nsets, int policy, int B, int H, int W, int ring, void* out, int dtype,
                        void* stream);
int dg_blur_bwd_augsum(const void* d, int dtype, float* dx, const int* t_h, const int* o_x, const int* o_y, int policy,
                       float* gsum, int B, int H, int W, int ring, void* stream);
int dg_diffaug_bwd_pre(const float* gy, const float* u_b, const float* u_c, const int* t_h, const int* t_w, const int* o_x,
                       const int* o_y, int policy, int B, int H, int W, const float* gsum, float* gx, void* stream);
int dg_head_post_bwd_aug(const float* gout, const float* noise_pixel, const float* noise_image, const float* mask,
                         const float* gy, const float* u_b, const float* u_c, const int* t_h, const int* t_w,
                         const int* o_x, const int* o_y, int policy, const float* gsum, int arch, float tau,
                         float drop_const, int B, int H, int W, float s_depth, float s_conf, float* draw, float* dbias,
                         void* draw_pm, int cp, float* bias_ws, void* stream);

enum { DG_GAN_NSGAN = 0, DG_GAN_WGAN = 1, DG_GAN_LSGAN = 2, DG_GAN_HINGE = 3, DG_GAN_RAGAN = 4, DG_GAN_RAHINGE = 5,
       DG_GAN_RALSGAN = 6 };
int dg_gan_d_step(int metric, float smoothing, const float* y_real, const float* y_fake, int B, float w_gan, float* dy,
                  float* up, float* rs, float* acc, float* dfinal_b, void* stream);
// ... 187 lines not shown
```

Before: 13560.

## Fold real-sample GAN gradient into R1 tangent pass to halve wgrad batch

Adds a folded R1 schedule. The real-sample GAN gradient is merged into the R1 tangent forward: the blur kernel adds a per-sample scaled copy of the stored activation, and the conv kernels seed their accumulators with a per-sample scaled bias. The weight-gradient pass then covers only the tangent-plus-real slots through a rotated gradient index (g_rot), and the real half of the final-layer wgrad is skipped. This removes a separate real-batch contribution from the D backward. In exchange it adds more ABI fields, extra dry-run support checks, and a new dependency on linearity assumptions.

```diff
diff --git a/dusty_gan_amd/_lib.py b/dusty_gan_amd/_lib.py
--- a/dusty_gan_amd/_lib.py
+++ b/dusty_gan_amd/_lib.py
@@ -49,6 +49,7 @@
         ("mask_out", C.c_void_p),
         ("mask_in", C.c_void_p),
         ("tanh_sum_parts", C.c_void_p),
+        ("bias_rowscale", C.c_void_p),
     ]
 
 
@@ -78,7 +79,7 @@
         ("g", C.c_void_p), ("g_sb", C.c_long), ("g_sp", C.c_long), ("g_sc", C.c_long),
         ("dw", C.c_void_p), ("scale", C.c_float), ("rowscale", C.c_void_p),
         ("a_dtype", C.c_int), ("g_dtype", C.c_int),
-        ("ws", C.c_void_p), ("g_mod", C.c_int),
+        ("ws", C.c_void_p), ("g_mod", C.c_int), ("g_rot", C.c_int),
     ]
 
 
@@ -140,6 +141,7 @@
     "dg_blur_bwd": [_P, _I, _P, _I, _I, _I, _I, _P],
     "dg_blur_bwd_r1": [_P, _I, _P, _F, _P, _I, _I, _I, _I, _P],
     "dg_blur_r1_tangent": [_P, _I, _P, _F, _P, _P, _I, _I, _I, _I, _I, _P],
+    "dg_blur_r1_tangent_fold": [_P, _I, _P, _F, _P, _P, _P, _P, _I, _I, _I, _I, _I, _P],
     "dg_final_fwd": [_P, _I, _P, _P, _F, _I, _L, _P, _P],
     "dg_final_fwd_acc": [_P, _I, _P, _P, _F, _I, _L, _P, _P],
     "dg_final_bwd_data": [_P, _I, _P, _P, _P, _F, _I, _L, _I, _P, _P, _P],
diff --git a/dusty_gan_amd/csrc/api.hip b/dusty_gan_amd/csrc/api.hip
--- a/dusty_gan_amd/csrc/api.hip
+++ b/dusty_gan_amd/csrc/api.hip
@@ -38,6 +38,7 @@
   if (p->epi == EPI_MASK && !p->aux) return DG_EINVAL;
   if (p->bias && p->bias_mod <= 0) return DG_EINVAL;
   if (p->dbias && p->bias_mod <= 0) return DG_EINVAL;
+  if (p->bias_rowscale && (p->epi != EPI_MASK || !p->bias || p->dbias)) return DG_EINVAL;
   if (plan) *plan = DgConvPlan{};
   const int force = force_flags & ~DG_FORCE_FP32X3;
   const bool mfma_ok = !p->nscale && dg_conv_mfma_supported(p), thin_ok = dg_conv_thin_supported(p);
@@ -67,9 +68,18 @@
   return DG_OK;
 }
 
+int conv_takes_bias_rowscale(const DgConv* p, ConvKernel k, int force_flags, int wg_cap) {
+  DgConvPlan pl{};
+  const int rc = conv_run(p, k, force_flags, wg_cap, nullptr, &pl);
+  if (rc) return rc;
+  const bool ok = pl.family == DG_CONV_FAMILY_PINGPONG || (pl.family == DG_CONV_FAMILY_THIN && pl.thin_mfma == 1);
+  return ok ? DG_OK : DG_EUNSUPPORTED;
+}
+
 int conv_dispatch(const DgConv* p, int force_flags, int wg_cap, hipStream_t s, DgConvPlan* plan) {
   ConvKernel k;
   int rc = select_conv(p, force_flags, &k, plan);
+  if (rc == DG_OK && p->bias_rowscale) rc = conv_takes_bias_rowscale(p, k, force_flags, wg_cap);
   if (rc || plan || !p->mask_out) return rc ? rc : conv_run(p, k, force_flags, wg_cap, s, plan);
   DgConvPlan pl{};
   rc = conv_run(p, k, force_flags, wg_cap, nullptr, &pl);
diff --git a/dusty_gan_amd/csrc/blur_aug.hip b/dusty_gan_amd/csrc/blur_aug.hip
--- a/dusty_gan_amd/csrc/blur_aug.hip
+++ b/dusty_gan_amd/csrc/blur_aug.hip
@@ -207,12 +207,14 @@
 template <typename T>
 __global__ __launch_bounds__(256) void blur_r1_tangent_kernel(const T* __restrict__ d, T* __restrict__ out, int H, int W,
                                                               int ring, float oscale, float* __restrict__ ssq,
-                                                              float* __restrict__ mean_acc, int mean_n, const DgDet det) {
+                                                              float* __restrict__ mean_acc, int mean_n, const DgDet det,
+                                                              const float* __restrict__ hscale, const T* __restrict__ h0) {
   extern __shared__ float s_g[];
   __shared__ float red[16];
   const int W4 = W >> 2, b = blockIdx.y;
   const long base = (long)b * H * W;
   const int y0 = blockIdx.x * R1T_ROWS;
+  const float hs = hscale ? hscale[b] : 0.f;
   float ssacc = 0.f;
   for (int q4 = threadIdx.x; q4 < W4; q4 += 256) {
     const int x0 = q4 * 4;
@@ -251,6 +253,19 @@
         o[2 * k + 1] = 0.25f * c[k] + 0.5f * c[k + 1] + 0.25f * c[k + 2];
       }
       T* op = out + (base + (long)y * W + x0) * 2;
+      if (hscale) {
+        const T* hp = h0 + (base + (long)y * W + x0) * 2;
+        float hv[8];
+        if constexpr (sizeof(T) == 2) {
+          Vec16<bf16>::load((const bf16*)hp, hv);
+        } else {
+          const float4 h_lo = *(const float4*)hp, h_hi = *(const float4*)(hp + 4);
+          hv[0] = h_lo.x; hv[1] = h_lo.y; hv[2] = h_lo.z; hv[3] = h_lo.w;
+          hv[4] = h_hi.x; hv[5] = h_hi.y; hv[6] = h_hi.z; hv[7] = h_hi.w;
+        }
+#pragma unroll
+        for (int k = 0; k < 8; ++k) o[k] = fmaf(hs, hv[k], o[k]);
+      }
       if constexpr (sizeof(T) == 2) {
         Vec16<bf16>::store((bf16*)op, o);
       } else {
@@ -473,20 +488,26 @@
   return DG_OK;
 }
 
-int dg_blur_r1_tangent(const void* d, int dtype, void* out, float oscale, float* ssq, float* mean_acc, int mean_n, int B, int H,
-                       int W, int ring, void* s_) {
+int dg_blur_r1_tangent_fold(const void* d, int dtype, void* out, float oscale, const float* hscale, const void* h0, float* ssq,
+                            float* mean_acc, int mean_n, int B, int H, int W, int ring, void* s_) {
   hipStream_t s = (hipStream_t)s_;
   if (!d || !out || !ssq || B <= 0 || (mean_acc && mean_n < 1)) return DG_EINVAL;
+  if ((hscale == nullptr) != (h0 == nullptr)) return DG_EINVAL;
+  if (((size_t)h0 & 15) != 0) return DG_EUNSUPPORTED;
   if (dtype != DG_BF16 && dtype != DG_F32) return DG_EINVAL;
   const size_t lds = (size_t)(R1T_ROWS + 2) * W * sizeof(float);
   if (W % 4 != 0 || W < 8 || H < 4 || H % R1T_ROWS != 0 || lds > 60 * 1024 || ((size_t)d & 15) != 0 || ((size_t)out & 15) != 0)
     return DG_EUNSUPPORTED;
   const dim3 grid(H / R1T_ROWS, B);
   const DgDet det = dg_det_current();
-  if (dtype == DG_BF16) blur_r1_tangent_kernel<bf16><<<grid, 256, lds, s>>>((const bf16*)d, (bf16*)out, H, W, ring, oscale, ssq, mean_acc, mean_n, det);
-  else blur_r1_tangent_kernel<float><<<grid, 256, lds, s>>>((const float*)d, (float*)out, H, W, ring, oscale, ssq, mean_acc, mean_n, det);
-  HIP_CHECK_RET(hipGetLastError());
-  return DG_OK;
+  if (dtype == DG_BF16) blur_r1_tangent_kernel<bf16><<<grid, 256, lds, s>>>((const bf16*)d, (bf16*)out, H, W, ring, oscale, ssq, mean_acc, mean_n, det, hscale, (const bf16*)h0);
+  else blur_r1_tangent_kernel<float><<<grid, 256, lds, s>>>((const float*)d, (float*)out, H, W, ring, oscale, ssq, mean_acc, mean_n, det, hscale, (const float*)h0);
+  HIP_CHECK_RET(hipGetLastError());
+  return DG_OK;
+}
+int dg_blur_r1_tangent(const void* d, int dtype, void* out, float oscale, float* ssq, float* mean_acc, int mean_n, int B, int H,
+                       int W, int ring, void* s_) {
+  return dg_blur_r1_tangent_fold(d, dtype, out, oscale, nullptr, nullptr, ssq, mean_acc, mean_n, B, H, W, ring, s_);
 }
 
 static int sample_sum_impl(const float* x, int B, long n, int sq, float* out, bool zero, void* s_) {
diff --git a/dusty_gan_amd/csrc/conv_mfma_pp.hip b/dusty_gan_amd/csrc/conv_mfma_pp.hip
--- a/dusty_gan_amd/csrc/conv_mfma_pp.hip
+++ b/dusty_gan_amd/csrc/conv_mfma_pp.hip
@@ -169,12 +169,15 @@
   float* s_db = s_bias + NDB;
   const unsigned srs0 = lds0 + NPS * PSTAGE, sbias0 = srs0 + NDB * 4, sdb0 = sbias0 + NDB * 4;
   const bool want_db = MASK && p.dbias != nullptr;
+  const bool brs = MASK && p.bias_rowscale != nullptr;
   const bool db_rows = MASK && DBW * p.N <= NDBR * NDB;
   const unsigned sdbw0 = db_rows ? sbias0 + (unsigned)((DUAL ? wave : wave / WN) * p.N) * 4u : sdb0;
   for (int i = tid; i < NDB; i += 64 * NWV) {
-    s_bias[i] = (!MASK && p.bias && i < p.N) ? p.bias[i % p.bias_mod] * (p.epi == EPI_LRELU ? SQRT2 : 1.f) : 0.f;
+    if (brs) s_bias[i] = i < p.N ? p.bias[i % p.bias_mod] / p.scale : 0.f;
+    else s_bias[i] = (!MASK && p.bias && i < p.N) ? p.bias[i % p.bias_mod] * (p.epi == EPI_LRELU ? SQRT2 : 1.f) : 0.f;
     s_db[i] = 0.f;
-    s_rs[i] = (p.rowscale && i < p.B) ? p.rowscale[i] : 1.f;
+    if (brs) s_rs[i] = i < p.B ? p.bias_rowscale[i] : 0.f;
+    else s_rs[i] = (p.rowscale && i < p.B) ? p.rowscale[i] : 1.f;
   }
   if (MASK)
     for (int i = tid; i < NDBX; i += 64 * NWV) s_db[NDB + i] = 0.f;
@@ -194,6 +197,26 @@
   bf16* out = (bf16*)p.out;
   const unsigned lane_c0 = (unsigned)((DUAL ? 0 : wn * WC) + g4 * CPL);
   const unsigned lane_coff = X2 ? lane_c0 * 2 + ((lane_c0 >> 6) << 7) : lane_c0 * 2;
+  auto start_acc = [&](const int t_bt, const int t_nt) __attribute__((always_inline)) {
+    float sb;
+    f32x4_t b0[TN];
+    const unsigned ra = srs0 + (unsigned)(t_bt * g.NSB + ((wm * 64) >> g.lsw)) * 4;
+    const unsigned ba = sbias0 + (unsigned)(t_nt * NCH * 4) + lane_c0 * 4;
+    asm volatile("ds_read_b32 %0, %1" : "=v"(sb) : "v"(ra) : "memory");
+#pragma unroll
+    for (int j = 0; j < TN; ++j)
+      asm volatile("ds_read_b128 %0, %1 offset:%2" : "=v"(b0[j]) : "v"(ba), "n"(j * 16) : "memory");
+    asm volatile("s_waitcnt lgkmcnt(0)" ::: "memory");
+    asm volatile("" : "+v"(sb));
+#pragma unroll
+    for (int j = 0; j < TN; ++j) {
+      asm volatile("" : "+v"(b0[j]));
+      const f32x4_t v = b0[j] * sb;
+#pragma unroll
+      for (int i = 0; i < TM; ++i) acc[i][j] = v;
+    }
+  };
+  if (brs) start_acc(first.bt, first.nt);
   const unsigned par_off = DUAL ? (unsigned)(wn * (int)p.out_sp * 2) : 0u;
   const long px_b = (long)(MODE == MODE_S2 ? 1 : 2) * p.out_sp * 2;
   unsigned pix_off;
@@ -393,6 +416,7 @@
   unsigned long long tsum[6] = {0, 0, 0, 0, 0, 0};
   unsigned long long tend = 0, tkf = 0;
 
+  int nx_bt = first.bt, nx_nt = first.nt;
   if (wave >= 4) __builtin_amdgcn_s_barrier();
   unsigned so_c = PSTAGE, so_i = 0;
   bool pending = false;
@@ -458,8 +482,10 @@
       else if (t == 0) { if (wave == 0) PP_WAIT(IA + IB + 1); else PP_WAIT(IA + IB); }
       else PP_WAIT(IB);
       auto finish_tile = [&]() __attribute__((always_inline)) {
-        if (!(dbg & 4)) epilogue(tprev);
-        else {
+        if (!(dbg & 4)) {
+          epilogue(tprev);
+          if constexpr (MASK && ISS) { if (brs) start_acc(nx_bt, nx_nt); }
+        } else {
 #pragma unroll
           for (int i = 0; i < TM; ++i)
 #pragma unroll
@@ -517,6 +543,7 @@
       nh = (int)(e >> 60) & 7;
       hl = e & 0x0fffffffffffffffull;
     }
+    if (MASK) { nx_bt = ti.bt; nx_nt = ti.nt; }
     const char* in_t = (const char*)(in + (long)(ti.bt * g.NSB) * p.in_sb);
     const char* w_t = (const char*)(w + (long)(ti.nt * NCH) * p.w_sn);
     const int x0 = cmul * ti.xt * BM;
@@ -650,7 +677,8 @@
   if ((Ws & (Ws - 1)) != 0 || p->in_sp * 2 >= (1 << 24)) return DG_EUNSUPPORTED;
   if ((p->mode == MODE_S2 ? p->Hc : 2 * p->Hc) > 256) return DG_EUNSUPPORTED;
   const bool mask = p->epi == EPI_MASK;
-  if (mask ? p->bias != nullptr : p->dbias != nullptr) return DG_EUNSUPPORTED;
+  if (p->bias_rowscale && (!mask || !p->bias || p->dbias || p->scale == 0.f || x2 || p->B > 512)) return DG_EUNSUPPORTED;
+  if (mask ? (p->bias != nullptr && !p->bias_rowscale) : p->dbias != nullptr) return DG_EUNSUPPORTED;
   if (p->rowscale && p->B > 512) return DG_EUNSUPPORTED;
   persist::Geo g;
   int bn = 0;
diff --git a/dusty_gan_amd/csrc/conv_thin.hip b/dusty_gan_amd/csrc/conv_thin.hip
--- a/dusty_gan_amd/csrc/conv_thin.hip
+++ b/dusty_gan_amd/csrc/conv_thin.hip
@@ -487,7 +487,7 @@
     const long u = u0 + gq / gpr;
     const int s0 = (gq % gpr) * WG_GS;
     const int b = (int)(u / p.Hc), Y = (int)(u % p.Hc);
-    const int bg = p.g_mod > 0 ? b % p.g_mod : b;
+    const int bg = p.g_mod > 0 ? (b + p.g_rot) % p.g_mod : b;
     const bf16* grow = G + (long)bg * p.g_sb + ((long)Y * p.Wc + wave * seg + 16 * s0) * p.g_sp;
 #pragma unroll
     for (int st = 0; st < WG_GS; ++st)
@@ -1029,6 +1029,7 @@
   if (!dg_wgrad_thin_supported(p)) return DG_EUNSUPPORTED;
   if (p->ws && !dg_wgrad_thin_ws_splits(p)) return DG_EUNSUPPORTED;
   if (p->g_mod && !wgrad_down_mfma_ok(p)) return DG_EUNSUPPORTED;
+  if (p->g_mod < 0 || p->g_rot < 0 || (p->g_rot && p->g_rot >= p->g_mod)) return DG_EINVAL;
   const long units = (long)p->B * p->Hc;
   const unsigned grid = wgrad_valu_grid(p);
   if (wgrad_down_mfma_ok(p)) {
@@ -1153,7 +1154,9 @@
   v2u pm[2];
   float prs[2];
   const int Wd = Wf * NPXD;
-  const float* rs_src = (p.dbias && p.rowscale) ? p.rowscale : (const float*)p.w;
+  const bool brs = p.bias_rowscale != nullptr;
+  const bool rs_ld = brs || (p.dbias && p.rowscale);
+  const float* rs_src = brs ? p.bias_rowscale : ((p.dbias && p.rowscale) ? p.rowscale : (const float*)p.w);
   const unsigned zero_off = 0u;
   auto out_base = [&](int xt_, int Y_, int b_) -> long { return (long)b_ * p.out_sb + ((long)Y_ * p.Wc + xt_ * 32) * 64; };
   auto prefetch = [&](int xt_, int Y_, int b_, auto buf_tag) __attribute__((always_inline)) {
@@ -1178,7 +1181,7 @@
       pa[I][s] = ta;
       pw[I][s] = tw;
     }
-    const float* rsp = rs_src + ((p.dbias && p.rowscale) ? b_ : 0);
+    const float* rsp = rs_src + (rs_ld ? b_ : 0);
     float trs;
     asm volatile("global_load_dword %0, %1, %2" : "=v"(trs) : "v"(zero_off), "s"(rsp) : "memory");
     prs[I] = trs;
@@ -1228,6 +1231,7 @@
     float rs = prs[I];
     v2u mword = pm[I];
     asm volatile("" : "+v"(rs), "+v"(mword));
+    const float bsc = rs;
     if (!(p.dbias && p.rowscale)) rs = 1.f;
     if (xt == 0 || xt == tiles_x - 1) {
       const bool lo = xt == 0 && lr == 0 && (CP == 2 || lh == 0);
@@ -1270,7 +1274,8 @@
     for (int jt = 0; jt < 2; ++jt)
 #pragma unroll
       for (int g = 0; g < 4; ++g) {
-        const float4 b4 = *(const float4*)&s_binit[jt * 32 + g * 8 + lh * 4];
+        float4 b4 = *(const float4*)&s_binit[jt * 32 + g * 8 + lh * 4];
+        if (brs) { b4.x *= bsc; b4.y *= bsc; b4.z *= bsc; b4.w *= bsc; }
         acc[jt][4 * g] = b4.x; acc[jt][4 * g + 1] = b4.y; acc[jt][4 * g + 2] = b4.z; acc[jt][4 * g + 3] = b4.w;
       }
 #pragma unroll
@@ -1406,6 +1411,7 @@
   if ((cp != 2 && cp != 4) || p->K > cp || p->in_sk != 1 || p->w_sk != 1 || p->out_sn != 1 || p->out_sp != 64) return 0;
   if (p->dbias && p->bias_mod != 64) return 0;
   if (p->bias && p->scale == 0.f) return 0;
+  if (p->bias_rowscale && (p->dbias || !p->bias || p->epi != EPI_MASK)) return 0;
   if (p->out_sb % 64 != 0) return 0;
   return 1;
 }
diff --git a/dusty_gan_amd/csrc/pointwise.hip b/dusty_gan_amd/csrc/pointwise.hip
--- a/dusty_gan_amd/csrc/pointwise.hip
+++ b/dusty_gan_amd/csrc/pointwise.hip
@@ -342,7 +342,7 @@
         const int b = b0 + NW * j;
         if (b < ns) {
           float g[V];
-          const float u = s_u[b], rsb = s_r[b], c = s_dy[b];
+          const float u = s_u[b], rsb = s_r[b], c = (r1 == 2 && b < B) ? 0.f : s_dy[b];
 #pragma unroll
           for (int k = 0; k < V; ++k) {
             g[k] = u * w[k] * (a[j][k] > 0.f ? SQRT2 : LRELU_SLOPE * SQRT2);
@@ -555,7 +555,7 @@
   const int rc = gan_form(metric, mode_g ? 1 : 0, mode_g ? 1.f : smoothing, &fm);
   if (rc != DG_OK) return rc;
   if (mode_g && fm.kr != PHI_NONE && !y_real) return DG_EINVAL;
-  if (mode_g && r1) return DG_EINVAL;
+  if ((mode_g && r1) || r1 < 0 || r1 > 2) return DG_EINVAL;
   const int ns = mode_g ? B : 2 * B;
   const int V = dtype == DG_BF16 ? 8 : 4;
   if (!(vec_ok(d4, n, dtype) && vec_ok(dd4, n, dtype) && C % V == 0 && ns <= 256 && ((size_t)wf & 15) == 0 &&
diff --git a/dusty_gan_amd/csrc/wgrad_mfma_dma.hip b/dusty_gan_amd/csrc/wgrad_mfma_dma.hip
--- a/dusty_gan_amd/csrc/wgrad_mfma_dma.hip
+++ b/dusty_gan_amd/csrc/wgrad_mfma_dma.hip
@@ -114,7 +114,7 @@
       const unsigned lo = __builtin_amdgcn_readfirstlane((unsigned)v), hi = __builtin_amdgcn_readfirstlane((unsigned)(v >> 32));
       return (const char*)(((unsigned long long)hi << 32) | lo);
     };
-    const int bg = p.g_mod > 0 ? b % p.g_mod : b;
+    const int bg = p.g_mod > 0 ? (b + p.g_rot) % p.g_mod : b;
     abase = uni(A + (long)b * p.a_sb + (long)rowa * Wa * asp + ci0 * (X2 ? 2 : 1));
     gbase = uni(G + (long)bg * p.g_sb + (long)rowg * Wg * gsp + co0 * (X2 ? 2 : 1));
   };
@@ -456,7 +456,7 @@
 
 int dg_wgrad_mfma_dma_launch(const WgradP* p, int accumulate, int pairs, hipStream_t stream, DgWgradPlan* plan) {
   if (!dg_wgrad_mfma_dma_supported(p)) return DG_EUNSUPPORTED;
-  if (p->g_mod < 0 || (p->ws && ((size_t)p->ws & 15) != 0)) return DG_EINVAL;
+  if (p->g_mod < 0 || p->g_rot < 0 || (p->g_rot && p->g_rot >= p->g_mod) || (p->ws && ((size_t)p->ws & 15) != 0)) return DG_EINVAL;
   const bool m128 = p->Ci % 128 == 0, n128 = p->Co % 128 == 0;
   if (p->wmode == 0) {
     if (m128 && n128) return launch_dma<0, 128, 128>(p, accumulate, pairs, stream, plan);
@@ -482,7 +482,7 @@
   for (int i = 0; i < n; ++i) {
     const WgradP* p = &items[i];
     if (!dg_wgrad_mfma_dma_supported(p) || (!plans && !p->ws)) return DG_EUNSUPPORTED;
-    if (p->g_mod < 0 || (!plans && ((size_t)p->ws & 15) != 0)) return DG_EINVAL;
+    if (p->g_mod < 0 || p->g_rot < 0 || (p->g_rot && p->g_rot >= p->g_mod) || (!plans && ((size_t)p->ws & 15) != 0)) return DG_EINVAL;
     long target = 512;
     if (rounds > 0) {
       target = (long)(rounds * 512.0 * fl[i] / fsum + 0.5);
diff --git a/dusty_gan_amd/engine.py b/dusty_gan_amd/engine.py
--- a/dusty_gan_amd/engine.py
+++ b/dusty_gan_amd/engine.py
@@ -527,7 +527,8 @@
 
     def conv(self, mode, adj, ring, B, Hc, Wc, K, N, x, x_strides, out, out_strides, w_ptr, scale, epi,
              bias=None, bias_mod=0, aux=None, dbias=None, rowscale=None, in_dt=None, out_dt=None, nscale=None,
-             x_off=0, out_off=0, aux_off=0, w_strides=None, w_dt=None, up_frag=None, defer_db=False, tanh_sums=None):
+             x_off=0, out_off=0, aux_off=0, w_strides=None, w_dt=None, up_frag=None, defer_db=False, tanh_sums=None,
+             bias_rowscale=None, dry=False):
         x2_out = None
         if mode == L.MODE_GEMM and (is_x2(x) or is_x2(out) or is_x2(aux)):
             if is_x2(x):
@@ -567,6 +568,7 @@
         p.dbias, p.rowscale = dbias, L.ptr(rowscale)
         p.in_dtype, p.out_dtype, p.w_dtype = in_dt, out_dt, (self.dt if w_dt is None else w_dt)
         p.nscale = L.ptr(nscale)
+        p.bias_rowscale = L.ptr(bias_rowscale)
         p.up_frag = up_frag
         sum_parts = 0
         if tanh_sums is not None:
@@ -579,6 +581,8 @@
             p.mask_out = MaskBits.slice_ptr(out, out_off, N, out_strides)
         elif epi == L.EPI_MASK and aux is not None and out_dt == L.DG_BF16:
             p.mask_in = MaskBits.slice_ptr(aux, aux_off, N, out_strides)
+        if dry:
+            return self.lib.dg_conv_plan(C.byref(p), self._f, self.wg_cap, C.byref(L.DgConvPlan())) == L.DG_OK
         if dbias is not None:
             ws = Ops._dbias_ws.get(str(x.device))
             if ws is None:
@@ -634,9 +638,9 @@
         return pl
 
     def wgrad(self, wmode, ring, B, Hc, Wc, Ci, Co, a, a_strides, g, g_strides, dw_ptr, scale, rowscale=None,
-              accumulate=1, a_dt=None, g_dt=None, a_off=0, g_off=0, g_mod=0, defer=False):
+              accumulate=1, a_dt=None, g_dt=None, a_off=0, g_off=0, g_mod=0, defer=False, g_rot=0):
         p = self._wgrad_params(wmode, ring, B, Hc, Wc, Ci, Co, a, a_strides, g, g_strides, dw_ptr, scale, rowscale, a_dt,
-                               g_dt, a_off, g_off, g_mod)
+                               g_dt, a_off, g_off, g_mod, g_rot)
         pl = self.wgrad_plan(p, accumulate) if self.use_ws else None
         if (self._group is not None and defer and pl is not None and pl.ws_floats > 0 and pl.variant == L.DG_WGRAD_VARIANT_DMA
                 and len(self._group) < self.GROUP_MAX and pl.ws_floats <= WgradWorkspace.FLOATS):
@@ -729,7 +733,7 @@
         return self.lib.dg_wgrad_has_sample_map(C.byref(p), self._f) == 1
 
     def _wgrad_params(self, wmode, ring, B, Hc, Wc, Ci, Co, a, a_strides, g, g_strides, dw_ptr, scale, rowscale, a_dt, g_dt,
-                      a_off, g_off, g_mod):
+                      a_off, g_off, g_mod, g_rot=0):
         if wmode == 2:
             if is_x2(a):
                 a = x2_unpack(a, self._f32_copy("wa", a))
@@ -750,7 +754,7 @@
         p.g_sb, p.g_sp, p.g_sc = g_strides
         p.dw, p.scale, p.rowscale = dw_ptr, scale, L.ptr(rowscale)
         p.a_dtype, p.g_dtype = a_dt, g_dt
-        p.ws, p.g_mod = None, int(g_mod)
+        p.ws, p.g_mod, p.g_rot = None, int(g_mod), int(g_rot)
         return p
 
 
@@ -1080,6 +1084,7 @@
         self.x2_asked = bool(x2)
         self.x2 = self.x2_asked and self.ops.x3 and x2_eligible(cfg)
         self.ws_B = 0
+        self._fold_ok = {}
 
     def alloc(self, nb, device):
         if self.ws_B >= nb and self.h[0].device == device:
@@ -1098,6 +1103,7 @@
             self.h4f, self.e4f = torch.empty_like(self.h[4]), torch.empty_like(self.e[4])
         self.y = torch.empty(nb, dtype=torch.float32, device=device)
         self.ws_B = nb
+        self._fold_ok = {}
 
     def forward(self, st, x, slot, tangent_of=None, mean=None):
         c, o, lib = self.cfg, self.ops, L.lib()
@@ -1131,7 +1137,18 @@
             A.apply(x, rp, out=xcat[k * n:(k + 1) * n])
         return self.forward(st, xcat, slot)
 
-    def _layers(self, st, n, slot, tangent_of):
+    def _down(self, st, i, n, slot, tangent_of, fold=None, dry=False):
+        c, o = self.cfg, self.ops
+        hc, wc = self.grid[i]
+        ci, co = self.chs[i - 1], self.chs[i]
+        tang = tangent_of is not None
+        return o.conv(L.MODE_S2, 0, c.ring, n, hc, wc, ci, co, self.h[i - 1], (self.per[i - 1], ci, 1), self.h[i],
+                      (self.per[i], co, 1), L.ptr(st.coci[f"d{i}_w"]), 1.0 / math.sqrt(ci * 16),
+                      L.EPI_MASK if tang else L.EPI_LRELU, bias=None if (tang and fold is None) else st.fptr(f"d{i}_b"),
+                      bias_mod=co, aux=self.h[i] if tang else None, x_off=slot * self.per[i - 1], out_off=slot * self.per[i],
+                      aux_off=(tangent_of or 0) * self.per[i], bias_rowscale=fold if tang else None, dry=dry)
+
+    def _layers(self, st, n, slot, tangent_of, fold=None):
         c, o, lib = self.cfg, self.ops, L.lib()
         sp = L.stream_ptr()
         if self.x2:
@@ -1139,14 +1156,7 @@
         st.refresh_shadows(self.dtype)
         es = o.es
         for i in range(1, 5):
-            hc, wc = self.grid[i]
-            ci, co = self.chs[i - 1], self.chs[i]
-            tang = tangent_of is not None
-            o.conv(L.MODE_S2, 0, c.ring, n, hc, wc, ci, co, self.h[i - 1], (self.per[i - 1], ci, 1), self.h[i],
-                   (self.per[i], co, 1), L.ptr(st.coci[f"d{i}_w"]), 1.0 / math.sqrt(ci * 16),
-                   L.EPI_MASK if tang else L.EPI_LRELU, bias=None if tang else st.fptr(f"d{i}_b"), bias_mod=co,
-                   aux=self.h[i] if tang else None, x_off=slot * self.per[i - 1], out_off=slot * self.per[i],
-                   aux_off=(tangent_of or 0) * self.per[i])
+            self._down(st, i, n, slot, tangent_of, fold)
         if tangent_of is None:
             nf = self.per[4]
             h4 = self._h4(slot, n)
@@ -1240,15 +1250,37 @@
                                 int(c.ring), L.stream_ptr()), "dg_blur_bwd")
         return True
 
-    def r1_turnaround(self, st, slot, n, tslot, oscale, ssq, mean_ptr):
+    def _r1_turnaround_shape(self):
+        c = self.cfg
+        return not (c.W % 4 or c.H % 4 or 6 * c.W * 4 > 60 * 1024)
+
+    def r1_fold_ok(self, st, B, rs):
+        if os.environ.get("DUSTY_GAN_R1_FOLD", "1") == "0" or self.x2 or not self._r1_turnaround_shape():
+            return False
+        ok = self._fold_ok.get(B)
+        if ok is None:
+            c, o = self.cfg, self.ops
+            st.refresh_shadows(self.dtype)
+            ok = all(self._down(st, i, B, 2 * B, 0, rs, dry=True) for i in range(1, 5))
+            for i in range(1, 5):
+                hc, wc = self.grid[i]
+                ci, co = self.chs[i - 1], self.chs[i]
+                ok = ok and o.wgrad_takes_map(0, c.ring, 2 * B, hc, wc, ci, co, self.h[i - 1], (self.per[i - 1], ci, 1),
+                                              self.e[i], (self.per[i], co, 1), st.fptr(f"d{i}_w", st.grad))
+            self._fold_ok[B] = ok
+        return ok
+
+    def r1_turnaround(self, st, slot, n, tslot, oscale, ssq, mean_ptr, fold=None):
         c, o, lib = self.cfg, self.ops, L.lib()
-        if c.W % 4 or c.H % 4 or 6 * c.W * 4 > 60 * 1024:
+        if not self._r1_turnaround_shape():
             return False
         self._bwd_layer(st, 1, slot, n, None, False)
-        L.check(lib.dg_blur_r1_tangent(L.ptr(self.e[0]) + o.es * slot * self.per[0], o.dt,
-                                       L.ptr(self.h[0]) + o.es * tslot * self.per[0], float(oscale), L.ptr(ssq), mean_ptr, int(n),
-                                       n, c.H, c.W, int(c.ring), L.stream_ptr()), "dg_blur_r1_tangent")
-        self._layers(st, n, tslot, slot)
+        h0 = L.ptr(self.h[0])
+        L.check(lib.dg_blur_r1_tangent_fold(L.ptr(self.e[0]) + o.es * slot * self.per[0], o.dt,
+                                            h0 + o.es * tslot * self.per[0], float(oscale), L.ptr(fold),
+                                            None if fold is None else h0 + o.es * slot * self.per[0], L.ptr(ssq), mean_ptr,
+                                            int(n), n, c.H, c.W, int(c.ring), L.stream_ptr()), "dg_blur_r1_tangent")
+        self._layers(st, n, tslot, slot, fold)
         return True
 
     def backward_input_aug(self, st, slot, n, A, rp, lazy=False):
@@ -1269,7 +1301,7 @@
                                 int(c.ring), L.stream_ptr()), "dg_blur_bwd")
         return A.backward(dx, rp)
 
-    def wgrad(self, st, a_slot, g_slot, n, rowscale, layers=(1, 2, 3, 4), g_mod=0):
+    def wgrad(self, st, a_slot, g_slot, n, rowscale, layers=(1, 2, 3, 4), g_mod=0, g_rot=0):
         c, o = self.cfg, self.ops
         with o.grouped():
             for i in layers:
@@ -1277,10 +1309,13 @@
                 ci, co = self.chs[i - 1], self.chs[i]
                 o.wgrad(0, c.ring, n, hc, wc, ci, co, self.h[i - 1], (self.per[i - 1], ci, 1), self.e[i],
                         (self.per[i], co, 1), st.fptr(f"d{i}_w", st.grad), 1.0 / math.sqrt(ci * 16), rowscale=rowscale,
-                        a_off=a_slot * self.per[i - 1], g_off=g_slot * self.per[i], g_mod=g_mod, defer=True)
-
-    def wgrad_r1(self, st, B, rs3, layers=(1, 2, 3, 4)):
+                        a_off=a_slot * self.per[i - 1], g_off=g_slot * self.per[i], g_mod=g_mod, g_rot=g_rot, defer=True)
+
+    def wgrad_r1(self, st, B, rs3, layers=(1, 2, 3, 4), fold=False):
         c, o = self.cfg, self.ops
+        if fold:
+            self.wgrad(st, B, 0, 2 * B, None, layers=layers, g_mod=2 * B, g_rot=B)
+            return
         with o.grouped():
             for i in layers:
                 hc, wc = self.grid[i]
diff --git a/dusty_gan_amd/trainers/dcgan_amp.py b/dusty_gan_amd/trainers/dcgan_amp.py
--- a/dusty_gan_amd/trainers/dcgan_amp.py
+++ b/dusty_gan_amd/trainers/dcgan_amp.py
@@ -687,13 +687,16 @@
             y = deng.forward_aug(Dst, self.A, [(x_real, rand["aug"][0]), (synth["depth"], rand["aug"][1])], 0)
             dy = torch.empty(2 * B, **f32)
             up = torch.empty(2 * B, **f32) if gp > 0 else None
-            rs = None
+            rs, ssq, fold = None, None, False
             if gp > 0:
                 if getattr(self, "_rs3", None) is None or self._rs3.numel() != 3 * B or self._rs3.device != self.device:
                     self._rs3 = torch.ones(3 * B, **f32)
                 rs = self._rs3
+                ssq = L.AccArena.take(B, dev)
+                fold = ssq is not None and deng.r1_fold_ok(Dst, B, rs)
             fused = deng.final_gan_bwd(Dst, 0, B, self.gan_code, False, float(self.criterion["gan"].smoothing), w_gan,
-                                       L.ptr(y), L.ptr(y) + 4 * B, gp > 0, dy, up, rs, L.ptr(scal), True, True)
+                                       L.ptr(y), L.ptr(y) + 4 * B, (2 if fold else 1) if gp > 0 else 0, dy, up, rs, L.ptr(scal),
+                                       True, True)
             if not fused:
                 L.check(lib.dg_gan_d_step(self.gan_code, float(self.criterion["gan"].smoothing), L.ptr(y),
                                           L.ptr(y) + 4 * B, B, w_gan, L.ptr(dy), L.ptr(up), L.ptr(rs), L.ptr(scal),
@@ -703,8 +706,10 @@
             if gp > 0:
                 deng.backward_data(Dst, 0, 2 * B, up, rs, want_dbias=True, skip_final=fused)
                 vscale = gp / self.n_acc / B
-                ssq = L.AccArena.take(B, dev)
-                if ssq is None or not deng.r1_turnaround(Dst, 0, B, 2 * B, vscale, ssq, L.ptr(scal) + 12):
+                if fold:
+                    if not deng.r1_turnaround(Dst, 0, B, 2 * B, vscale, ssq, L.ptr(scal) + 12, fold=rs):
+                        raise L.DgError("the folded R1 schedule was selected for a shape r1_turnaround does not take")
+                elif ssq is None or not deng.r1_turnaround(Dst, 0, B, 2 * B, vscale, ssq, L.ptr(scal) + 12):
                     g = torch.empty(B, 1, self.H, self.W, **f32)
                     vg = torch.empty_like(g)
                     if ssq is None or not deng.backward_input(Dst, 0, B, vg, r1=(vscale, ssq)):
@@ -717,9 +722,11 @@
                         L.check(lib.dg_scale(L.ptr(g), vscale, g.numel(), L.ptr(vg), sp), "dg_scale")
                     deng.forward(Dst, vg, 2 * B, tangent_of=0, mean=(ssq, B, L.ptr(scal) + 12))
                 for layers in (((4,), (3, 2, 1)) if bucketed else ((4, 3, 2, 1),)):
-                    deng.wgrad_r1(Dst, B, rs, layers=layers)
+                    deng.wgrad_r1(Dst, B, rs, layers=layers, fold=fold)
                     if 4 in layers:
-                        if not fused:
+                        if not fused and fold:
+                            deng.final_wgrad(Dst, B, B, dy[B:])
+                        elif not fused:
                             deng.final_wgrad(Dst, 0, 2 * B, dy)
                         if (not bucketed and self.n_acc == 1 and not deng.x2 and self.optim_D.will_fuse(self.dtype)):
                             extra_D = {"final_w": deng.final_wgrad_term(2 * B, B)}
diff --git a/include/dusty_gan_hip.h b/include/dusty_gan_hip.h
--- a/include/dusty_gan_hip.h
+++ b/include/dusty_gan_hip.h
@@ -48,6 +48,7 @@
   void* mask_out;
   const void* mask_in;
   float* tanh_sum_parts;
+  const float* bias_rowscale;
 } DgConv;
 #define DG_UP_FRAG_BYTES (3 * 18 * 1024)
 #define DG_DBIAS_SLOTS 32
@@ -67,6 +68,7 @@
   int a_dtype, g_dtype;
   float* ws;
   int g_mod;
+  int g_rot;
 } DgWgrad;
 
 int dg_conv(const DgConv* p, int force, void* stream);
@@ -137,6 +139,8 @@
 int dg_blur_bwd_r1(const void* d, int dtype, float* dx, float oscale, float* ssq, int B, int H, int W, int ring, void* stream);
 int dg_blur_r1_tangent(const void* d, int dtype, void* out, float oscale, float* ssq, float* mean_acc, int mean_n, int B, int H,
                        int W, int ring, void* stream);
+int dg_blur_r1_tangent_fold(const void* d, int dtype, void* out, float oscale, const float* hscale, const void* h0, float* ssq,
+                            float* mean_acc, int mean_n, int B, int H, int W, int ring, void* stream);
 
 int dg_final_fwd(const void* d4, int dtype, const float* wf, const float* bias, float scale, int B, long n, float* y,
                  void* stream);
```

Result: slower. 13350 (-1.5%).
